# s-esposito/MonoGS

Hardware: AMD Instinct MI355X
Metric: rasteriser fwd+bwd Mpix/s @1080p (higher is better)
Workload: dtype f32; 1 GPU; C5: 2000000 Gaussians, 1920x1080, fwd+bwd, seeded synthetic map (SURVEY.md 8d), one keyframe per GPU; gaussians=2000000, width=1920, height=1080, settle_steps=60, instance_count=device-side (capacity mode, overflow checked), parallelism=keyframe-per-gpu x1

## Files before the change

monogs_amd/csrc/api.hip:

```cpp
#include "common.h"

#include <stdarg.h>
#include <stdio.h>
#include <string.h>

namespace mgs {

static thread_local char g_err[512] = "";

void set_error(const char* fmt, ...) {
    va_list ap;
    va_start(ap, fmt);
    vsnprintf(g_err, sizeof(g_err), fmt, ap);
    va_end(ap);
}

static inline char* take(char*& p, size_t bytes) {
    char* r = p;
    p += align_up(bytes, 256);
    return r;
}

GeometryState GeometryState::carve(void* base, int P) {
    char* p = (char*)align_up((size_t)base, 256);
// ... 17 lines not shown
    g.end = p;
    return g;
}
size_t GeometryState::bytes(int P) {
    const GeometryState g = carve(nullptr, P);
    return (size_t)g.end + 256;
}

size_t ImageState::bytes(int W, int H) {
    const size_t HW = (size_t)W * H, nt = (size_t)tiles_x(W) * tiles_y(H);
    return align_up(HW * 4, 256) * 2 + align_up(nt * sizeof(uint2), 256) + 256;
}
ImageState ImageState::carve(void* base, int W, int H) {
    const size_t HW = (size_t)W * H, nt = (size_t)tiles_x(W) * tiles_y(H);
    char* p = (char*)align_up((size_t)base, 256);
    ImageState s;
    s.final_T = (float*)take(p, HW * 4);
    s.n_contrib = (uint32_t*)take(p, HW * 4);
    s.ranges = (uint2*)take(p, nt * sizeof(uint2));
    return s;
}

size_t BinningState::fwd_mask_rows(uint64_t R, int W, int H) {
    return (size_t)(R / 64) + (size_t)tiles_x(W) * tiles_y(H) + 1;
}
size_t BinningState::bytes(uint64_t R, int W, int H) {
    const size_t r = (size_t)(R ? R : 1);
    return align_up(r * 4, 256) * 4 + align_up(mgs::sort_temp_bytes(R, tile_bits(W, H)), 256) + 256 +
           align_up(fwd_mask_rows(R, W, H) * 4 * sizeof(unsigned long long), 256) + 256;
}
BinningState BinningState::carve(void* base, uint64_t R, int W, int H) {
    const size_t r = (size_t)(R ? R : 1);
    char* p = (char*)align_up((size_t)base, 256);
    BinningState b;
    b.keys_a = (uint32_t*)take(p, r * 4);
    b.keys_b = (uint32_t*)take(p, r * 4);
    b.vals_a = (uint32_t*)take(p, r * 4);
    b.vals_b = (uint32_t*)take(p, r * 4);
    const bool in_b = radix_result_in_b(tile_bits(W, H));
    b.keys_sorted = in_b ? b.keys_b : b.keys_a;
    b.vals_sorted = in_b ? b.vals_b : b.vals_a;
    b.sort_temp_bytes = mgs::sort_temp_bytes(R, tile_bits(W, H));
    b.sort_temp = take(p, b.sort_temp_bytes);
    b.count = (uint32_t*)take(p, 2 * sizeof(uint32_t));
    b.fwd_masks = (unsigned long long*)take(p, fwd_mask_rows(R, W, H) * 4 * sizeof(unsigned long long));
    return b;
}

struct StageTimer {
    hipStream_t s;
    bool on;
    hipEvent_t ev[10];
    int n = 0;
    StageTimer(hipStream_t s_, bool on_) : s(s_), on(on_) {
        if (on) for (auto& e : ev) (void)hipEventCreate(&e);
    }
    ~StageTimer() {
        if (on) for (auto& e : ev) (void)hipEventDestroy(e);
    }
    void mark() {
        if (on && n < 10) (void)hipEventRecord(ev[n++], s);
    }
    float ms(int i) {
        float t = 0.f;
        if (on && i + 1 < n) (void)hipEventElapsedTime(&t, ev[i], ev[i + 1]);
        return t;
    }
    void sync() {
        if (on && n) (void)hipEventSynchronize(ev[n - 1]);
    }
};

static int check_cam(const mgs_camera* cam) {
    if (!cam) { set_error("camera is NULL"); return 1; }
    if (cam->image_width <= 0 || cam->image_height <= 0) { set_error("image size must be positive"); return 1; }
    if (!cam->bg || !cam->viewmatrix || !cam->projmatrix || !cam->projmatrix_raw || !cam->campos) {
        set_error("camera tensors (bg, viewmatrix, projmatrix, projmatrix_raw, campos) must be non-NULL");
        return 1;
    }
    return 0;
}

static hipEvent_t g_dbg_fwd_events[2] = {nullptr, nullptr}, g_dbg_bwd_events[2] = {nullptr, nullptr};

static int check_map_size(int32_t P) {
    if (P > MGS_MAX_GAUSSIANS) {
        set_error("P exceeds MGS_MAX_GAUSSIANS (2^26 - 1): the gradient-line offset of the blend backward is 32-bit");
        return 1;
    }
    return 0;
}

}

using namespace mgs;

extern "C" {

int mgs_abi_version(void) { return MGS_ABI_VERSION; }
int mgs_binning_path(int32_t P, int32_t W, int32_t H) { return binning_path(P, W, H); }
const char* mgs_last_error(void) { return g_err; }

size_t mgs_geometry_bytes(int32_t P) { return GeometryState::bytes(P < 0 ? 0 : P); }
size_t mgs_image_bytes(int32_t W, int32_t H) { return ImageState::bytes(W, H); }
size_t mgs_binning_bytes(uint64_t R, int32_t W, int32_t H) { return BinningState::bytes(R, W, H); }
size_t mgs_backward_bytes(int32_t P) {
    return (size_t)(P < 0 ? 0 : P) * GRAD_FLOATS * sizeof(float) + (size_t)(TAU_SLOTS + 1) * 16 * sizeof(float) + 256;
}
float* mgs_backward_tau(void* backward_scratch, int32_t P) { return backward_tau_out(backward_scratch, P < 0 ? 0 : P); }

int mgs_forward_preprocess(const mgs_camera* cam, int32_t P, const float* means3D, const float* shs,
                           const float* colors_precomp, const float* opacities, const float* scales,
                           const float* rotations, const float* cov3D_precomp, void* geometry, int32_t* radii,
                           void* prepare_backward, uint64_t* num_rendered, const uint32_t* prev_status,
                           uint32_t* prev_status_out, mgs_timing* timing, void* stream) {
    if (check_cam(cam)) return 1;
    if (P < 0) { set_error("P must be >= 0"); return 1; }
    if (check_map_size(P)) return 1;
    if (num_rendered) *num_rendered = 0;
    if (prev_status_out) *prev_status_out = 0;
    if (P == 0) {
        if (prev_status && prev_status_out) {
            MGS_HIP(hipMemcpyAsync(prev_status_out, prev_status, sizeof(uint32_t), hipMemcpyDeviceToHost, (hipStream_t)stream));
            MGS_HIP(hipStreamSynchronize((hipStream_t)stream));
        }
        return 0;
    }
    if (!means3D || !opacities || !geometry || !radii) { set_error("means3D, opacities, geometry, radii must be non-NULL"); return 1; }
    if ((shs == nullptr) == (colors_precomp == nullptr)) {
        set_error("Please provide excatly one of either SHs or precomputed colors!");
        return 1;
    }
    const bool have_sr = scales != nullptr || rotations != nullptr;
    if ((have_sr && (!scales || !rotations || cov3D_precomp)) || (!have_sr && !cov3D_precomp)) {
        set_error("Please provide exactly one of either scale/rotation pair or precomputed 3D covariance!");
        return 1;
    }
    if (shs && (cam->sh_degree < 0 || cam->sh_degree > 3 || cam->sh_coeffs < (cam->sh_degree + 1) * (cam->sh_degree + 1))) {
        set_error("sh_degree must be 0..3 and shs must hold at least (degree+1)^2 coefficients");
        return 1;
    }
    hipStream_t s = (hipStream_t)stream;
    GeometryState g = GeometryState::carve(geometry, P);
    StageTimer tm(s, timing != nullptr);
    tm.mark();
    if (int rc = launch_preprocess_forward(*cam, P, means3D, shs, colors_precomp, opacities, scales, rotations,
                                           cov3D_precomp, g, radii,
                                           prepare_backward ? backward_grad_acc(prepare_backward) : nullptr, s)) return rc;
    tm.mark();
    const bool exclusive = (cam->flags & MGS_FLAG_EXCLUSIVE_DEVICE) != 0;
    const bool per_tile = binning_path(P, cam->image_width, cam->image_height) != 0;
    if (per_tile) {
        tm.mark();
        if (int rc = launch_scan(g, P, s, exclusive, g.rect)) return rc;
    } else {
        if (int rc = launch_depth_sort(g, P, depth_sort_payload(P, cam->image_width, cam->image_height), s, exclusive)) return rc;
        tm.mark();
        if (int rc = launch_scan(g, P, s, exclusive, g.rect_sorted)) return rc;
    }
    tm.mark();
    if (num_rendered) {
        uint32_t total = 0, sort_errors[RADIX_ERROR_WORDS] = {0, 0, 0, 0};
        MGS_HIP(hipMemcpyAsync(&total, g.scan_blocks + scan_nblocks(P), sizeof(uint32_t), hipMemcpyDeviceToHost, s));
        MGS_HIP(hipMemcpyAsync(sort_errors, radix_depth_error_flag(g.sort_temp, (uint64_t)P), sizeof(sort_errors),
                               hipMemcpyDeviceToHost, s));
        if (prev_status && prev_status_out)
            MGS_HIP(hipMemcpyAsync(prev_status_out, prev_status, sizeof(uint32_t), hipMemcpyDeviceToHost, s));
        MGS_HIP(hipStreamSynchronize(s));
        if (sort_errors[0] | sort_errors[1] | sort_errors[2] | sort_errors[3]) { set_error("depth sort: a look-back spin timed out (results invalid)"); return 3; }
        *num_rendered = total;
    }
    if (timing) {
        if (!num_rendered) MGS_HIP(hipStreamSynchronize(s));
        timing->preprocess_ms = tm.ms(0);
        timing->depth_sort_ms = per_tile ? 0.f : tm.ms(1);
        timing->scan_ms = tm.ms(2);
    }
    return 0;
}

static int g_opt_tile_sort_fused = 1;

static int forward_render_impl(const mgs_camera* cam, int32_t P, uint64_t R, bool capacity, void* geometry,
                               void* binning, void* image, float* out_color, float* out_depth, float* out_opacity,
                               int32_t* n_touched, uint32_t* overflow, mgs_timing* timing, void* stream) {
    if (check_cam(cam)) return 1;
    if (P < 0) { set_error("P must be >= 0"); return 1; }
    if (check_map_size(P)) return 1;
    if (!image || !out_color || !out_depth || !out_opacity) { set_error("image scratch and outputs must be non-NULL"); return 1; }
    if (P > 0 && (!geometry || !n_touched)) { set_error("geometry and n_touched must be non-NULL"); return 1; }
    if (R > 0 && !binning) { set_error("binning scratch is NULL"); return 1; }
    if (R >= (1ull << 32)) { set_error("num_rendered exceeds 2^32-1"); return 1; }
    if (P == 0) R = 0;
    hipStream_t s = (hipStream_t)stream;
    const int W = cam->image_width, H = cam->image_height;
    GeometryState g = GeometryState::carve(geometry, P);
    ImageState img = ImageState::carve(image, W, H);
    BinningState b = BinningState::carve(binning, R, W, H);
    const uint32_t* n_dev = nullptr;
    StageTimer tm(s, timing != nullptr);
    const bool cap = capacity && binning;
    if (cap) n_dev = b.count;
    const bool per_tile = binning_path(P, W, H) != 0;
    tm.mark();
    if (int rc = launch_duplicate(*cam, P, g, b, capacity ? R : (R > 0 ? 0xFFFFFFFFull : 0ull), n_touched, img, R,
                                  tile_bits(W, H), cap ? b.count : nullptr, overflow, s, per_tile)) return rc;
    tm.mark();
    if (int rc = launch_sort(g, b, R, tile_bits(W, H), s, n_dev, (cam->flags & MGS_FLAG_EXCLUSIVE_DEVICE) != 0, img.ranges,
                             per_tile)) return rc;
    const uint32_t* sort_err = R > 0 ? radix_error_flag(b.sort_temp, R, tile_bits(W, H)) : nullptr;
    const bool sort_tiles = per_tile && R > 0;
    const TileSortArgs ts = sort_tiles ? tile_sort_args(*cam, g, b, R, n_dev) : TileSortArgs{};
    const bool fused = sort_tiles && g_opt_tile_sort_fused != 0;
    if (sort_tiles && !fused)
        if (int rc = launch_tile_depth_sort(*cam, ts, img, sort_err, s)) return rc;
    tm.mark();
    if (g_dbg_fwd_events[0]) MGS_HIP(hipEventRecord(g_dbg_fwd_events[0], s));
    if (int rc = launch_blend_forward(*cam, g, b, img, out_color, out_depth, out_opacity, n_touched, sort_err, overflow,
                                      fused ? &ts : nullptr, P, s)) return rc;
    if (g_dbg_fwd_events[1]) MGS_HIP(hipEventRecord(g_dbg_fwd_events[1], s));
    tm.mark();
    if (timing) {
        tm.sync();
        timing->duplicate_ms = tm.ms(0);
        timing->sort_ms = tm.ms(1);
        timing->ranges_ms = 0.f;
        timing->blend_fwd_ms = tm.ms(2);
    }
    return 0;
}

int mgs_forward_render(const mgs_camera* cam, int32_t P, uint64_t R, void* geometry, void* binning, void* image,
                       float* out_color, float* out_depth, float* out_opacity, int32_t* n_touched,
                       uint32_t* status, mgs_timing* timing, void* stream) {
    return forward_render_impl(cam, P, R, false, geometry, binning, image, out_color, out_depth, out_opacity, n_touched,
                               status, timing, stream);
}

int mgs_forward_render_capacity(const mgs_camera* cam, int32_t P, uint64_t capacity, void* geometry, void* binning,
                                void* image, float* out_color, float* out_depth, float* out_opacity,
                                int32_t* n_touched, uint32_t* overflow, mgs_timing* timing, void* stream) {
    if (capacity == 0) { set_error("capacity must be > 0"); return 1; }
    return forward_render_impl(cam, P, capacity, true, geometry, binning, image, out_color, out_depth, out_opacity,
                               n_touched, overflow, timing, stream);
}

int mgs_forward_capacity(const mgs_camera* cam, int32_t P, const float* means3D, const float* shs,
                         const float* colors_precomp, const float* opacities, const float* scales, const float* rotations,
                         const float* cov3D_precomp, void* geometry, int32_t* radii, void* prepare_backward,
                         uint64_t capacity, void* binning, void* image, float* out_color, float* out_depth,
                         float* out_opacity, int32_t* n_touched, uint32_t* overflow, mgs_timing* timing, void* stream) {
    if (int rc = mgs_forward_preprocess(cam, P, means3D, shs, colors_precomp, opacities, scales, rotations, cov3D_precomp,
                                        geometry, radii, prepare_backward, nullptr, nullptr, nullptr, timing, stream)) return rc;
    return mgs_forward_render_capacity(cam, P, capacity, geometry, binning, image, out_color, out_depth, out_opacity,
                                       n_touched, overflow, timing, stream);
}

int mgs_backward(const mgs_camera* cam, int32_t P, uint64_t R, const float* means3D, const float* shs,
                 const float* colors_precomp, const float* opacities, const float* scales, const float* rotations,
                 const float* cov3D_precomp, const int32_t* radii, const void* geometry, const void* binning,
                 const void* image, const float* dL_dcolor, const float* dL_ddepth, const float* out_color,
                 const float* out_depth, float* dL_dmeans2D, float* dL_dcolors, float* dL_dopacity, float* dL_dmeans3D, float* dL_dcov3D, float* dL_dsh,
                 float* dL_dscales, float* dL_drotations, float* dL_dtau, void* backward_scratch,
                 int32_t scratch_prepared, mgs_timing* timing, void* stream) {
    if (check_cam(cam)) return 1;
    if (P < 0) { set_error("P must be >= 0"); return 1; }
    if (check_map_size(P)) return 1;
    hipStream_t s = (hipStream_t)stream;
    if (P == 0) {
        if (dL_dtau) MGS_HIP(zero_fill(dL_dtau, 6 * sizeof(float), s));
        return 0;
    }
    if (!means3D || !opacities || !radii || !geometry || !image || !dL_dcolor || !dL_ddepth || !backward_scratch) {
        set_error("means3D, opacities, radii, geometry, image, dL_dcolor, dL_ddepth, backward_scratch must be non-NULL");
        return 1;
    }
    if (R > 0 && !binning) { set_error("binning scratch is NULL"); return 1; }
    const int W = cam->image_width, H = cam->image_height;
    GeometryState g = GeometryState::carve(const_cast<void*>(geometry), P);
    ImageState img = ImageState::carve(const_cast<void*>(image), W, H);
    BinningState b = BinningState::carve(const_cast<void*>(binning), R, W, H);
    float* grad_acc = backward_grad_acc(backward_scratch);
    StageTimer tm(s, timing != nullptr);
    float* tau_part = (dL_dtau && (P + 255) / 256 > TAU_DIRECT_MAX_BLOCKS) ? backward_tau_part(backward_scratch, P) : nullptr;
    if (scratch_prepared) {
        if (dL_dtau && dL_dtau != backward_tau_out(backward_scratch, P)) {
            set_error("scratch_prepared: dL_dtau must be mgs_backward_tau(backward_scratch, P)");
            return 1;
        }
    } else {
        MGS_HIP(zero_fill2(grad_acc, (size_t)P * GRAD_FLOATS * sizeof(float) + (tau_part ? (size_t)TAU_SLOTS * 16 * sizeof(float) : 0),
                           dL_dtau, 6 * sizeof(float), s));
    }
    tm.mark();
    if (R > 0) {
        const bool pose_only = !dL_dcolors && !dL_dopacity && !dL_dsh && !shs;
        if (g_dbg_bwd_events[0]) MGS_HIP(hipEventRecord(g_dbg_bwd_events[0], s));
        if (int rc = launch_blend_backward(*cam, g, b, img, dL_dcolor, dL_ddepth, out_color, out_depth, grad_acc, pose_only, R, s)) return rc;
        if (g_dbg_bwd_events[1]) MGS_HIP(hipEventRecord(g_dbg_bwd_events[1], s));
    }
    tm.mark();
    GeomBackwardArgs a;
    a.means3D = means3D; a.shs = shs; a.colors_precomp = colors_precomp; a.opacities = opacities;
    a.scales = scales; a.rotations = rotations; a.cov3D_precomp = cov3D_precomp; a.radii = radii;
    a.grad_acc = grad_acc;
    a.dL_dmeans2D = dL_dmeans2D; a.dL_dcolors = dL_dcolors; a.dL_dopacity = dL_dopacity;
    a.dL_dmeans3D = dL_dmeans3D; a.dL_dcov3D = dL_dcov3D; a.dL_dsh = dL_dsh; a.dL_dscales = dL_dscales;
// ... 154 lines not shown
```

monogs_amd/csrc/binning.hip:

```cpp
#include "common.h"
#include "tile_sort.h"


namespace mgs {

constexpr int SCAN_THREADS = 256;
__device__ __forceinline__ int scan_nblocks_dev(int P) { return (P + SCAN_ITEMS - 1) / SCAN_ITEMS; }
constexpr int SCAN_PER_THREAD = SCAN_ITEMS / SCAN_THREADS;

__device__ __forceinline__ uint32_t wave_incl_scan(uint32_t v, int) { return wave_incl_scan_dpp(v); }

__device__ __forceinline__ uint32_t block_excl_scan(uint32_t v, uint32_t& total, uint32_t* smem ) {
    const int lane = threadIdx.x & 63, wv = threadIdx.x >> 6;
    const uint32_t incl = wave_incl_scan(v, lane);
    if (lane == 63) smem[wv] = incl;
    __syncthreads();
    uint32_t base = 0;
    for (int w = 0; w < wv; ++w) base += smem[w];
    total = smem[0] + smem[1] + smem[2] + smem[3];
    __syncthreads();
    return base + incl - v;
}

__device__ __forceinline__ uint32_t scan_block_rows(const uint2* __restrict__ rects, int n, int cbase, int lane, int wv,
                                                    uint32_t (&incl)[SCAN_PER_THREAD], uint32_t* smem ) {
    uint32_t v[SCAN_PER_THREAD];
#pragma unroll
    for (int i = 0; i < SCAN_PER_THREAD; ++i) {
        const int idx = cbase + i * WAVE + lane;
        const uint32_t wh = idx < n ? rects[idx].y : 0u;
        v[i] = (wh & 0xFFFFu) * (wh >> 16);
    }
    uint32_t run = 0;
#pragma unroll
    for (int i = 0; i < SCAN_PER_THREAD; ++i) {
        const uint32_t sc = wave_incl_scan_dpp(v[i]);
        incl[i] = run + sc;
        run += (uint32_t)__builtin_amdgcn_readlane((int)sc, 63);
    }
    if (lane == 0) smem[wv] = run;
    __syncthreads();
    uint32_t wbase = 0;
    for (int w = 0; w < wv; ++w) wbase += smem[w];
    const uint32_t total = (smem[0] + smem[1]) + (smem[2] + smem[3]);
#pragma unroll
    for (int i = 0; i < SCAN_PER_THREAD; ++i) incl[i] += wbase;
    return total;
}

__global__ void __launch_bounds__(SCAN_THREADS) scan_local_kernel(const uint2* __restrict__ rects, uint32_t* out,
                                                                  uint32_t* block_sums, int n) {
    __shared__ uint32_t smem[8];
    const int lane = threadIdx.x & 63, wv = threadIdx.x >> 6;
    const int cbase = blockIdx.x * SCAN_ITEMS + wv * (SCAN_PER_THREAD * WAVE);
    uint32_t incl[SCAN_PER_THREAD];
    const uint32_t total = scan_block_rows(rects, n, cbase, lane, wv, incl, smem);
#pragma unroll
    for (int i = 0; i < SCAN_PER_THREAD; ++i) {
        const int idx = cbase + i * WAVE + lane;
        if (idx < n) out[idx] = incl[i];
    }
    if (threadIdx.x == 0) block_sums[blockIdx.x] = total;
}

__global__ void __launch_bounds__(SCAN_THREADS) scan_blocks_kernel(uint32_t* block_sums, int nblocks) {
    __shared__ uint32_t smem[8];
    uint32_t carry = 0;
    for (int start = 0; start < nblocks; start += SCAN_THREADS) {
        const int i = start + threadIdx.x;
        const uint32_t v = i < nblocks ? block_sums[i] : 0u;
        uint32_t total;
        const uint32_t ex = block_excl_scan(v, total, smem);
        if (i < nblocks) block_sums[i] = carry + ex;
        carry += total;
    }
    if (threadIdx.x == 0) block_sums[nblocks] = carry;
}

constexpr uint32_t SCAN_SPIN_LIMIT = 1u << 22;
__global__ void __launch_bounds__(SCAN_THREADS) scan_small_kernel(const uint2* __restrict__ rects, uint32_t* out,
                                                                  uint32_t* block_sums, uint64_t* status, int n, int nb,
                                                                  uint32_t* err, int ticketed) {
    __shared__ uint32_t smem[8];
    __shared__ uint32_t s_prefix, s_bid;
    const int lane = threadIdx.x & 63, wv = threadIdx.x >> 6;
    int bid = (int)blockIdx.x;
    if (ticketed) {
        if (threadIdx.x == 0) s_bid = atomicAdd((uint32_t*)(status + SCAN_SMALL_MAX_BLOCKS), 1u);
        __syncthreads();
        bid = (int)s_bid;
    }
    const int cbase = bid * SCAN_ITEMS + wv * (SCAN_PER_THREAD * WAVE);
    uint32_t incl[SCAN_PER_THREAD];
    const uint32_t total = scan_block_rows(rects, n, cbase, lane, wv, incl, smem);
    if (threadIdx.x == 0)
        __hip_atomic_store(status + bid, (1ull << 63) | (uint64_t)total, __ATOMIC_RELAXED, __HIP_MEMORY_SCOPE_AGENT);
    if (threadIdx.x < WAVE) {
        uint32_t before = 0;
        if ((int)threadIdx.x < bid) {
            uint64_t w = 0;
            uint32_t spins = 0;
            while (true) {
                w = __hip_atomic_load(status + threadIdx.x, __ATOMIC_RELAXED, __HIP_MEMORY_SCOPE_AGENT);
                if (w >> 63) break;
                if (++spins > SCAN_SPIN_LIMIT) { atomicExch(err, 1u); break; }
                __builtin_amdgcn_s_sleep(1);
            }
            before = (uint32_t)w;
        }
#pragma unroll
        for (int o = 32; o > 0; o >>= 1) before += __shfl_xor(before, o, 64);
        if (threadIdx.x == 0) s_prefix = before;
    }
    __syncthreads();
#pragma unroll
    for (int i = 0; i < SCAN_PER_THREAD; ++i) {
        const int idx = cbase + i * WAVE + lane;
        if (idx < n) out[idx] = incl[i] + s_prefix;
    }
    if (threadIdx.x == 0 && bid == nb - 1) block_sums[nb] = s_prefix + total;
}
int g_opt_scan_small = -1;
bool scan_is_small(int P) { return g_opt_scan_small != 0 && scan_nblocks(P) <= SCAN_SMALL_MAX_BLOCKS; }


int launch_scan(const GeometryState& g, int P, hipStream_t s, bool exclusive, const uint2* rects) {
    if (P == 0) return 0;
    const int nb = scan_nblocks(P);
    if (scan_is_small(P)) {
        hipLaunchKernelGGL(scan_small_kernel, dim3(nb), dim3(SCAN_THREADS), 0, s, rects, g.point_offsets, g.scan_blocks,
                           g.scan_status, P, nb, const_cast<uint32_t*>(radix_depth_error_flag(g.sort_temp, (uint64_t)P)),
                           exclusive ? 0 : 1);
        MGS_HIP(hipGetLastError());
        return 0;
    }
    hipLaunchKernelGGL(scan_local_kernel, dim3(nb), dim3(SCAN_THREADS), 0, s, rects, g.point_offsets,
                       g.scan_blocks, P);
    hipLaunchKernelGGL(scan_blocks_kernel, dim3(1), dim3(SCAN_THREADS), 0, s, g.scan_blocks, nb);
    MGS_HIP(hipGetLastError());
    return 0;
}

__device__ __forceinline__ void dup_pair(uint32_t gidx, const uint32_t* __restrict__ depth_key, int lo, uint32_t& val,
                                         uint32_t& kfield) {
    val = gidx; kfield = 0u;
    if (depth_key) {
        const uint32_t k = depth_key[gidx];
        const uint32_t d = k == 0xFFFFFFFFu ? DEPTH_KEY_NARROW : min(k - DEPTH_KEY_SUB, DEPTH_KEY_NARROW);
        kfield = d >> lo;
        if (lo) val |= (d & ((1u << lo) - 1u)) << (32 - lo);
    }
}
__global__ void __launch_bounds__(256) duplicate_kernel(int P, const uint2* __restrict__ rects,
                                                        const uint32_t* __restrict__ perm,
                                                        const uint32_t* __restrict__ depth_key, int tshift, int lo,
                                                        const uint32_t* __restrict__ offsets ,
                                                        const uint32_t* __restrict__ block_sums ,
                                                        uint32_t* keys,
                                                        uint32_t* vals, int gx, int gy, uint32_t r_cap,
                                                        int32_t* __restrict__ n_touched, uint2* __restrict__ ranges,
                                                        int ntiles, uint32_t* __restrict__ zero_ptr, size_t zero_words,
                                                        uint32_t* __restrict__ count, uint32_t* __restrict__ overflow,
                                                        const uint32_t* __restrict__ depth_err, int offsets_global,
                                                        uint32_t* __restrict__ hist , int hist_passes,
                                                        int n_threads , int slot_major,
                                                        unsigned long long* __restrict__ prepare ) {
    const int i = blockIdx.x * 256 + threadIdx.x;
    if (i == 0 && prepare) {
        prepare[1] = prepare[0];
        prepare[0] = 0ull;
    }
    const int lane = threadIdx.x & 63;
    grid_zero(zero_ptr, zero_words, (size_t)n_threads, 256);
    const bool depth_bad = depth_err && radix_failed(depth_err) != 0u;
    if (i == 0 && count) {
        const uint32_t R = (P > 0 && !depth_bad) ? block_sums[scan_nblocks_dev(P)] : 0u;
        count[0] = min(R, r_cap);
        count[1] = R > r_cap ? 1u : 0u;
    }
    if (i == 0 && overflow)
        overflow[0] = (count ? count[1] : 0u) | (depth_bad ? (uint32_t)MGS_STATUS_DEPTH_SORT_TIMEOUT : 0u);
    if (i < ntiles) ranges[i] = make_uint2(0xFFFFFFFFu, 0u);
    if (i < P) n_touched[i] = 0;
    uint32_t idx = 0, nt = 0, off = 0, kf = 0;
    int x0 = 0, y0 = 0, x1 = 0;
    if (i < P) {
        dup_pair(perm ? perm[i] : (uint32_t)i, depth_key, lo, idx, kf);
        const uint2 r = rects[i];
        const int w = (int)(r.y & 0xFFFFu), h = (int)(r.y >> 16);
        nt = (uint32_t)(w * h);
        x0 = (int)(r.x & 0xFFFFu); y0 = (int)(r.x >> 16); x1 = x0 + w;
    }
    if (depth_bad) nt = 0;
    if (nt) off = i == 0 ? 0u : offsets[i - 1] + (offsets_global ? 0u : block_sums[(i - 1) / SCAN_ITEMS]);
    __shared__ uint32_t s_own[4][WAVE];
    __shared__ uint32_t s_idx[4][WAVE], s_off[4][WAVE], s_kf[4][WAVE];
    __shared__ int s_x0[4][WAVE], s_y0[4][WAVE], s_w[4][WAVE];
    __shared__ uint32_t s_hist[2][256];
    if (hist) {
        s_hist[0][threadIdx.x] = 0u; s_hist[1][threadIdx.x] = 0u;
        __syncthreads();
    }
    const int wv = threadIdx.x >> 6;
    if (slot_major) {
        const uint32_t R_all = (P > 0 && !depth_bad) ? block_sums[scan_nblocks_dev(P)] : 0u;
        const uint32_t R_emit = min(R_all, r_cap);
        const uint32_t n_waves = (uint32_t)n_threads / WAVE;
        const uint32_t CH = (((R_emit + n_waves - 1u) / n_waves) + 63u) & ~63u;
        const uint32_t wave_id = (uint32_t)blockIdx.x * 4u + (uint32_t)wv;
        const uint64_t s0w = (uint64_t)wave_id * CH;
        const uint32_t s0 = s0w < (uint64_t)R_emit ? (uint32_t)s0w : R_emit, s1 = (uint64_t)s0 + CH < (uint64_t)R_emit ? s0 + CH : R_emit;
        auto incl = [&](uint32_t k) { return offsets[k] + (offsets_global ? 0u : block_sums[k / SCAN_ITEMS]); };
        uint32_t g = 0;
        if (s0 < s1) {
            uint32_t lo = 0, hi = (uint32_t)P;
            while (hi - lo > 1u) {
                const uint32_t span = hi - lo, step = (span + 63u) / 64u;
                const uint32_t probe = lo + min(((uint32_t)lane + 1u) * step, span) - 1u;
                const unsigned long long above = __builtin_amdgcn_ballot_w64(incl(probe) > s0);
                const int k = __builtin_ctzll(above);
                const uint32_t pk = lo + min(((uint32_t)k + 1u) * step, span) - 1u;
                const uint32_t pk1 = k == 0 ? lo : lo + min((uint32_t)k * step, span);
                lo = pk1; hi = pk + 1u;
            }
            g = lo;
        }
        uint32_t sl = s0;
        while (sl < s1 && g < (uint32_t)P) {
            const uint32_t gi = g + (uint32_t)lane;
            const bool valid = gi < (uint32_t)P;
            uint32_t inc = 0, ntg = 0, idg = 0, kfg = 0;
            int gx0 = 0, gy0 = 0, gw = 1;
            if (valid) {
                inc = incl(gi);
                const uint2 r = rects[gi];
                gw = (int)(r.y & 0xFFFFu);
                ntg = (uint32_t)(gw * (int)(r.y >> 16));
                gx0 = (int)(r.x & 0xFFFFu); gy0 = (int)(r.x >> 16);
                dup_pair(perm ? perm[gi] : gi, depth_key, lo, idg, kfg);
            }
            const uint32_t exc = inc - ntg;
            uint32_t Eg = valid ? inc : 0u;
#pragma unroll
            for (int o2 = 32; o2 > 0; o2 >>= 1) Eg = max(Eg, (uint32_t)__shfl_xor((int)Eg, o2, 64));
            __builtin_amdgcn_wave_barrier();
            s_idx[wv][lane] = idg; s_kf[wv][lane] = kfg; s_off[wv][lane] = exc; s_x0[wv][lane] = gx0; s_y0[wv][lane] = gy0; s_w[wv][lane] = max(gw, 1);
            const uint32_t e = min(s1, Eg);
            const uint32_t cb0 = sl & ~63u;
            const unsigned long long before = __builtin_amdgcn_ballot_w64(ntg != 0u && exc < cb0);
            uint32_t carry = before ? 64u - (uint32_t)__builtin_clzll(before) : 0u;
            for (uint32_t cb = cb0; cb < e; cb += WAVE) {
                __builtin_amdgcn_wave_barrier();
                s_own[wv][lane] = 0u;
                __builtin_amdgcn_wave_barrier();
                if (ntg != 0u && exc >= cb && exc < cb + WAVE) s_own[wv][exc - cb] = (uint32_t)lane + 1u;
                __builtin_amdgcn_wave_barrier();
                uint32_t m = s_own[wv][lane];
#define MGS_DPP_MAX(ctrl, row_mask) m = max(m, (uint32_t)__builtin_amdgcn_update_dpp(0, (int)m, ctrl, row_mask, 0xf, false))
                MGS_DPP_MAX(0x111, 0xf); MGS_DPP_MAX(0x112, 0xf); MGS_DPP_MAX(0x114, 0xf); MGS_DPP_MAX(0x118, 0xf);
                MGS_DPP_MAX(0x142, 0xa); MGS_DPP_MAX(0x143, 0xc);
#undef MGS_DPP_MAX
                const uint32_t owner = max(m, carry);
                carry = (uint32_t)__builtin_amdgcn_readlane((int)owner, 63);
                const uint32_t o = cb + lane;
                if (owner != 0u && o >= sl && o < e) {
                    const uint32_t L = owner - 1u;
                    const uint32_t t = o - s_off[wv][L];
                    const uint32_t w = (uint32_t)s_w[wv][L];
                    const uint32_t yy = t / w, xx = t - yy * w;
                    const uint32_t tid = (uint32_t)((s_y0[wv][L] + (int)yy) * gx + s_x0[wv][L] + (int)xx);
                    const uint32_t key = (tid << tshift) | s_kf[wv][L];
                    keys[o] = key;
                    vals[o] = s_idx[wv][L];
                    if (hist) {
                        atomicAdd(&s_hist[0][(key >> tshift) & 0xFFu], 1u);
                        if (hist_passes > 1) {
                            const uint32_t d1 = (key >> (tshift + 8)) & 0xFFu;
                            const uint32_t lead = (uint32_t)__builtin_amdgcn_readfirstlane((int)d1);
                            const unsigned long long same = __builtin_amdgcn_ballot_w64(d1 == lead);
                            if (d1 != lead) atomicAdd(&s_hist[1][d1], 1u);
                            else if (lane == (int)__builtin_ctzll(same)) atomicAdd(&s_hist[1][lead], (uint32_t)__popcll(same));
                        }
                    }
                }
            }
            sl = max(sl, e);
            if (Eg <= sl) g += WAVE;
        }
        if (hist) {
            __syncthreads();
            const uint32_t c0 = s_hist[0][threadIdx.x], c1 = s_hist[1][threadIdx.x];
            if (c0) atomicAdd(hist + threadIdx.x, c0);
            if (c1) atomicAdd(hist + 256 + threadIdx.x, c1);
        }
        return;
    }
    s_idx[wv][lane] = idx; s_kf[wv][lane] = kf; s_off[wv][lane] = off; s_x0[wv][lane] = x0; s_y0[wv][lane] = y0; s_w[wv][lane] = max(x1 - x0, 1);
    const unsigned long long live = __builtin_amdgcn_ballot_w64(nt != 0);
    if (live == 0ull && !hist) return;
    const int first = live ? __builtin_ctzll(live) : 0, lastl = live ? 63 - __builtin_clzll(live) : 0;
    const uint32_t S = live ? (uint32_t)__builtin_amdgcn_readlane((int)off, first) : 0u;
    const uint32_t E = live ? (uint32_t)__builtin_amdgcn_readlane((int)(off + nt), lastl) : 0u;
    uint32_t carry = 0;
    for (uint32_t cb = S & ~63u; cb < E; cb += WAVE) {
        __builtin_amdgcn_wave_barrier();
        s_own[wv][lane] = 0u;
        __builtin_amdgcn_wave_barrier();
        if (nt != 0 && off >= cb && off < cb + WAVE) s_own[wv][off - cb] = (uint32_t)lane + 1u;
        __builtin_amdgcn_wave_barrier();
        uint32_t m = s_own[wv][lane];
#define MGS_DPP_MAX(ctrl, row_mask) m = max(m, (uint32_t)__builtin_amdgcn_update_dpp(0, (int)m, ctrl, row_mask, 0xf, false))
        MGS_DPP_MAX(0x111, 0xf); MGS_DPP_MAX(0x112, 0xf); MGS_DPP_MAX(0x114, 0xf); MGS_DPP_MAX(0x118, 0xf);
        MGS_DPP_MAX(0x142, 0xa); MGS_DPP_MAX(0x143, 0xc);
#undef MGS_DPP_MAX
        const uint32_t owner = max(m, carry);
        carry = (uint32_t)__builtin_amdgcn_readlane((int)owner, 63);
        const uint32_t o = cb + lane;
        if (owner != 0u && o < E && o < r_cap) {
            const uint32_t L = owner - 1u;
            const uint32_t t = o - s_off[wv][L];
            const uint32_t w = (uint32_t)s_w[wv][L];
            const uint32_t yy = t / w, xx = t - yy * w;
            const uint32_t tid = (uint32_t)((s_y0[wv][L] + (int)yy) * gx + s_x0[wv][L] + (int)xx);
            const uint32_t key = (tid << tshift) | s_kf[wv][L];
            keys[o] = key;
            vals[o] = s_idx[wv][L];
            if (hist) {
                atomicAdd(&s_hist[0][(key >> tshift) & 0xFFu], 1u);
                if (hist_passes > 1) {
                    const uint32_t d1 = (key >> (tshift + 8)) & 0xFFu;
                    const uint32_t lead = (uint32_t)__builtin_amdgcn_readfirstlane((int)d1);
                    const unsigned long long same = __builtin_amdgcn_ballot_w64(d1 == lead);
                    if (d1 != lead) atomicAdd(&s_hist[1][d1], 1u);
                    else if (lane == (int)__builtin_ctzll(same)) atomicAdd(&s_hist[1][lead], (uint32_t)__popcll(same));
                }
            }
        }
    }
    if (hist) {
        __syncthreads();
        const uint32_t c0 = s_hist[0][threadIdx.x], c1 = s_hist[1][threadIdx.x];
        if (c0) atomicAdd(hist + threadIdx.x, c0);
        if (c1) atomicAdd(hist + 256 + threadIdx.x, c1);
    }
}

constexpr uint64_t DUP_SLOT_MAJOR_MIN = 768ull * 1024;
int g_opt_dup_slot_major = -1;

int launch_duplicate(const mgs_camera& cam, int P, const GeometryState& g, const BinningState& b, uint64_t r_cap,
                     int32_t* n_touched, const ImageState& img, uint64_t sort_n, int sort_bits, uint32_t* count,
                     uint32_t* overflow, hipStream_t s, bool per_tile) {
    const uint32_t* depth_err = P > 0 ? radix_depth_error_flag(g.sort_temp, (uint64_t)P) : nullptr;
    const int ntiles = tiles_x(cam.image_width) * tiles_y(cam.image_height);
    int n = P > ntiles ? P : ntiles;
    if (n == 0) return 0;
    const bool slot_major = P > 0 && g_opt_dup_slot_major != 0 &&
                            (g_opt_dup_slot_major > 0 || (sort_n >= DUP_SLOT_MAJOR_MIN && sort_n >= 6ull * (uint64_t)P));
    if (slot_major) {
        const uint64_t want = sort_n / 8;
        if (want > (uint64_t)n) n = (int)(want > 0x3FFFFFFFull ? 0x3FFFFFFFull : want);
    }
    const int n_threads = (n + 255) / 256 * 256;
    uint32_t* zero_ptr = nullptr;
    size_t zero_words = 0;
    if (sort_n > 0) radix_zero_region(b.sort_temp, sort_n, sort_bits, &zero_ptr, &zero_words);
    const bool count_digits = P > 0 && sort_bits <= 16 && radix_wants_hist(sort_n);
    const int tb = tile_bits(cam.image_width, cam.image_height);
    hipLaunchKernelGGL(duplicate_kernel, dim3(n_threads / 256), dim3(256), 0, s, P, per_tile ? g.rect : g.rect_sorted,
                       per_tile ? nullptr : g.perm, per_tile ? g.depth_key : nullptr, per_tile ? 32 - tb : 0,
                       per_tile ? tile_depth_lo_bits(tb) : 0, g.point_offsets,
                       g.scan_blocks, b.keys_a, b.vals_a, tiles_x(cam.image_width), tiles_y(cam.image_height),
                       (uint32_t)(r_cap > 0xFFFFFFFFull ? 0xFFFFFFFFull : r_cap), n_touched, img.ranges, ntiles, zero_ptr,
                       zero_words, count, overflow, depth_err,
                       (P > 0 && scan_is_small(P)) ? 1 : 0,
                       count_digits ? g.tile_hist : nullptr, (sort_bits + 7) / 8, n_threads, slot_major ? 1 : 0,
                       P > 0 ? g.prepare : nullptr);
    MGS_HIP(hipGetLastError());
    return 0;
}

size_t sort_temp_bytes(uint64_t n, int bits) { return radix_temp_bytes(n, bits); }

int launch_depth_sort(const GeometryState& g, int P, bool payload, hipStream_t s, bool exclusive) {
    return radix_sort_depth(g.depth_key, g.depth_alt, g.iota, g.iota_alt, g.rect, payload, g.perm, g.rect_sorted, (uint64_t)P,
                            g.sort_temp, s, true, exclusive);
}

int launch_sort(const GeometryState& g, const BinningState& b, uint64_t R, int bits, hipStream_t s, const uint32_t* n_dev,
                bool exclusive, uint2* ranges, bool per_tile) {
    if (R == 0) return 0;
    const bool counted = bits <= 16 && radix_wants_hist(R) && g.tile_hist != nullptr;
    return radix_sort_pairs(b.keys_a, b.vals_a, b.keys_b, b.vals_b, R, bits, b.sort_temp, s, n_dev, true, nullptr, nullptr,
                            counted ? g.tile_hist : nullptr, false, exclusive, ranges, per_tile ? 32 - bits : 0);
}

TileSortArgs tile_sort_args(const mgs_camera& cam, const GeometryState& g, const BinningState& b, uint64_t R,
                            const uint32_t* n_dev) {
    TileSortArgs ts;
    ts.keys = b.keys_sorted;
    ts.vals = b.vals_sorted;
    ts.keys_alt = b.keys_sorted == b.keys_a ? b.keys_b : b.keys_a;
    ts.vals_alt = b.vals_sorted == b.vals_a ? b.vals_b : b.vals_a;
    ts.depth_key = g.depth_key;
    ts.n_dev = n_dev;
    ts.n_cap = (uint32_t)R;
    ts.tb = tile_bits(cam.image_width, cam.image_height);
    return ts;
}

__global__ void __launch_bounds__(TDS_THREADS) tile_depth_sort_kernel(TileSortArgs ts, const uint2* __restrict__ ranges,
                                                                       int ntiles, const uint32_t* __restrict__ sort_err) {
    __shared__ uint32_t s_k[TDS_CAP], s_v[TDS_CAP];
    __shared__ uint32_t s_cnt[TDS_WAVES][TDS_RADIX];
    __shared__ uint32_t s_wsum[TDS_WAVES], s_red[2 * TDS_WAVES];
    const int tile = blockIdx.x;
    if (tile >= ntiles) return;
    tile_depth_sort(ts, ranges[tile], sort_err && radix_failed(sort_err) != 0u, TdsLds{s_k, s_v, s_cnt, s_wsum, s_red});
}

int launch_tile_depth_sort(const mgs_camera& cam, const TileSortArgs& ts, const ImageState& img, const uint32_t* sort_err,
                           hipStream_t s) {
    const int ntiles = tiles_x(cam.image_width) * tiles_y(cam.image_height);
    hipLaunchKernelGGL(tile_depth_sort_kernel, dim3(ntiles), dim3(TDS_THREADS), 0, s, ts, img.ranges, ntiles, sort_err);
    MGS_HIP(hipGetLastError());
    return 0;
}


}
```

monogs_amd/csrc/common.h:

```cpp
#pragma once

#include <hip/hip_runtime.h>
#include <stdint.h>
#include <stddef.h>

#include "../../include/monogs_raster.h"

namespace mgs {

constexpr int TILE = MGS_TILE;
constexpr int WAVE = 64;
constexpr int SUB = 8;
constexpr int REC_FLOATS = 16;
constexpr int GRAD_FLOATS = 16;

enum : int {
    R_X = 0, R_Y = 1, R_EX = 2, R_EY = 3,
    R_CA = 4, R_CB = 5, R_CC = 6, R_OPAC = 7,
    R_R = 8, R_G = 9, R_B = 10, R_DEPTH = 11,
    R_NA = 12, R_NB = 13, R_NC = 14, R_RADIUS = 15
};
enum : int {
    G_SX = 0, G_SY = 1, G_SXX = 2, G_SXY = 3, G_SYY = 4, G_SH = 5,
    G_DR = 6, G_DG = 7, G_DB = 8, G_DDEPTH = 9
};

inline size_t align_up(size_t v, size_t a) { return (v + a - 1) / a * a; }

#if defined(__HIP_DEVICE_COMPILE__)
typedef const float __attribute__((address_space(4))) * const_float_p;
typedef const unsigned long long __attribute__((address_space(4))) * const_u64_p;
#define MGS_CONST(p) ((mgs::const_float_p)(p))
#define MGS_CONST_U64(p) ((mgs::const_u64_p)(p))
#else
typedef const float* const_float_p;
typedef const unsigned long long* const_u64_p;
#define MGS_CONST(p) (p)
#define MGS_CONST_U64(p) (p)
#endif

__device__ __forceinline__ uint32_t wave_incl_scan_dpp(uint32_t v) {
#define MGS_DPP_ADD(ctrl, row_mask) v += (uint32_t)__builtin_amdgcn_update_dpp(0, (int)v, ctrl, row_mask, 0xf, false)
    MGS_DPP_ADD(0x111, 0xf);
    MGS_DPP_ADD(0x112, 0xf);
    MGS_DPP_ADD(0x114, 0xf);
    MGS_DPP_ADD(0x118, 0xf);
    MGS_DPP_ADD(0x142, 0xa);
    MGS_DPP_ADD(0x143, 0xc);
#undef MGS_DPP_ADD
    return v;
}

__global__ static void zero_fill_kernel(uint32_t* __restrict__ p, size_t n_words, int vec) {
    const size_t i0 = (size_t)blockIdx.x * blockDim.x + threadIdx.x, stride = (size_t)gridDim.x * blockDim.x;
    if (vec) {
        uint4* q = reinterpret_cast<uint4*>(p);
        const size_t nv = n_words / 4;
        for (size_t i = i0; i < nv; i += stride) q[i] = make_uint4(0u, 0u, 0u, 0u);
        for (size_t i = nv * 4 + i0; i < n_words; i += stride) p[i] = 0u;
    } else {
        for (size_t i = i0; i < n_words; i += stride) p[i] = 0u;
    }
}
__device__ __forceinline__ void grid_zero(uint32_t* __restrict__ p, size_t n_words, size_t threads, int block) {
    const size_t i0 = (size_t)blockIdx.x * block + threadIdx.x, stride = threads;
    uint4* q = reinterpret_cast<uint4*>(p);
    const size_t nv = n_words / 4;
    for (size_t i = i0; i < nv; i += stride) q[i] = make_uint4(0u, 0u, 0u, 0u);
    for (size_t i = nv * 4 + i0; i < n_words; i += stride) p[i] = 0u;
}
__global__ static void zero_fill2_kernel(uint32_t* __restrict__ p, size_t n_words, uint32_t* __restrict__ p2, int n2) {
    grid_zero(p, n_words, (size_t)gridDim.x * 256, 256);
    if (blockIdx.x == 0 && (int)threadIdx.x < n2) p2[threadIdx.x] = 0u;
}
static inline hipError_t zero_fill2(void* ptr, size_t bytes, void* ptr2, size_t bytes2, hipStream_t s) {
    const size_t n_words = bytes / 4;
    size_t blocks = (n_words / 4 + 255) / 256;
    blocks = blocks < 1 ? 1 : (blocks > 4096 ? 4096 : blocks);
    hipLaunchKernelGGL(zero_fill2_kernel, dim3((unsigned)blocks), dim3(256), 0, s, (uint32_t*)ptr, n_words,
                       (uint32_t*)ptr2, ptr2 ? (int)(bytes2 / 4) : 0);
    return hipGetLastError();
}
static inline hipError_t zero_fill(void* ptr, size_t bytes, hipStream_t s) {
    if (bytes == 0) return hipSuccess;
    const size_t n_words = bytes / 4;
    const int vec = ((size_t)ptr % 16 == 0) ? 1 : 0;
    const size_t items = vec ? (n_words + 3) / 4 : n_words;
    size_t blocks = (items + 255) / 256;
    if (blocks > 4096) blocks = 4096;
    hipLaunchKernelGGL(zero_fill_kernel, dim3((unsigned)blocks), dim3(256), 0, s, (uint32_t*)ptr, n_words, vec);
    return hipGetLastError();
}

struct GeometryState {
    float* rec;
    uint32_t* depth_key;
    uint32_t* depth_alt;
    uint32_t* iota;
    uint32_t* iota_alt;
    uint32_t* perm;
    uint32_t* point_offsets;
    uint32_t* scan_blocks;
    uint8_t* clamped;
    uint2* rect;
    uint2* rect_sorted;
    uint64_t* scan_status;
    uint32_t* tile_hist;
    void* sort_temp;
    size_t sort_temp_bytes;
    unsigned long long* prepare;
    char* end;
    static size_t bytes(int P);
    static GeometryState carve(void* base, int P);
};
constexpr int SCAN_SMALL_MAX_BLOCKS = 64;

struct ImageState {
    float* final_T;
    uint32_t* n_contrib;
    uint2* ranges;
    static size_t bytes(int W, int H);
    static ImageState carve(void* base, int W, int H);
};

struct BinningState {
    uint32_t* keys_a;
    uint32_t* vals_a;
    uint32_t* keys_b;
    uint32_t* vals_b;
    uint32_t* keys_sorted;
    uint32_t* vals_sorted;
    void* sort_temp;
    size_t sort_temp_bytes;
    uint32_t* count;
    unsigned long long* fwd_masks;
    static size_t fwd_mask_rows(uint64_t R, int W, int H);
    static size_t bytes(uint64_t R, int W, int H);
    static BinningState carve(void* base, uint64_t R, int W, int H);
};

constexpr int SCAN_ITEMS = 2048;
inline int scan_nblocks(int P) { return (P + SCAN_ITEMS - 1) / SCAN_ITEMS; }

inline int tiles_x(int W) { return (W + TILE - 1) / TILE; }
inline int tiles_y(int H) { return (H + TILE - 1) / TILE; }
inline int tile_bits(int W, int H) {
    uint32_t n = (uint32_t)(tiles_x(W) * tiles_y(H));
    int b = 0;
    while ((1u << b) < n && b < 31) ++b;
    return b == 0 ? 1 : b;
}

constexpr uint32_t DEPTH_KEY_SUB = 0x3E4CCCCDu;
constexpr uint32_t DEPTH_KEY_NARROW = (1u << 27) - 1u;
__host__ __device__ inline int tile_depth_lo_bits(int tb) { return tb > 5 ? tb - 5 : 0; }
int binning_path(int P, int W, int H);

void set_error(const char* fmt, ...);
#define MGS_HIP(expr)                                                                     \
    do {                                                                                  \
        hipError_t _e = (expr);                                                           \
        if (_e != hipSuccess) {                                                           \
            mgs::set_error("%s failed: %s (%s:%d)", #expr, hipGetErrorString(_e), __FILE__, __LINE__); \
            return 2;                                                                     \
        }                                                                                 \
    } while (0)

struct StageTimer;

int launch_preprocess_forward(const mgs_camera& cam, int P, const float* means3D, const float* shs,
                              const float* colors_precomp, const float* opacities, const float* scales,
                              const float* rotations, const float* cov3D_precomp,
                              const GeometryState& g, int32_t* radii, float* prepare_grad_acc, hipStream_t s);
constexpr int TAU_SLOTS = 256;
inline float* backward_grad_acc(void* scratch) { return (float*)align_up((size_t)scratch, 256); }
inline float* backward_tau_part(void* scratch, int P) { return backward_grad_acc(scratch) + (size_t)P * GRAD_FLOATS; }
inline float* backward_tau_out(void* scratch, int P) { return backward_tau_part(scratch, P) + (size_t)TAU_SLOTS * 16; }
int launch_scan(const GeometryState& g, int P, hipStream_t s, bool exclusive, const uint2* rects);
int launch_duplicate(const mgs_camera& cam, int P, const GeometryState& g, const BinningState& b, uint64_t r_cap,
                     int32_t* n_touched, const ImageState& img, uint64_t sort_n, int sort_bits, uint32_t* count,
                     uint32_t* overflow, hipStream_t s, bool per_tile);
size_t sort_temp_bytes(uint64_t n, int bits);
size_t radix_temp_bytes(uint64_t n, int bits);
size_t radix_depth_temp_bytes(uint64_t n);
bool radix_result_in_b(int bits);
constexpr int RADIX_ERROR_WORDS = 4;
const uint32_t* radix_error_flag(void* temp, uint64_t n, int bits);
const uint32_t* radix_depth_error_flag(void* temp, uint64_t n);
__device__ __forceinline__ uint32_t radix_failed(const uint32_t* __restrict__ e) { return (e[0] | e[1]) | (e[2] | e[3]); }
void radix_zero_region(void* temp, uint64_t n, int bits, uint32_t** ptr, size_t* words);
void radix_depth_zero_region(void* temp, uint64_t n, uint32_t** ptr, size_t* words, bool header_only = false);
int radix_sort_pairs(uint32_t* ka, uint32_t* va, uint32_t* kb, uint32_t* vb, uint64_t n, int bits, void* temp,
                     hipStream_t s, const uint32_t* n_dev = nullptr, bool temp_zeroed = false,
                     const uint2* aux_in = nullptr, uint2* aux_out = nullptr,
                     const uint32_t* ext_hist = nullptr,
                     bool aux_empty_for_ones = false,
                     bool exclusive = false,
                     uint2* ranges = nullptr,
                     int key_shift = 0);
bool radix_wants_hist(uint64_t n);
bool radix_depth_payload(uint64_t n);
int radix_sort_depth(uint32_t* keys, uint32_t* key_b, uint32_t* val_a, uint32_t* val_b, void* rect, bool payload,
                     uint32_t* perm, uint2* rect_sorted, uint64_t n, void* temp, hipStream_t s, bool temp_zeroed,
                     bool exclusive = false);
inline bool depth_sort_payload(int P, int W, int H) { return radix_depth_payload((uint64_t)P) && tiles_x(W) <= 255 && tiles_y(H) <= 255; }
int launch_depth_sort(const GeometryState& g, int P, bool payload, hipStream_t s, bool exclusive = false);
int launch_sort(const GeometryState& g, const BinningState& b, uint64_t R, int bits, hipStream_t s,
                const uint32_t* n_dev = nullptr, bool exclusive = false, uint2* ranges = nullptr, bool per_tile = false);
struct TileSortArgs {
    uint32_t* keys;
    uint32_t* vals;
    uint32_t* keys_alt;
    uint32_t* vals_alt;
    const uint32_t* depth_key;
    const uint32_t* n_dev;
    uint32_t n_cap;
    int tb;
};
TileSortArgs tile_sort_args(const mgs_camera& cam, const GeometryState& g, const BinningState& b, uint64_t R,
                            const uint32_t* n_dev);
int launch_tile_depth_sort(const mgs_camera& cam, const TileSortArgs& ts, const ImageState& img, const uint32_t* sort_err,
                           hipStream_t s);
int set_radix_spin_limit(uint32_t limit);
extern bool g_opt_blend_bwd_transposed_set;
extern int g_dbg_last_bwd_split;
extern int g_opt_radix_ballot_rank, g_opt_radix_scanned, g_opt_radix_xcd_band, g_opt_knn_grid_min, g_opt_scan_small, g_opt_dup_slot_major, g_opt_blend_bwd_transposed, g_opt_blend_bwd_split, g_opt_blend_bwd_split_min, g_opt_blend_bwd_split_frac;
int launch_blend_forward(const mgs_camera& cam, const GeometryState& g, const BinningState& b,
                         const ImageState& img, float* out_color, float* out_depth, float* out_opacity,
                         int32_t* n_touched, const uint32_t* sort_err, uint32_t* status, const TileSortArgs* tile_sort,
                         int P, hipStream_t s);
int launch_blend_backward(const mgs_camera& cam, const GeometryState& g, const BinningState& b,
                          const ImageState& img, const float* dL_dcolor, const float* dL_ddepth, const float* out_color,
                          const float* out_depth, float* grad_acc, bool pose_only, uint64_t num_rendered, hipStream_t s);
int launch_blend_backward_stats(const mgs_camera& cam, const GeometryState& g, const BinningState& b,
                                const ImageState& img, unsigned long long* stats, hipStream_t s);
int launch_blend_mask_stats(const mgs_camera& cam, const GeometryState& g, const BinningState& b,
                            const ImageState& img, unsigned long long* stats, hipStream_t s);
int launch_valu_ceiling(float* out, int iters, hipStream_t s);
int launch_features_forward(const mgs_camera& cam, int P, int K, const GeometryState& g, const BinningState& b,
                            const ImageState& img, const float* features, const float* bg, float* out, int32_t* labels,
                            float min_opacity, hipStream_t s);
int launch_features_backward(const mgs_camera& cam, int P, int K, const GeometryState& g, const BinningState& b,
                             const ImageState& img, const float* dL_dout, float* dL_dfeatures, hipStream_t s);
struct GeomBackwardArgs {
    const float *means3D, *shs, *colors_precomp, *opacities, *scales, *rotations, *cov3D_precomp;
    const int32_t* radii;
    const float* grad_acc;
    float *dL_dmeans2D, *dL_dcolors, *dL_dopacity, *dL_dmeans3D, *dL_dcov3D, *dL_dsh, *dL_dscales,
        *dL_drotations, *dL_dtau;
    float* tau_part;
};
constexpr int TAU_DIRECT_MAX_BLOCKS = 256;
int launch_geom_backward(const mgs_camera& cam, int P, const GeometryState& g, const GeomBackwardArgs& a,
                         hipStream_t s);
int launch_mark_visible(int P, const float* means3D, const float* viewmatrix, uint8_t* visible, hipStream_t s);
size_t knn_scratch_bytes(int P);
int launch_knn(int P, const float* points, float* out, void* scratch, hipStream_t s);

}
```

monogs_amd/csrc/preprocess.hip:

```cpp
#include "common.h"

#pragma clang fp contract(off)

namespace mgs {

__device__ __forceinline__ float dot3p(float m0, float m1, float m2, float m3, float x, float y, float z) {
    return ((m0 * x + m1 * y) + m2 * z) + m3;
}

__device__ constexpr float SH_C0 = 0.28209479177387814f;
__device__ constexpr float SH_C1 = 0.4886025119029199f;
__device__ constexpr float SH_C2[5] = {1.0925484305920792f, -1.0925484305920792f, 0.31539156525252005f,
                                       -1.0925484305920792f, 0.5462742152960396f};
__device__ constexpr float SH_C3[7] = {-0.5900435899266435f, 2.890611442640554f, -0.4570457994644658f,
                                       0.3731763325901154f, -0.4570457994644658f, 1.445305721320277f,
                                       -0.5900435899266435f};

struct Cam {
    float V[16], PM[16], PR[16];
    float campos[3];
    float tanfovx, tanfovy, focal_x, focal_y, mod;
    int W, H, gx, gy, deg, M;
};

__device__ __forceinline__ void load_cam(Cam& c, const float* V_, const float* PM_, const float* PR_,
                                         const float* campos_) {
    const const_float_p V = MGS_CONST(V_), PM = MGS_CONST(PM_), PR = MGS_CONST(PR_), campos = MGS_CONST(campos_);
#pragma unroll
    for (int i = 0; i < 16; ++i) { c.V[i] = V[i]; c.PM[i] = PM[i]; }
    if (PR_) {
#pragma unroll
        for (int i = 0; i < 16; ++i) c.PR[i] = PR[i];
    } else {
#pragma unroll
        for (int i = 0; i < 16; ++i) c.PR[i] = 0.f;
    }
    c.campos[0] = campos[0]; c.campos[1] = campos[1]; c.campos[2] = campos[2];
}

__device__ __forceinline__ void pin_cam(const Cam& c, bool with_pr) {
    asm volatile("" ::"s"(c.V[0]), "s"(c.V[1]), "s"(c.V[2]), "s"(c.V[3]), "s"(c.V[4]), "s"(c.V[5]), "s"(c.V[6]), "s"(c.V[7]),
                 "s"(c.V[8]), "s"(c.V[9]), "s"(c.V[10]), "s"(c.V[11]), "s"(c.V[12]), "s"(c.V[13]), "s"(c.V[14]), "s"(c.V[15]));
    asm volatile("" ::"s"(c.PM[0]), "s"(c.PM[1]), "s"(c.PM[2]), "s"(c.PM[3]), "s"(c.PM[4]), "s"(c.PM[5]), "s"(c.PM[6]),
                 "s"(c.PM[7]), "s"(c.PM[8]), "s"(c.PM[9]), "s"(c.PM[10]), "s"(c.PM[11]), "s"(c.PM[12]), "s"(c.PM[13]),
                 "s"(c.PM[14]), "s"(c.PM[15]), "s"(c.campos[0]), "s"(c.campos[1]), "s"(c.campos[2]));
    if (with_pr)
        asm volatile("" ::"s"(c.PR[0]), "s"(c.PR[1]), "s"(c.PR[2]), "s"(c.PR[3]), "s"(c.PR[4]), "s"(c.PR[5]), "s"(c.PR[6]),
                     "s"(c.PR[7]), "s"(c.PR[8]), "s"(c.PR[9]), "s"(c.PR[10]), "s"(c.PR[11]), "s"(c.PR[12]), "s"(c.PR[13]),
                     "s"(c.PR[14]), "s"(c.PR[15]));
}

__device__ __forceinline__ void cov3d_from_scale_rot(const float s[3], const float q[4], float mod, float cov[6],
                                                     float Mm[9]) {
    const float r = q[0], x = q[1], y = q[2], z = q[3];
    float Rm[9] = {1.f - 2.f * (y * y + z * z), 2.f * (x * y - r * z), 2.f * (x * z + r * y),
                   2.f * (x * y + r * z), 1.f - 2.f * (x * x + z * z), 2.f * (y * z - r * x),
                   2.f * (x * z - r * y), 2.f * (y * z + r * x), 1.f - 2.f * (x * x + y * y)};
    const float sx = s[0] * mod, sy = s[1] * mod, sz = s[2] * mod;
#pragma unroll
    for (int i = 0; i < 3; ++i) {
        Mm[3 * i + 0] = Rm[3 * i + 0] * sx;
        Mm[3 * i + 1] = Rm[3 * i + 1] * sy;
        Mm[3 * i + 2] = Rm[3 * i + 2] * sz;
    }
    auto e = [&](int i, int j) {
        return (Mm[3 * i] * Mm[3 * j] + Mm[3 * i + 1] * Mm[3 * j + 1]) + Mm[3 * i + 2] * Mm[3 * j + 2];
    };
    cov[0] = e(0, 0); cov[1] = e(0, 1); cov[2] = e(0, 2);
    cov[3] = e(1, 1); cov[4] = e(1, 2); cov[5] = e(2, 2);
}

struct Proj {
    float tx, ty, tz;
    bool clamp_x, clamp_y;
    float J00, J02, J11, J12;
    float T0[3], T1[3];
    float cxx, cxy, cyy;
};

__device__ __forceinline__ void project_cov(const Cam& c, const float pv[3], const float cov[6], Proj& p) {
    const float limx = 1.3f * c.tanfovx, limy = 1.3f * c.tanfovy;
    const float tz = pv[2];
    const float txtz = pv[0] / tz, tytz = pv[1] / tz;
    p.clamp_x = (txtz < -limx) || (txtz > limx);
    p.clamp_y = (tytz < -limy) || (tytz > limy);
    p.tx = fminf(limx, fmaxf(-limx, txtz)) * tz;
    p.ty = fminf(limy, fmaxf(-limy, tytz)) * tz;
    p.tz = tz;
    const float tz2 = tz * tz;
    p.J00 = c.focal_x / tz;
    p.J02 = -(c.focal_x * p.tx) / tz2;
    p.J11 = c.focal_y / tz;
    p.J12 = -(c.focal_y * p.ty) / tz2;
#pragma unroll
    for (int j = 0; j < 3; ++j) {
        p.T0[j] = p.J00 * c.V[4 * j + 0] + p.J02 * c.V[4 * j + 2];
        p.T1[j] = p.J11 * c.V[4 * j + 1] + p.J12 * c.V[4 * j + 2];
    }
    const float S[3][3] = {{cov[0], cov[1], cov[2]}, {cov[1], cov[3], cov[4]}, {cov[2], cov[4], cov[5]}};
    float U0[3], U1[3];
#pragma unroll
    for (int j = 0; j < 3; ++j) {
        U0[j] = (p.T0[0] * S[0][j] + p.T0[1] * S[1][j]) + p.T0[2] * S[2][j];
        U1[j] = (p.T1[0] * S[0][j] + p.T1[1] * S[1][j]) + p.T1[2] * S[2][j];
    }
    p.cxx = ((U0[0] * p.T0[0] + U0[1] * p.T0[1]) + U0[2] * p.T0[2]) + 0.3f;
    p.cxy = (U0[0] * p.T1[0] + U0[1] * p.T1[1]) + U0[2] * p.T1[2];
    p.cyy = ((U1[0] * p.T1[0] + U1[1] * p.T1[1]) + U1[2] * p.T1[2]) + 0.3f;
}

__device__ __forceinline__ void tile_rect(float px, float py, float radius, int gx, int gy, int& x0, int& y0,
                                          int& x1, int& y1) {
    x0 = min(gx, max(0, (int)((px - radius) / (float)TILE)));
    y0 = min(gy, max(0, (int)((py - radius) / (float)TILE)));
    x1 = min(gx, max(0, (int)(((px + radius) + (float)(TILE - 1)) / (float)TILE)));
    y1 = min(gy, max(0, (int)(((py + radius) + (float)(TILE - 1)) / (float)TILE)));
}

__device__ __forceinline__ void eval_sh(int deg, const float* sh, const float d[3], float out[3]) {
    const float x = d[0], y = d[1], z = d[2];
#pragma unroll
    for (int ch = 0; ch < 3; ++ch) {
        float res = SH_C0 * sh[ch];
        if (deg > 0) {
            res = res - SH_C1 * y * sh[3 + ch] + SH_C1 * z * sh[6 + ch] - SH_C1 * x * sh[9 + ch];
            if (deg > 1) {
                const float xx = x * x, yy = y * y, zz = z * z, xy = x * y, yz = y * z, xz = x * z;
                res = res + SH_C2[0] * xy * sh[12 + ch] + SH_C2[1] * yz * sh[15 + ch] +
                      SH_C2[2] * (2.f * zz - xx - yy) * sh[18 + ch] + SH_C2[3] * xz * sh[21 + ch] +
                      SH_C2[4] * (xx - yy) * sh[24 + ch];
                if (deg > 2) {
                    res = res + SH_C3[0] * y * (3.f * xx - yy) * sh[27 + ch] + SH_C3[1] * xy * z * sh[30 + ch] +
                          SH_C3[2] * y * (4.f * zz - xx - yy) * sh[33 + ch] +
                          SH_C3[3] * z * (2.f * zz - 3.f * xx - 3.f * yy) * sh[36 + ch] +
                          SH_C3[4] * x * (4.f * zz - xx - yy) * sh[39 + ch] + SH_C3[5] * z * (xx - yy) * sh[42 + ch] +
                          SH_C3[6] * x * (xx - 3.f * yy) * sh[45 + ch];
                }
            }
        }
        out[ch] = res + 0.5f;
    }
}

struct PreArgs {
    const float *means3D, *shs, *colors, *opacities, *scales, *rotations, *cov3D;
    const float *V, *PM, *campos;
    float* rec;
    uint32_t* depth_key;
    int rect_packed;
    uint8_t* clamped;
    uint2* rect;
    int32_t* radii;
    float tanfovx, tanfovy, focal_x, focal_y, mod;
    int P, W, H, gx, gy, deg, M;
    int iso;
    int rot_aligned16;
    uint32_t* zero_ptr;
    size_t zero_words;
    float* grad_acc;
    unsigned long long* prepare;
};

__device__ __forceinline__ void load4(const float* __restrict__ p, bool aligned16, float o[4]) {
    if (aligned16) {
        const float4 v = *reinterpret_cast<const float4*>(p);
        o[0] = v.x; o[1] = v.y; o[2] = v.z; o[3] = v.w;
    } else {
        o[0] = p[0]; o[1] = p[1]; o[2] = p[2]; o[3] = p[3];
    }
}

struct PreOut {
    float4 r0, r1, r2, r3;
    int radius;
    uint2 rect;
    uint32_t key;
};

template <bool COV, bool PRECOMP>
__device__ __forceinline__ bool preprocess_one(const PreArgs& a, const Cam& c, int idx, float x, float y, float z,
                                               const float cov_in[6], const float s[3], const float q[4],
                                               const float col_in[3], float opac, PreOut& o) {
    float pv[3];
#pragma unroll
    for (int k = 0; k < 3; ++k) pv[k] = dot3p(c.V[k], c.V[4 + k], c.V[8 + k], c.V[12 + k], x, y, z);
    if (!(pv[2] > 0.2f)) return false;
    float ph[4];
#pragma unroll
    for (int k = 0; k < 4; ++k) ph[k] = dot3p(c.PM[k], c.PM[4 + k], c.PM[8 + k], c.PM[12 + k], x, y, z);
    const float p_w = 1.0f / (ph[3] + 0.0000001f);
    const float projx = ph[0] * p_w, projy = ph[1] * p_w;

    float cov[6];
    if (COV) {
#pragma unroll
        for (int k = 0; k < 6; ++k) cov[k] = cov_in[k];
    } else {
        float Mm[9];
        cov3d_from_scale_rot(s, q, a.mod, cov, Mm);
    }
    Proj p;
    project_cov(c, pv, cov, p);
    const float det = p.cxx * p.cyy - p.cxy * p.cxy;
    if (det == 0.0f) return false;
    const float det_inv = 1.f / det;
    const float ca = p.cyy * det_inv, cb = -p.cxy * det_inv, cc = p.cxx * det_inv;
    const float mid = 0.5f * (p.cxx + p.cyy);
    const float disc = sqrtf(fmaxf(0.1f, mid * mid - det));
    const float lam = fmaxf(mid + disc, mid - disc);
    const float radius = ceilf(3.f * sqrtf(lam));
    const float px = ((projx + 1.0f) * (float)a.W - 1.0f) * 0.5f;
    const float py = ((projy + 1.0f) * (float)a.H - 1.0f) * 0.5f;
    if (!(isfinite(px) && isfinite(py) && isfinite(radius))) return false;
    int x0, y0, x1, y1;
    tile_rect(px, py, radius, a.gx, a.gy, x0, y0, x1, y1);
    const int ntile = (x1 - x0) * (y1 - y0);
    if (ntile == 0) return false;

    float rgb[3];
    if (PRECOMP) {
        rgb[0] = col_in[0]; rgb[1] = col_in[1]; rgb[2] = col_in[2];
    } else {
        float d[3] = {x - c.campos[0], y - c.campos[1], z - c.campos[2]};
        const float len = sqrtf((d[0] * d[0] + d[1] * d[1]) + d[2] * d[2]);
        d[0] = d[0] / len; d[1] = d[1] / len; d[2] = d[2] / len;
        eval_sh(a.deg, a.shs + (size_t)idx * a.M * 3, d, rgb);
#pragma unroll
        for (int ch = 0; ch < 3; ++ch) {
            a.clamped[4 * idx + ch] = rgb[ch] < 0.f;
            rgb[ch] = fmaxf(rgb[ch], 0.f);
        }
    }

    float ex = -1.f, ey = -1.f;
    float na = 0.f, nb = 0.f, nc = 0.f;
    const float tau = logf(255.0f * opac);
    if (tau > 0.f) {
        ex = sqrtf(2.f * tau * p.cxx) * 1.001f + 0.05f;
        ey = sqrtf(2.f * tau * p.cyy) * 1.001f + 0.05f;
        const float it = 1.f / (2.f * tau);
        na = ca * it; nb = cb * it; nc = cc * it;
    } else if (!(tau <= 0.f)) {
        ex = ey = 3.0e38f;
    }

    o.r0 = make_float4(px, py, ex, ey);
    constexpr float LOG2E = 1.4426950408889634f;
    o.r1 = make_float4(-0.5f * LOG2E * ca, -LOG2E * cb, -0.5f * LOG2E * cc, opac);
    o.r2 = make_float4(rgb[0], rgb[1], rgb[2], pv[2]);
    o.r3 = make_float4(na, nb, nc, radius);
    o.radius = (int)radius;
    o.rect = make_uint2((uint32_t)x0 | ((uint32_t)y0 << 16), (uint32_t)(x1 - x0) | ((uint32_t)(y1 - y0) << 16));
    o.key = __float_as_uint(pv[2]);
    return true;
}

template <bool COV, bool PRECOMP>
__global__ void __launch_bounds__(256) preprocess_forward_kernel(PreArgs a) {
    const int idx = blockIdx.x * 256 + threadIdx.x;
    grid_zero(a.zero_ptr, a.zero_words, (size_t)((a.P + 255) / 256) * 256, 256);
    if (a.grad_acc && blockIdx.x == 0) {
        float4* t4 = reinterpret_cast<float4*>(a.grad_acc + (size_t)a.P * GRAD_FLOATS);
        for (int i = threadIdx.x; i < (TAU_SLOTS + 1) * 4; i += 256) t4[i] = make_float4(0.f, 0.f, 0.f, 0.f);
    }
    if (idx == 0) a.prepare[0] = (unsigned long long)(uintptr_t)a.grad_acc;
    if (idx >= a.P) return;
    Cam c;
    load_cam(c, a.V, a.PM, nullptr, a.campos);
    c.tanfovx = a.tanfovx; c.tanfovy = a.tanfovy; c.focal_x = a.focal_x; c.focal_y = a.focal_y;
    const float x = a.means3D[3 * idx], y = a.means3D[3 * idx + 1], z = a.means3D[3 * idx + 2];
    const float opac = a.opacities[idx];
    float cov_in[6] = {0.f, 0.f, 0.f, 0.f, 0.f, 0.f}, s[3] = {0.f, 0.f, 0.f}, q[4] = {1.f, 0.f, 0.f, 0.f};
    float col_in[3] = {0.f, 0.f, 0.f};
    if (COV) {
#pragma unroll
        for (int k = 0; k < 6; ++k) cov_in[k] = a.cov3D[6 * idx + k];
    } else {
        const float* sp = a.scales + (a.iso ? (size_t)idx : 3 * (size_t)idx);
        const int o1 = a.iso ? 0 : 1, o2 = a.iso ? 0 : 2;
        s[0] = sp[0]; s[1] = sp[o1]; s[2] = sp[o2];
        load4(a.rotations + 4 * (size_t)idx, a.rot_aligned16 != 0, q);
    }
    if (PRECOMP) { col_in[0] = a.colors[3 * idx]; col_in[1] = a.colors[3 * idx + 1]; col_in[2] = a.colors[3 * idx + 2]; }
    asm volatile("" ::"v"(x), "v"(y), "v"(z), "v"(opac), "v"(s[0]), "v"(s[1]), "v"(s[2]), "v"(q[0]), "v"(q[1]), "v"(q[2]),
                 "v"(q[3]), "v"(col_in[0]), "v"(col_in[1]), "v"(col_in[2]));
    if (COV) asm volatile("" ::"v"(cov_in[0]), "v"(cov_in[1]), "v"(cov_in[2]), "v"(cov_in[3]), "v"(cov_in[4]), "v"(cov_in[5]));
    pin_cam(c, false);

    PreOut o;
    const bool vis = preprocess_one<COV, PRECOMP>(a, c, idx, x, y, z, cov_in, s, q, col_in, opac, o);
    a.radii[idx] = vis ? o.radius : 0;
    if (a.rect_packed) {
        const uint32_t r4 = (o.rect.x & 0xFFu) | ((o.rect.x >> 16) << 8) | ((o.rect.y & 0xFFu) << 16) | ((o.rect.y >> 16) << 24);
        reinterpret_cast<uint32_t*>(a.rect)[idx] = vis ? r4 : 0u;
    } else {
        a.rect[idx] = vis ? o.rect : make_uint2(0u, 0u);
    }
    a.depth_key[idx] = vis ? o.key : 0xFFFFFFFFu;
    {
        __shared__ float4 s_rec[4][WAVE * 5];
        const int lane = threadIdx.x & 63, wv = threadIdx.x >> 6, wave_first = idx - lane;
        if (wave_first + WAVE <= a.P) {
            const unsigned long long vm = __builtin_amdgcn_ballot_w64(vis);
            float4* mine = s_rec[wv] + lane * 5;
            mine[0] = o.r0; mine[1] = o.r1; mine[2] = o.r2; mine[3] = o.r3;
            float4* base = reinterpret_cast<float4*>(a.rec + (size_t)wave_first * REC_FLOATS);
#pragma unroll
            for (int k = 0; k < 4; ++k) {
                const int src = (lane >> 2) + 16 * k;
                const float4 v = s_rec[wv][src * 5 + (lane & 3)];
                if ((vm >> src) & 1ull) base[k * WAVE + lane] = v;
            }
        } else if (vis) {
            float4* rec = reinterpret_cast<float4*>(a.rec + (size_t)idx * REC_FLOATS);
            rec[0] = o.r0; rec[1] = o.r1; rec[2] = o.r2; rec[3] = o.r3;
        }
    }
}

int launch_preprocess_forward(const mgs_camera& cam, int P, const float* means3D, const float* shs,
                              const float* colors_precomp, const float* opacities, const float* scales,
                              const float* rotations, const float* cov3D_precomp, const GeometryState& g,
                              int32_t* radii, float* prepare_grad_acc, hipStream_t s) {
    PreArgs a;
    a.means3D = means3D; a.shs = shs; a.colors = colors_precomp; a.opacities = opacities;
    a.scales = scales; a.rotations = rotations; a.cov3D = cov3D_precomp;
    a.V = cam.viewmatrix; a.PM = cam.projmatrix; a.campos = cam.campos;
    a.rec = g.rec; a.depth_key = g.depth_key;
    a.grad_acc = prepare_grad_acc;
    a.prepare = g.prepare;
    a.rot_aligned16 = rotations && ((size_t)rotations % 16 == 0);
    a.clamped = g.clamped; a.rect = g.rect; a.radii = radii;
    a.tanfovx = cam.tanfovx; a.tanfovy = cam.tanfovy;
    a.focal_x = (float)cam.image_width / (2.0f * cam.tanfovx);
    a.focal_y = (float)cam.image_height / (2.0f * cam.tanfovy);
    a.mod = cam.scale_modifier;
    a.iso = cam.scale_dim == 1;
    a.P = P; a.W = cam.image_width; a.H = cam.image_height;
    a.gx = tiles_x(a.W); a.gy = tiles_y(a.H); a.deg = cam.sh_degree; a.M = cam.sh_coeffs;
    if (P == 0) return 0;
    const bool per_tile = binning_path(P, cam.image_width, cam.image_height) != 0;
    a.rect_packed = (!per_tile && depth_sort_payload(P, cam.image_width, cam.image_height)) ? 1 : 0;
    radix_depth_zero_region(g.sort_temp, (uint64_t)P, &a.zero_ptr, &a.zero_words, per_tile);
    a.zero_words += (size_t)((char*)a.zero_ptr - (char*)g.scan_status) / 4;
    a.zero_ptr = (uint32_t*)g.scan_status;
    const dim3 grid((P + 255) / 256), block(256);
    if (cov3D_precomp && colors_precomp) hipLaunchKernelGGL((preprocess_forward_kernel<true, true>), grid, block, 0, s, a);
    else if (cov3D_precomp) hipLaunchKernelGGL((preprocess_forward_kernel<true, false>), grid, block, 0, s, a);
    else if (colors_precomp) hipLaunchKernelGGL((preprocess_forward_kernel<false, true>), grid, block, 0, s, a);
    else hipLaunchKernelGGL((preprocess_forward_kernel<false, false>), grid, block, 0, s, a);
    MGS_HIP(hipGetLastError());
    return 0;
}

struct BwdArgs {
    GeomBackwardArgs g;
    const float *V, *PM, *PR, *campos;
    const float* rec;
    const uint8_t* clamped;
    float tanfovx, tanfovy, focal_x, focal_y, mod;
    int P, W, H, deg, M;
    int iso;
    int rot_aligned16, drot_aligned16;
};

__device__ __forceinline__ float wave_sum(float v) {
#pragma unroll
    for (int o = 32; o > 0; o >>= 1) v += __shfl_xor(v, o, 64);
    return v;
}

template <bool SH, bool COV>
__global__ void __launch_bounds__(256) geom_backward_kernel(BwdArgs a) {
    const int idx = blockIdx.x * 256 + threadIdx.x;
    float tau[6] = {0.f, 0.f, 0.f, 0.f, 0.f, 0.f};
    const bool in = idx < a.P;
    const size_t ci = in ? (size_t)idx : 0;
    Cam c;
    load_cam(c, a.V, a.PM, a.PR, a.campos);
    c.tanfovx = a.tanfovx; c.tanfovy = a.tanfovy; c.focal_x = a.focal_x; c.focal_y = a.focal_y;
    const int rad = a.g.radii[ci];
    const float x = a.g.means3D[3 * ci], y = a.g.means3D[3 * ci + 1], z = a.g.means3D[3 * ci + 2];
    const float opq = a.g.opacities[ci];
    __shared__ float4 s_ga[4][WAVE * 5];
    const int lane_ = threadIdx.x & 63, wv_ = threadIdx.x >> 6, wave_first = idx - lane_;
    const bool full_wave = wave_first + WAVE <= a.P;
    const float4* gsrc = full_wave ? reinterpret_cast<const float4*>(a.g.grad_acc + (size_t)wave_first * GRAD_FLOATS) + lane_
                                   : reinterpret_cast<const float4*>(a.g.grad_acc + ci * GRAD_FLOATS);
    const int gstep = full_wave ? WAVE : 1;
    const float4 t0 = gsrc[0], t1 = gsrc[gstep], t2 = gsrc[2 * gstep], t3 = gsrc[3 * gstep];
    float cov[6] = {0.f, 0.f, 0.f, 0.f, 0.f, 0.f}, Mm[9];
    float s[3] = {0.f, 0.f, 0.f}, q[4] = {1.f, 0.f, 0.f, 0.f};
    if (COV) {
#pragma unroll
        for (int k = 0; k < 6; ++k) cov[k] = a.g.cov3D_precomp[6 * ci + k];
        asm volatile("" ::"v"(cov[0]), "v"(cov[1]), "v"(cov[2]), "v"(cov[3]), "v"(cov[4]), "v"(cov[5]));
    } else {
        const float* sp = a.g.scales + (a.iso ? ci : 3 * ci);
        const int o1 = a.iso ? 0 : 1, o2 = a.iso ? 0 : 2;
        s[0] = sp[0]; s[1] = sp[o1]; s[2] = sp[o2];
        load4(a.g.rotations + 4 * ci, a.rot_aligned16 != 0, q);
        asm volatile("" ::"v"(s[0]), "v"(s[1]), "v"(s[2]), "v"(q[0]), "v"(q[1]), "v"(q[2]), "v"(q[3]));
    }
    asm volatile("" ::"v"(rad), "v"(x), "v"(y), "v"(z), "v"(opq));
    float4 ga0 = t0, ga1 = t1, ga2 = t2;
    if (full_wave) {
        float4* row = s_ga[wv_] + (lane_ >> 2) * 5 + (lane_ & 3);
        row[0] = t0; row[16 * 5] = t1; row[32 * 5] = t2; row[48 * 5] = t3;
        ga0 = s_ga[wv_][lane_ * 5 + 0]; ga1 = s_ga[wv_][lane_ * 5 + 1]; ga2 = s_ga[wv_][lane_ * 5 + 2];
    }
    pin_cam(c, true);
    const float ga[GRAD_FLOATS] = {ga0.x, ga0.y, ga0.z, ga0.w, ga1.x, ga1.y, ga1.z, ga1.w, ga2.x, ga2.y, 0.f, 0.f, 0.f, 0.f, 0.f, 0.f};
    const bool live = in && rad > 0;
    float o_m2[2] = {0.f, 0.f}, o_m3[3] = {0.f, 0.f, 0.f}, o_col[3] = {0.f, 0.f, 0.f}, o_sc[3] = {0.f, 0.f, 0.f};
    float o_rot[4] = {0.f, 0.f, 0.f, 0.f}, o_cov[6] = {0.f, 0.f, 0.f, 0.f, 0.f, 0.f}, o_opac = 0.f, o_siso = 0.f;
    if (in && !live && a.g.dL_dsh) for (int k = 0; k < a.M * 3; ++k) a.g.dL_dsh[(size_t)idx * a.M * 3 + k] = 0.f;
    if (live) {
        float pv[3];
#pragma unroll
        for (int k = 0; k < 3; ++k) pv[k] = dot3p(c.V[k], c.V[4 + k], c.V[8 + k], c.V[12 + k], x, y, z);
        if (!COV) cov3d_from_scale_rot(s, q, a.mod, cov, Mm);
        Proj p;
        project_cov(c, pv, cov, p);

        const float det_q = p.cxx * p.cyy - p.cxy * p.cxy;
        const float det_inv_q = 1.f / det_q;
        const float qa = p.cyy * det_inv_q, qb = -p.cxy * det_inv_q, qc = p.cxx * det_inv_q;
        const float gA = -0.5f * opq * ga[G_SXX], gBh = 0.5f * (-opq * ga[G_SXY]), gC = -0.5f * opq * ga[G_SYY];
        const float n00 = gA * qa + gBh * qb, n01 = gA * qb + gBh * qc;
        const float n10 = gBh * qa + gC * qb, n11 = gBh * qb + gC * qc;
        const float m00 = -(qa * n00 + qb * n10);
        const float m01 = -(qa * n01 + qb * n11);
        const float m11 = -(qb * n01 + qc * n11);

        float A0[3], A1[3];
#pragma unroll
        for (int j = 0; j < 3; ++j) {
            A0[j] = m00 * p.T0[j] + m01 * p.T1[j];
            A1[j] = m01 * p.T0[j] + m11 * p.T1[j];
        }
        float Gs[3][3];
#pragma unroll
        for (int i = 0; i < 3; ++i)
#pragma unroll
            for (int j = 0; j < 3; ++j) Gs[i][j] = p.T0[i] * A0[j] + p.T1[i] * A1[j];
        const float S[3][3] = {{cov[0], cov[1], cov[2]}, {cov[1], cov[3], cov[4]}, {cov[2], cov[4], cov[5]}};
        float dT0[3], dT1[3];
#pragma unroll
        for (int j = 0; j < 3; ++j) {
            dT0[j] = 2.f * ((A0[0] * S[0][j] + A0[1] * S[1][j]) + A0[2] * S[2][j]);
            dT1[j] = 2.f * ((A1[0] * S[0][j] + A1[1] * S[1][j]) + A1[2] * S[2][j]);
        }
        const float dJ00 = (dT0[0] * c.V[0] + dT0[1] * c.V[4]) + dT0[2] * c.V[8];
        const float dJ02 = (dT0[0] * c.V[2] + dT0[1] * c.V[6]) + dT0[2] * c.V[10];
        const float dJ11 = (dT1[0] * c.V[1] + dT1[1] * c.V[5]) + dT1[2] * c.V[9];
        const float dJ12 = (dT1[0] * c.V[2] + dT1[1] * c.V[6]) + dT1[2] * c.V[10];
        float dRv[3][3];
#pragma unroll
        for (int j = 0; j < 3; ++j) {
            dRv[0][j] = p.J00 * dT0[j];
            dRv[1][j] = p.J11 * dT1[j];
            dRv[2][j] = p.J02 * dT0[j] + p.J12 * dT1[j];
        }
        const float tz = p.tz, itz = 1.f / tz, itz2 = itz * itz, itz3 = itz2 * itz;
        float gpc[3];
        gpc[0] = p.clamp_x ? 0.f : -c.focal_x * itz2 * dJ02;
        gpc[1] = p.clamp_y ? 0.f : -c.focal_y * itz2 * dJ12;
        gpc[2] = -c.focal_x * itz2 * dJ00 - c.focal_y * itz2 * dJ11 + 2.f * c.focal_x * p.tx * itz3 * dJ02 +
                 2.f * c.focal_y * p.ty * itz3 * dJ12;

        const float gpx = -opq * (qa * ga[G_SX] + qb * ga[G_SY]);
        const float gpy = -opq * (qc * ga[G_SY] + qb * ga[G_SX]);
        const float gnx = gpx * 0.5f * (float)a.W, gny = gpy * 0.5f * (float)a.H;
        o_m2[0] = gnx; o_m2[1] = gny;
        float ph[4];
#pragma unroll
        for (int k = 0; k < 4; ++k) ph[k] = dot3p(c.PM[k], c.PM[4 + k], c.PM[8 + k], c.PM[12 + k], x, y, z);
        const float p_w = 1.0f / (ph[3] + 0.0000001f);
        const float dph[4] = {gnx * p_w, gny * p_w, 0.f, -(gnx * ph[0] + gny * ph[1]) * p_w * p_w};
#pragma unroll
        for (int j = 0; j < 3; ++j)
            gpc[j] += ((dph[0] * c.PR[4 * j] + dph[1] * c.PR[4 * j + 1]) + dph[2] * c.PR[4 * j + 2]) +
                      dph[3] * c.PR[4 * j + 3];
        gpc[2] += ga[G_DDEPTH];

        float gmean_w[3] = {0.f, 0.f, 0.f};
        if (!SH) {
            if (a.g.dL_dcolors) { o_col[0] = ga[G_DR]; o_col[1] = ga[G_DG]; o_col[2] = ga[G_DB]; }
        } else {
            float gc[3] = {ga[G_DR], ga[G_DG], ga[G_DB]};
#pragma unroll
            for (int ch = 0; ch < 3; ++ch) if (a.clamped[4 * idx + ch]) gc[ch] = 0.f;
            float dv[3] = {x - c.campos[0], y - c.campos[1], z - c.campos[2]};
            const float len2 = (dv[0] * dv[0] + dv[1] * dv[1]) + dv[2] * dv[2];
            const float len = sqrtf(len2), ilen = 1.f / len;
            const float dx = dv[0] * ilen, dy = dv[1] * ilen, dz = dv[2] * ilen;
            const float* sh = a.g.shs + (size_t)idx * a.M * 3;
            float* dsh = a.g.dL_dsh ? a.g.dL_dsh + (size_t)idx * a.M * 3 : nullptr;
// ... 212 lines not shown
```

monogs_amd/csrc/radix_sort.hip:

```cpp
#include "common.h"

namespace mgs {

#ifdef RS_TRACE
__device__ uint64_t* g_rs_trace = nullptr;
#define RS_STAMP(k) do { if (g_rs_trace && threadIdx.x == 0) g_rs_trace[(size_t)blockIdx.x * 8 + (k)] = wall_clock64(); } while (0)
#define RS_DRAIN() asm volatile("s_waitcnt vmcnt(0) lgkmcnt(0)" ::: "memory")
__device__ uint64_t* g_rs_htrace = nullptr;
#define RS_HSTAMP(k) do { if (g_rs_htrace && threadIdx.x == 0) g_rs_htrace[(size_t)blockIdx.x * 4 + (k)] = wall_clock64(); } while (0)
#else
#define RS_HSTAMP(k)
#define RS_STAMP(k)
#define RS_DRAIN()
#endif

constexpr int RS_THREADS = 256;
constexpr int RS_WAVES = RS_THREADS / WAVE;
constexpr int RS_ITEMS = 16;
constexpr int RS_ITEMS_WIDE = 12;
constexpr int RS_ITEMS_MID = 8;
constexpr int RS_ITEMS_SMALL = 4;
constexpr uint64_t RS_ONE_SWEEP_MAX = 512ull * 1024;
static inline int rs_items(uint64_t n) {
    return n <= 192ull * 1024 ? RS_ITEMS_SMALL : (n <= RS_ONE_SWEEP_MAX ? RS_ITEMS_MID : RS_ITEMS);
}
constexpr int RS_MAX_RADIX = 512;
constexpr int RS_MAX_PASSES = 4;
constexpr uint64_t RS_FLAG_LOCAL = 1ull << 62;
constexpr uint64_t RS_FLAG_GLOBAL = 2ull << 62;
constexpr uint64_t RS_COUNT_MASK = (1ull << 62) - 1;
constexpr uint32_t RS_SPIN_LIMIT = 1u << 22;
__device__ uint32_t g_rs_spin_limit = RS_SPIN_LIMIT;
constexpr uint32_t RS_GROUP = 16;

constexpr uint32_t RS_DEPTH_SUB = DEPTH_KEY_SUB;
constexpr uint32_t RS_DEPTH_NARROW = DEPTH_KEY_NARROW;
__device__ __forceinline__ uint32_t rs_xf(uint32_t k, uint32_t sub) { return k == 0xFFFFFFFFu ? k : k - sub; }

int g_opt_radix_scanned = -1;
int g_opt_radix_ballot_rank = 0;
int g_opt_radix_xcd_band = 1;
constexpr uint64_t RS_SCANNED_MIN = 64ull * 1024;
static inline bool rs_scanned(uint64_t n) {
    if (g_opt_radix_scanned >= 0) return g_opt_radix_scanned == 1 && n > RS_SCANNED_MIN;
    return n > RS_ONE_SWEEP_MAX;
}

int binning_path(int P, int W, int H) {
    if (P <= 0) return 0;
    const bool large = g_opt_radix_scanned >= 0 ? g_opt_radix_scanned == 1 : (uint64_t)P > RS_ONE_SWEEP_MAX;
    const int tb = tile_bits(W, H);
    if (!large || tb > 16) return 0;
    return (uint64_t)P <= (1ull << (32 - tile_depth_lo_bits(tb))) ? 1 : 0;
}
static inline int rs_tile_items(uint64_t n, bool scanned) {
    if (!scanned) return rs_items(n);
    return n > 1024ull * RS_THREADS * RS_ITEMS ? RS_ITEMS_WIDE : RS_ITEMS;
}
static inline uint32_t rs_tiles(uint64_t n, bool scanned) {
    const uint64_t tile = (uint64_t)RS_THREADS * rs_tile_items(n, scanned);
    return (uint32_t)((n + tile - 1) / tile);
}
static inline uint32_t rs_tiles(uint64_t n) { return rs_tiles(n, rs_scanned(n)); }

struct RsPlan {
    int npasses;
    int shift[RS_MAX_PASSES];
    int db[RS_MAX_PASSES];
    int radix;
    uint32_t sub;
    bool depth;
};
static inline RsPlan rs_plan_plain(int bits) {
    RsPlan pl;
    pl.npasses = (bits + 7) / 8;
    for (int p = 0; p < RS_MAX_PASSES; ++p) { pl.shift[p] = 8 * p; pl.db[p] = 8; }
    pl.radix = 256; pl.sub = 0u; pl.depth = false;
    return pl;
}
static inline RsPlan rs_plan_depth() {
    RsPlan pl;
    pl.npasses = 4;
    for (int p = 0; p < 3; ++p) { pl.shift[p] = 9 * p; pl.db[p] = 9; }
    pl.shift[3] = 27; pl.db[3] = 8;
    pl.radix = 512; pl.sub = RS_DEPTH_SUB; pl.depth = true;
    return pl;
}

static inline RsPlan rs_plan_for_depth(uint64_t n) { return rs_scanned(n) ? rs_plan_depth() : rs_plan_plain(32); }

constexpr int RS_FAN_LOG = 2;
constexpr int RS_TOP_BATCH = 8;
constexpr int RS_MAX_LEVELS = 6;
struct RsTree {
    int levels;
    uint32_t rows[RS_MAX_LEVELS];
    uint32_t off[RS_MAX_LEVELS];
    uint32_t sum_rows;
};
static inline RsTree rs_tree(uint32_t tiles) {
    RsTree tr;
    tr.levels = 1; tr.rows[0] = tiles; tr.off[0] = 0; tr.sum_rows = 0;
    while (tr.rows[tr.levels - 1] > (uint32_t)RS_TOP_BATCH && tr.levels < RS_MAX_LEVELS) {
        tr.rows[tr.levels] = (tr.rows[tr.levels - 1] + (1u << RS_FAN_LOG) - 1u) >> RS_FAN_LOG;
        tr.off[tr.levels] = tr.sum_rows;
        tr.sum_rows += tr.rows[tr.levels];
        ++tr.levels;
    }
    return tr;
}

static inline size_t rs_status_rows(uint32_t tiles) { return (size_t)tiles + (tiles + RS_GROUP - 1) / RS_GROUP; }
struct RsTemp {
    uint32_t* hist;
    uint32_t* tickets;
    uint32_t* error;
    uint32_t* wide;
    uint64_t* status;
    uint32_t* sums;
    uint32_t* counts;
    size_t zero_bytes;
    size_t bytes;
};
static RsTemp rs_carve(void* temp, uint64_t n, const RsPlan& pl, bool scanned) {
    char* p = (char*)align_up((size_t)temp, 256);
    RsTemp t;
    t.hist = (uint32_t*)p;
    t.tickets = t.hist + RS_MAX_PASSES * pl.radix;
    t.error = t.tickets + RS_MAX_PASSES;
    t.wide = t.error + RS_MAX_PASSES;
    char* q = (char*)align_up((size_t)(t.wide + 1), 256);
    t.status = (uint64_t*)q;
    t.sums = (uint32_t*)q;
    const uint32_t tiles = rs_tiles(n, scanned);
    if (scanned) {
        const size_t sums_bytes = (size_t)pl.npasses * rs_tree(tiles).sum_rows * pl.radix * sizeof(uint32_t);
        t.counts = (uint32_t*)(q + sums_bytes);
        t.zero_bytes = (size_t)(q - p) + sums_bytes;
        t.bytes = t.zero_bytes + (size_t)tiles * pl.radix * sizeof(uint32_t);
    } else {
        t.counts = nullptr;
        t.zero_bytes = (size_t)(q - p) + (size_t)pl.npasses * rs_status_rows(tiles) * pl.radix * sizeof(uint64_t);
        t.bytes = t.zero_bytes;
    }
    return t;
}
static size_t rs_temp_bytes(uint64_t n, const RsPlan& pl) {
    if (n == 0) return 256;
    const size_t a = rs_carve(nullptr, n, pl, false).bytes;
    const size_t b = n > RS_SCANNED_MIN ? rs_carve(nullptr, n, pl, true).bytes : 0;
    return (a > b ? a : b) + 512;
}
size_t radix_temp_bytes(uint64_t n, int bits) { return rs_temp_bytes(n, rs_plan_plain(bits)); }
size_t radix_depth_temp_bytes(uint64_t n) {
    const size_t a = rs_temp_bytes(n, rs_plan_depth()), b = rs_temp_bytes(n, rs_plan_plain(32));
    return a > b ? a : b;
}


struct RsHistArgs {
    int npasses, radix;
    int shift[RS_MAX_PASSES], mask[RS_MAX_PASSES];
    uint32_t sub;
    uint32_t* wide;
};
__global__ void __launch_bounds__(RS_THREADS) rs_hist_kernel(const uint32_t* __restrict__ keys, uint32_t n,
                                                             const uint32_t* __restrict__ n_dev, RsHistArgs h,
                                                             uint32_t* __restrict__ hist) {
    __shared__ uint32_t lh[RS_WAVES][RS_MAX_PASSES * RS_MAX_RADIX];
    if (n_dev) n = min(n, n_dev[0]);
    const int words = h.npasses * h.radix;
    for (int w = 0; w < RS_WAVES; ++w)
        for (int i = threadIdx.x; i < words; i += RS_THREADS) lh[w][i] = 0;
    __syncthreads();
    const int wv = threadIdx.x >> 6;
    bool far = false;
    for (uint32_t i = blockIdx.x * RS_THREADS + threadIdx.x; i < n; i += gridDim.x * RS_THREADS) {
        const uint32_t k = keys[i], x = rs_xf(k, h.sub);
        far |= k != 0xFFFFFFFFu && x >= RS_DEPTH_NARROW;
        for (int p = 0; p < h.npasses; ++p) atomicAdd(&lh[wv][p * h.radix + ((x >> h.shift[p]) & h.mask[p])], 1u);
    }
    if (h.wide && far) atomicOr(h.wide, 1u);
    __syncthreads();
    for (int i = threadIdx.x; i < words; i += RS_THREADS) {
        uint32_t c = 0;
#pragma unroll
        for (int w = 0; w < RS_WAVES; ++w) c += lh[w][i];
        if (c) atomicAdd(hist + i, c);
    }
}

struct RsTreeArgs {
    int levels;
    uint32_t off[RS_MAX_LEVELS];
    uint32_t top_rows;
};
struct RsTileHistArgs {
    const uint32_t* keys;
    uint32_t n;
    const uint32_t* n_dev;
    int shift;
    uint32_t sub;
    uint32_t tiles;
    RsTreeArgs tr;
    uint32_t* counts;
    uint32_t* sums;
    uint32_t* wide;
    int detect;
    int only_if_wide;
};
template <int ITEMS, int TPW, int DB>
__global__ void __launch_bounds__(RS_THREADS * TPW) rs_tile_hist_kernel(RsTileHistArgs a) {
    static_assert(TPW == 1 || TPW == (1 << RS_FAN_LOG), "a workgroup counts one tile or one level-1 node");
    constexpr int RADIX = 1 << DB, DPT = RADIX / RS_THREADS, COPIES = 16 / DPT;
    constexpr uint32_t TILE_PAIRS = RS_THREADS * ITEMS;
    __shared__ uint32_t wh[TPW][COPIES][RADIX];
    const int t = threadIdx.x & (RS_THREADS - 1), q = threadIdx.x >> 8, wv = t >> 6, lane = t & 63;
    if (a.only_if_wide && a.wide[0] == 0u) return;
    RS_HSTAMP(0);
    const uint32_t n_live = a.n_dev ? min(a.n, a.n_dev[0]) : a.n;
    if (a.tr.levels > 1 && (uint64_t)blockIdx.x * TPW * TILE_PAIRS >= n_live) return;
    const uint32_t tile = blockIdx.x * TPW + q, tile_start = tile * TILE_PAIRS;
    const uint32_t tile_n = tile_start < n_live ? min(TILE_PAIRS, n_live - tile_start) : 0u;
    uint32_t k[ITEMS];
#pragma unroll
    for (int i = 0; i < ITEMS; ++i) {
        const uint32_t e = (uint32_t)i * RS_THREADS + t;
        k[i] = e < tile_n ? a.keys[tile_start + e] : 0xFFFFFFFFu;
    }
#pragma unroll
    for (int i = 0; i < COPIES; ++i)
#pragma unroll
        for (int j = 0; j < DPT; ++j) wh[q][i][t * DPT + j] = 0;
    __syncthreads();
    RS_DRAIN();
    RS_HSTAMP(1);
    uint32_t* mine = wh[q][wv * (COPIES / RS_WAVES) + (lane & (COPIES / RS_WAVES - 1))];
    bool far = false;
#pragma unroll
    for (int i = 0; i < ITEMS; ++i) {
        const uint32_t x = rs_xf(k[i], a.sub);
        far |= k[i] != 0xFFFFFFFFu && x >= RS_DEPTH_NARROW;
        if ((uint32_t)i * RS_THREADS + t < tile_n) atomicAdd(&mine[(x >> a.shift) & (RADIX - 1)], 1u);
    }
    if (a.detect && far) atomicOr(a.wide, 1u);
    __syncthreads();
    RS_HSTAMP(2);
    uint32_t c[DPT];
#pragma unroll
    for (int j = 0; j < DPT; ++j) {
        c[j] = 0;
#pragma unroll
        for (int i = 0; i < COPIES; ++i) c[j] += wh[q][i][t * DPT + j];
        if (tile < a.tiles) a.counts[(size_t)tile * RADIX + t * DPT + j] = c[j];
    }
    if (TPW == 1) {
#pragma unroll
        for (int j = 0; j < DPT; ++j)
            if (c[j])
                for (int l = 1; l < a.tr.levels; ++l)
                    atomicAdd(a.sums + ((size_t)a.tr.off[l] + (tile >> (RS_FAN_LOG * l))) * RADIX + t * DPT + j, c[j]);
    } else if (a.tr.levels > 1) {
        __syncthreads();
#pragma unroll
        for (int j = 0; j < DPT; ++j) wh[q][0][t * DPT + j] = c[j];
        __syncthreads();
        if (q == 0) {
#pragma unroll
            for (int j = 0; j < DPT; ++j) {
                uint32_t s1 = 0;
#pragma unroll
                for (int m = 0; m < TPW; ++m) s1 += wh[m][0][t * DPT + j];
                a.sums[((size_t)a.tr.off[1] + blockIdx.x) * RADIX + t * DPT + j] = s1;
                if (s1)
                    for (int l = 2; l < a.tr.levels; ++l)
                        atomicAdd(a.sums + ((size_t)a.tr.off[l] + (blockIdx.x >> (RS_FAN_LOG * (l - 1)))) * RADIX + t * DPT + j, s1);
            }
        }
    }
    RS_DRAIN();
    RS_HSTAMP(3);
}
template <int ITEMS, int DB>
static void rs_launch_tile_hist(const RsTileHistArgs& a, hipStream_t s) {
    if (a.tiles >= 1024u)
        hipLaunchKernelGGL((rs_tile_hist_kernel<ITEMS, 4, DB>), dim3((a.tiles + 3) / 4), dim3(RS_THREADS * 4), 0, s, a);
    else
        hipLaunchKernelGGL((rs_tile_hist_kernel<ITEMS, 1, DB>), dim3(a.tiles), dim3(RS_THREADS), 0, s, a);
}

struct RsPassArgs {
    const uint32_t* kin;
    const uint32_t* vin;
    const uint32_t* pin;
    uint32_t* kout;
    uint32_t* vout;
    uint32_t* pout;
    uint32_t* vfinal;
    uint32_t* kfinal;
    const uint2* aux_in;
    uint2* aux_out;
    int aux_skip_ones;
    uint32_t n;
    const uint32_t* n_dev;
    int shift;
    uint32_t sub;
    const uint32_t* hist;
    uint64_t* status;
    uint32_t tiles;
    uint32_t* ticket;
    uint32_t* error;
    int pass;
    int xcd_band;
    int last;
    int range_shift;
    int cond;
    const uint32_t* wide;
    uint2* ranges;
    const uint32_t* counts;
    const uint32_t* sums;
    RsTreeArgs tree;
};

template <int ITEMS>
__device__ __forceinline__ void rs_exchange(uint32_t* __restrict__ sbuf, const uint32_t (&slot)[ITEMS], uint32_t (&x)[ITEMS], int t) {
#pragma unroll
    for (int i = 0; i < ITEMS; ++i)
        if (slot[i] != 0xFFFFFFFFu) sbuf[slot[i]] = x[i];
    __syncthreads();
#pragma unroll
    for (int i = 0; i < ITEMS; ++i) x[i] = sbuf[min((uint32_t)i * RS_THREADS + (uint32_t)t, (uint32_t)(RS_THREADS * ITEMS - 1))];
}

template <int DPT>
__device__ __forceinline__ void rs_digit_bases(const uint32_t (&hcount)[DPT], uint32_t (&gdigit_base)[DPT], uint32_t* wsum, int lane, int wv) {
    uint32_t hsum = 0;
#pragma unroll
    for (int j = 0; j < DPT; ++j) hsum += hcount[j];
    const uint32_t hincl = wave_incl_scan_dpp(hsum);
    __syncthreads();
    if (lane == 63) wsum[wv] = hincl;
    __syncthreads();
    uint32_t hadd = 0;
    for (int w = 0; w < wv; ++w) hadd += wsum[w];
    uint32_t run = hadd + hincl - hsum;
#pragma unroll
    for (int j = 0; j < DPT; ++j) { gdigit_base[j] = run; run += hcount[j]; }
}

__device__ __forceinline__ bool rs_gather(const uint64_t* row, size_t stride, uint32_t cnt, uint32_t& pre, uint32_t& spins,
                                          uint32_t* err) {
    constexpr uint32_t G = RS_GROUP;
    for (uint32_t r0 = 0; r0 < cnt; r0 += G) {
        uint64_t w[G];
        bool ready;
        do {
#pragma unroll
            for (uint32_t q = 0; q < G; ++q) {
                const uint32_t r = r0 + q;
                w[q] = r < cnt ? __hip_atomic_load(row + (size_t)r * stride, __ATOMIC_RELAXED, __HIP_MEMORY_SCOPE_AGENT)
                                              : RS_FLAG_GLOBAL;
            }
            ready = true;
#pragma unroll
            for (uint32_t q = 0; q < G; ++q) ready &= (w[q] >> 62) != 0ull;
            if (!ready) {
                if (++spins > g_rs_spin_limit) { atomicExch(err, 1u); return false; }
                __builtin_amdgcn_s_sleep(1);
            }
        } while (!ready);
#pragma unroll
        for (uint32_t q = 0; q < G; ++q) pre += (uint32_t)(w[q] & RS_COUNT_MASK);
    }
    return true;
}

template <int ITEMS, int DB, bool SCANNED, bool PAYLOAD, bool BALLOT, bool VIDX>
__global__ void __launch_bounds__(RS_THREADS, (SCANNED && ITEMS == RS_ITEMS_WIDE && DB == 8 && !PAYLOAD) ? 7 : 1) rs_pass_kernel(RsPassArgs a) {
    constexpr int TILE_PAIRS = RS_THREADS * ITEMS;
    constexpr int RADIX = 1 << DB, DPT = RADIX / RS_THREADS;
    constexpr int SBUF = (SCANNED && 2 * RS_WAVES * RADIX > TILE_PAIRS) ? 2 * RS_WAVES * RADIX : TILE_PAIRS;
    __shared__ uint32_t wave_hist[RS_WAVES][RADIX];
    __shared__ uint32_t digit_base[RADIX];
    __shared__ uint32_t gbase[RADIX];
    __shared__ uint32_t sbuf[SBUF];
    __shared__ uint32_t wsum[RS_WAVES];
    __shared__ uint32_t s_tile;

    const int t = threadIdx.x, lane = t & 63, wv = t >> 6;
    const bool wide = a.wide ? a.wide[0] != 0u : false;
    if (a.cond == 2 && !wide) return;
    RS_STAMP(0);
    const bool final_pass = a.cond == 0 ? a.last != 0 : (a.cond == 1 ? !wide : true);
    if (!SCANNED) {
        uint32_t failed = 0;
        for (int q = 0; q < a.pass; ++q) failed |= a.error[q];
        if (failed) return;
    }
    const uint32_t n_live = a.n_dev ? min(a.n, a.n_dev[0]) : a.n;
    if (t == 0) {
        uint32_t id = blockIdx.x;
        if (a.xcd_band) {
            const uint32_t live = (n_live + (uint32_t)TILE_PAIRS - 1) / (uint32_t)TILE_PAIRS;
            const uint32_t q = live >> 3, r = live & 7u, x = id & 7u, j = id >> 3;
            id = j < q + (x < r ? 1u : 0u) ? x * q + min(x, r) + j : 0xFFFFFFFFu;
        }
        s_tile = (!SCANNED && a.ticket) ? atomicAdd(a.ticket, 1u) : id;
    }
#pragma unroll
    for (int w = 0; w < RS_WAVES; ++w)
#pragma unroll
        for (int j = 0; j < DPT; ++j) wave_hist[w][t * DPT + j] = 0;
    __syncthreads();
    const uint32_t tile = s_tile;
    if (tile == 0xFFFFFFFFu) return;
    const uint32_t tile_start = tile * (uint32_t)TILE_PAIRS;
    if (tile_start >= n_live) return;
    const uint32_t tile_n = min((uint32_t)TILE_PAIRS, n_live - tile_start);

    uint32_t hcount[DPT], before[DPT];
#pragma unroll
    for (int j = 0; j < DPT; ++j) hcount[j] = before[j] = 0;
    constexpr int R4 = RADIX / 4;
    uint4 lv[RS_MAX_LEVELS - 1][DPT], tv[RS_TOP_BATCH / RS_WAVES][DPT];
    uint32_t lw[RS_MAX_LEVELS - 1], tw[RS_TOP_BATCH / RS_WAVES], tb[RS_TOP_BATCH / RS_WAVES];
    const int levels = a.tree.levels;
    const uint32_t top_node = tile >> (RS_FAN_LOG * (levels - 1));
    const uint4* __restrict__ c4 = reinterpret_cast<const uint4*>(a.counts);
    const uint4* __restrict__ top4 = levels == 1 ? c4 : reinterpret_cast<const uint4*>(a.sums) + (size_t)a.tree.off[levels - 1] * R4;
    if (SCANNED) {
#pragma unroll
        for (int l = 0; l < RS_MAX_LEVELS - 1; ++l) {
            const bool have = l < levels - 1;
            const uint32_t node = tile >> (RS_FAN_LOG * l), first = node & ~3u, nb = node & 3u;
            const uint4* base = (l == 0 || !have) ? c4 : reinterpret_cast<const uint4*>(a.sums) + (size_t)a.tree.off[l] * R4;
            lw[l] = (have && (uint32_t)wv < nb) ? 1u : 0u;
#pragma unroll
            for (int j = 0; j < DPT; ++j) lv[l][j] = base[(size_t)(lw[l] ? first + (uint32_t)wv : 0u) * R4 + j * WAVE + lane];
        }
#pragma unroll
        for (int q = 0; q < RS_TOP_BATCH / RS_WAVES; ++q) {
            const uint32_t r = (uint32_t)wv + 4u * q;
            tw[q] = r < a.tree.top_rows ? 1u : 0u;
            tb[q] = r < top_node ? 1u : 0u;
#pragma unroll
            for (int j = 0; j < DPT; ++j) tv[q][j] = top4[(size_t)(tw[q] ? r : 0u) * R4 + j * WAVE + lane];
        }
    } else {
#pragma unroll
        for (int j = 0; j < DPT; ++j) hcount[j] = a.hist[t * DPT + j];
    }

    uint32_t key[ITEMS], val[ITEMS], rank[ITEMS], pay[PAYLOAD ? ITEMS : 1];
#pragma unroll
    for (int i = 0; i < ITEMS; ++i) {
        const uint32_t e = (uint32_t)wv * (ITEMS * WAVE) + (uint32_t)i * WAVE + lane;
        const bool valid = e < tile_n;
        key[i] = valid ? a.kin[tile_start + e] : 0xFFFFFFFFu;
        if constexpr (VIDX) val[i] = tile_start + e;
        else val[i] = valid ? a.vin[tile_start + e] : 0u;
        if constexpr (PAYLOAD) pay[i] = valid ? a.pin[tile_start + e] : 0u;
    }
    if (SCANNED) {
        uint4* part = reinterpret_cast<uint4*>(sbuf);
#pragma unroll
        for (int j = 0; j < DPT; ++j) {
            uint4 ab = make_uint4(0u, 0u, 0u, 0u), at = make_uint4(0u, 0u, 0u, 0u);
#pragma unroll
            for (int l = 0; l < RS_MAX_LEVELS - 1; ++l) {
                ab.x += lw[l] ? lv[l][j].x : 0u; ab.y += lw[l] ? lv[l][j].y : 0u; ab.z += lw[l] ? lv[l][j].z : 0u; ab.w += lw[l] ? lv[l][j].w : 0u;
            }
#pragma unroll
            for (int q = 0; q < RS_TOP_BATCH / RS_WAVES; ++q) {
                at.x += tw[q] ? tv[q][j].x : 0u; at.y += tw[q] ? tv[q][j].y : 0u; at.z += tw[q] ? tv[q][j].z : 0u; at.w += tw[q] ? tv[q][j].w : 0u;
                ab.x += tb[q] ? tv[q][j].x : 0u; ab.y += tb[q] ? tv[q][j].y : 0u; ab.z += tb[q] ? tv[q][j].z : 0u; ab.w += tb[q] ? tv[q][j].w : 0u;
            }
            for (uint32_t r0 = RS_TOP_BATCH; r0 < a.tree.top_rows; r0 += RS_TOP_BATCH)
#pragma unroll
                for (int q = 0; q < RS_TOP_BATCH / RS_WAVES; ++q) {
                    const uint32_t r = r0 + (uint32_t)wv + 4u * q;
                    if (r < a.tree.top_rows) {
                        const uint4 v = top4[(size_t)r * R4 + j * WAVE + lane];
                        at.x += v.x; at.y += v.y; at.z += v.z; at.w += v.w;
                        if (r < top_node) { ab.x += v.x; ab.y += v.y; ab.z += v.z; ab.w += v.w; }
                    }
                }
            part[(wv * 2 + 0) * R4 + j * WAVE + lane] = ab;
            part[(wv * 2 + 1) * R4 + j * WAVE + lane] = at;
        }
    }
    RS_DRAIN();
    RS_STAMP(1);
    if (!BALLOT) {
#pragma unroll
        for (int i = 0; i < ITEMS; ++i) {
            const uint32_t e = (uint32_t)wv * (ITEMS * WAVE) + (uint32_t)i * WAVE + lane;
            const uint32_t d = (rs_xf(key[i], a.sub) >> a.shift) & (RADIX - 1);
            rank[i] = 0;
            if (e < tile_n) rank[i] = __hip_atomic_fetch_add(&wave_hist[wv][d], 1u, __ATOMIC_RELAXED, __HIP_MEMORY_SCOPE_WORKGROUP);
        }
    } else {
        const unsigned long long lt_mask = (1ull << lane) - 1ull;
#pragma unroll
        for (int i = 0; i < ITEMS; ++i) {
            const uint32_t e = (uint32_t)wv * (ITEMS * WAVE) + (uint32_t)i * WAVE + lane;
            const bool valid = e < tile_n;
            const uint32_t d = (rs_xf(key[i], a.sub) >> a.shift) & (RADIX - 1);
            unsigned long long peers = __builtin_amdgcn_ballot_w64(valid);
#pragma unroll
            for (int b = 0; b < DB; ++b) {
                const bool bit = (d >> b) & 1u;
                const unsigned long long bm = __builtin_amdgcn_ballot_w64(valid && bit);
                peers &= bit ? bm : ~bm;
            }
            rank[i] = 0;
            if (valid) {
                const uint32_t prev = wave_hist[wv][d];
                rank[i] = prev + (uint32_t)__popcll(peers & lt_mask);
                if ((peers & lt_mask) == 0ull) wave_hist[wv][d] = prev + (uint32_t)__popcll(peers);
            }
        }
    }
    __syncthreads();
    if (SCANNED) {
#pragma unroll
        for (int j = 0; j < DPT; ++j)
#pragma unroll
            for (int w = 0; w < RS_WAVES; ++w) {
                before[j] += sbuf[(w * 2 + 0) * RADIX + t * DPT + j];
                hcount[j] += sbuf[(w * 2 + 1) * RADIX + t * DPT + j];
            }
    }
    RS_STAMP(2);

    uint32_t total[DPT], tsum = 0;
#pragma unroll
    for (int j = 0; j < DPT; ++j) {
        uint32_t run = 0;
#pragma unroll
        for (int w = 0; w < RS_WAVES; ++w) {
            const uint32_t c = wave_hist[w][t * DPT + j];
            wave_hist[w][t * DPT + j] = run;
            run += c;
        }
        total[j] = run;
        tsum += run;
    }
    const uint32_t incl = wave_incl_scan_dpp(tsum);
    if (lane == 63) wsum[wv] = incl;
    __syncthreads();
    uint32_t wadd = 0;
    for (int w = 0; w < wv; ++w) wadd += wsum[w];
    uint32_t dbase[DPT];
    {
        uint32_t run = wadd + incl - tsum;
#pragma unroll
        for (int j = 0; j < DPT; ++j) { dbase[j] = run; digit_base[t * DPT + j] = run; run += total[j]; }
    }
    uint32_t gdigit_base[DPT];
    if constexpr (SCANNED) {
        rs_digit_bases<DPT>(hcount, gdigit_base, wsum, lane, wv);
#pragma unroll
        for (int j = 0; j < DPT; ++j) gbase[t * DPT + j] = gdigit_base[j] + before[j] - dbase[j];
        __syncthreads();
    } else {
        static_assert(DPT == 1, "the one-sweep path ranks 256 digits");
        constexpr uint32_t G = RS_GROUP;
        const uint32_t live_tiles = (n_live + (uint32_t)TILE_PAIRS - 1) / (uint32_t)TILE_PAIRS;
        const uint32_t grp = tile / G, jin = tile % G;
        const uint32_t members = min(G, live_tiles - grp * G);
        uint64_t* gstat = a.status + (size_t)a.tiles * RADIX;
        rs_digit_bases<DPT>(hcount, gdigit_base, wsum, lane, wv);
        __hip_atomic_store(a.status + (size_t)tile * RADIX + t, RS_FLAG_LOCAL | (uint64_t)total[0], __ATOMIC_RELAXED,
                           __HIP_MEMORY_SCOPE_AGENT);
        uint32_t spins = 0, pre = 0, gpre = 0;
        bool ok = rs_gather(a.status + (size_t)grp * G * RADIX + t, RADIX, jin, pre, spins, a.error + a.pass);
        if (jin == members - 1)
            __hip_atomic_store(gstat + (size_t)grp * RADIX + t, RS_FLAG_GLOBAL | (uint64_t)(pre + total[0]), __ATOMIC_RELAXED,
                               __HIP_MEMORY_SCOPE_AGENT);
        if (ok) ok = rs_gather(gstat + t, RADIX, grp, gpre, spins, a.error + a.pass);
        gbase[t] = gdigit_base[0] + gpre + pre - dbase[0];
        __syncthreads();
    }

    RS_STAMP(3);
#pragma unroll
    for (int i = 0; i < ITEMS; ++i) {
        const uint32_t e = (uint32_t)wv * (ITEMS * WAVE) + (uint32_t)i * WAVE + lane;
        const uint32_t d = (rs_xf(key[i], a.sub) >> a.shift) & (RADIX - 1);
        rank[i] = e < tile_n ? digit_base[d] + wave_hist[wv][d] + rank[i] : 0xFFFFFFFFu;
    }
    rs_exchange<ITEMS>(sbuf, rank, key, t);
    __syncthreads();
    rs_exchange<ITEMS>(sbuf, rank, val, t);
    if constexpr (PAYLOAD) {
        __syncthreads();
        rs_exchange<ITEMS>(sbuf, rank, pay, t);
    }
    RS_STAMP(4);
    uint32_t g[ITEMS];
    bool live[ITEMS];
#pragma unroll
    for (int i = 0; i < ITEMS; ++i) {
        const uint32_t p = (uint32_t)i * RS_THREADS + t;
        live[i] = p < tile_n;
        g[i] = gbase[(rs_xf(key[i], a.sub) >> a.shift) & (RADIX - 1)] + p;
    }
    if (!final_pass) {
#pragma unroll
        for (int i = 0; i < ITEMS; ++i)
            if (live[i]) {
                a.kout[g[i]] = key[i];
                a.vout[g[i]] = val[i];
                if constexpr (PAYLOAD) a.pout[g[i]] = pay[i];
            }
        RS_STAMP(5); RS_DRAIN(); RS_STAMP(6); RS_STAMP(7);
        return;
    }
#pragma unroll
    for (int i = 0; i < ITEMS; ++i)
        if (live[i]) {
            if (a.kfinal) a.kfinal[g[i]] = key[i];
            a.vfinal[g[i]] = val[i];
        }
    if (a.ranges) {
        __shared__ uint32_t s_edge[RS_WAVES * ITEMS];
        if (lane == 63) {
#pragma unroll
            for (int i = 0; i < ITEMS; ++i) s_edge[wv * ITEMS + i] = key[i];
        }
        __syncthreads();
#pragma unroll
        for (int i = 0; i < ITEMS; ++i) {
            const uint32_t p = (uint32_t)i * RS_THREADS + t;
            uint32_t l = (uint32_t)__shfl_up((int)key[i], 1, 64);
            if (lane == 0) l = wv > 0 ? s_edge[(wv - 1) * ITEMS + i] : (i > 0 ? s_edge[(RS_WAVES - 1) * ITEMS + i - 1] : 0xFFFFFFFFu);
            const uint32_t kr = key[i] >> a.range_shift, lr = l >> a.range_shift;
            if (p < tile_n && (p == 0 || lr != kr)) {
                atomicMin(&a.ranges[kr].x, g[i]);
                if (p > 0)
                    atomicMax(&a.ranges[lr].y, gbase[(rs_xf(l, a.sub) >> a.shift) & (RADIX - 1)] + p);
            }
            if (p + 1 == tile_n) atomicMax(&a.ranges[kr].y, g[i] + 1u);
        }
    }
    RS_STAMP(5);
    RS_DRAIN();
    RS_STAMP(6);
    if (a.aux_out) {
        uint2* __restrict__ aout = a.aux_out;
        if constexpr (PAYLOAD) {
#pragma unroll
            for (int i = 0; i < ITEMS; ++i)
                if (live[i]) {
                    const uint32_t r = pay[i];
                    aout[g[i]] = key[i] == 0xFFFFFFFFu ? make_uint2(0u, 0u)
                                                       : make_uint2((r & 0xFFu) | ((r & 0xFF00u) << 8), ((r >> 16) & 0xFFu) | ((r >> 24) << 16));
                }
        } else {
            const uint2* __restrict__ ain = a.aux_in;
            uint2 r[ITEMS];
#pragma unroll
            for (int i = 0; i < ITEMS; ++i)
                r[i] = (live[i] && !(a.aux_skip_ones && key[i] == 0xFFFFFFFFu)) ? ain[val[i]] : make_uint2(0u, 0u);
#pragma unroll
            for (int i = 0; i < ITEMS; ++i)
                if (live[i]) aout[g[i]] = r[i];
        }
    }
    RS_DRAIN();
    RS_STAMP(7);
}


bool radix_result_in_b(int bits) { return (rs_plan_plain(bits).npasses & 1) != 0; }

const uint32_t* radix_error_flag(void* temp, uint64_t n, int bits) {
    return rs_carve(temp, n ? n : 1, rs_plan_plain(bits), rs_scanned(n ? n : 1)).error;
}
const uint32_t* radix_depth_error_flag(void* temp, uint64_t n) {
    return rs_carve(temp, n ? n : 1, rs_plan_for_depth(n ? n : 1), rs_scanned(n ? n : 1)).error;
}

void radix_zero_region(void* temp, uint64_t n, int bits, uint32_t** ptr, size_t* words) {
    const RsTemp t = rs_carve(temp, n ? n : 1, rs_plan_plain(bits), rs_scanned(n ? n : 1));
    *ptr = t.hist;
    *words = t.zero_bytes / 4;
}
void radix_depth_zero_region(void* temp, uint64_t n, uint32_t** ptr, size_t* words, bool header_only) {
    const RsTemp t = rs_carve(temp, n ? n : 1, rs_plan_for_depth(n ? n : 1), rs_scanned(n ? n : 1));
    *ptr = t.hist;
    *words = header_only ? (size_t)((char*)t.status - (char*)t.hist) / 4 : t.zero_bytes / 4;
}

bool radix_wants_hist(uint64_t n) { return n > 0 && !rs_scanned(n); }
bool radix_depth_payload(uint64_t n) { return n > 0 && rs_scanned(n); }

template <int ITEMS, int DB, bool SCANNED, bool PAYLOAD>
static void rs_launch_pass(const RsPassArgs& a, uint32_t tiles, bool ballot, hipStream_t s) {
    if (ballot && DB == 8 && !PAYLOAD && a.vin != nullptr)
        hipLaunchKernelGGL((rs_pass_kernel<ITEMS, 8, SCANNED, false, true, false>), dim3(tiles), dim3(RS_THREADS), 0, s, a);
    else if (a.vin == nullptr && (DB == 9 || !SCANNED))
        hipLaunchKernelGGL((rs_pass_kernel<ITEMS, DB, SCANNED, PAYLOAD, false, (DB == 9 || !SCANNED)>), dim3(tiles), dim3(RS_THREADS), 0, s, a);
    else
        hipLaunchKernelGGL((rs_pass_kernel<ITEMS, DB, SCANNED, PAYLOAD, false, false>), dim3(tiles), dim3(RS_THREADS), 0, s, a);
}
template <int DB, bool PAYLOAD>
static void rs_launch_pass_items(const RsPassArgs& a, int items, bool scanned, uint32_t tiles, bool ballot, hipStream_t s) {
    if (scanned) {
        if (items == RS_ITEMS_WIDE) rs_launch_pass<RS_ITEMS_WIDE, DB, true, PAYLOAD>(a, tiles, ballot, s);
        else rs_launch_pass<RS_ITEMS, DB, true, PAYLOAD>(a, tiles, ballot, s);
    } else if constexpr (!PAYLOAD && DB == 8) {
        if (items == RS_ITEMS_SMALL) rs_launch_pass<RS_ITEMS_SMALL, 8, false, false>(a, tiles, ballot, s);
        else if (items == RS_ITEMS_MID) rs_launch_pass<RS_ITEMS_MID, 8, false, false>(a, tiles, ballot, s);
        else rs_launch_pass<RS_ITEMS, 8, false, false>(a, tiles, ballot, s);
    }
}

struct RsBuffers {
    uint2* ranges;
    uint32_t *ka, *va, *pa;
    bool va_is_index;
    uint32_t *kb, *vb, *pb;
    uint32_t *kfinal, *vfinal;
    const uint2* aux_in;
    uint2* aux_out;
    bool aux_skip_ones;
};
static int rs_run(const RsPlan& pl, const RsBuffers& b, uint64_t n, void* temp, hipStream_t s, const uint32_t* n_dev,
                  bool temp_zeroed, const uint32_t* ext_hist, bool exclusive, int key_shift = 0) {
    if (n == 0) return 0;
    if (n >= (1ull << 32)) { set_error("radix sort: more than 2^32-1 pairs"); return 1; }
    const bool scanned = rs_scanned(n);
    const RsTemp t = rs_carve(temp, n, pl, scanned);
    if (!temp_zeroed) MGS_HIP(zero_fill(t.hist, t.zero_bytes, s));
    const uint32_t tiles = rs_tiles(n, scanned);
    const int items = rs_tile_items(n, scanned);
    const bool payload = b.pa != nullptr;
    if (payload && !scanned) { set_error("radix sort: payloads need the counted-tiles path"); return 1; }
    const RsTree tree = rs_tree(tiles);
    RsTreeArgs ta;
    ta.levels = tree.levels;
    for (int l = 0; l < RS_MAX_LEVELS; ++l) ta.off[l] = l < tree.levels ? tree.off[l] : 0u;
    ta.top_rows = tree.rows[tree.levels - 1];
    if (!scanned && !ext_hist) {
        RsHistArgs h;
        h.npasses = pl.npasses; h.radix = pl.radix; h.sub = pl.sub; h.wide = pl.depth ? t.wide : nullptr;
        for (int p = 0; p < RS_MAX_PASSES; ++p) { h.shift[p] = pl.shift[p]; h.mask[p] = (1 << pl.db[p]) - 1; }
        hipLaunchKernelGGL(rs_hist_kernel, dim3(min(tiles, 1024u)), dim3(RS_THREADS), 0, s, b.ka, (uint32_t)n, n_dev, h, t.hist);
    }
    const uint32_t* ghist = (!scanned && ext_hist) ? ext_hist : t.hist;
    const int hstride = (!scanned && ext_hist) ? 256 : pl.radix;
    const uint32_t *kin = b.ka, *vin = b.va_is_index ? nullptr : b.va, *pin = b.pa;
    uint32_t *kout = b.kb, *vout = b.vb, *pout = b.pb;
    uint32_t *kalt = b.ka, *valt = b.va, *palt = b.pa;
    for (int p = 0; p < pl.npasses; ++p) {
        RsPassArgs a;
        a.kin = kin; a.vin = vin; a.pin = pin; a.kout = kout; a.vout = vout; a.pout = pout;
        a.n = (uint32_t)n; a.n_dev = n_dev; a.shift = pl.shift[p]; a.sub = pl.sub;
        a.hist = ghist + p * hstride;
        a.status = t.status + (size_t)p * rs_status_rows(tiles) * pl.radix;
        a.tiles = tiles;
        a.ticket = (exclusive && tiles <= 256u) ? nullptr : t.tickets + p;
        a.error = t.error;
        a.pass = p;
        a.xcd_band = (scanned && g_opt_radix_xcd_band != 0) ? 1 : 0;
        a.counts = t.counts; a.sums = t.sums + (size_t)p * tree.sum_rows * pl.radix;
        a.tree = ta;
        a.wide = pl.depth ? t.wide : nullptr;
        a.cond = pl.depth ? (p == 2 ? 1 : (p == 3 ? 2 : 0)) : 0;
        a.last = (!pl.depth && p == pl.npasses - 1) ? 1 : 0;
        a.vfinal = b.vfinal ? b.vfinal : vout;
        a.kfinal = b.vfinal ? b.kfinal : kout;
        a.ranges = (!pl.depth && p == pl.npasses - 1) ? b.ranges : nullptr;
        a.range_shift = key_shift;
        if (a.ranges && key_shift == 0) a.kfinal = nullptr;
        a.aux_in = b.aux_in; a.aux_out = b.aux_out; a.aux_skip_ones = b.aux_skip_ones ? 1 : 0;
        if (scanned) {
            RsTileHistArgs h;
            h.keys = kin; h.n = (uint32_t)n; h.n_dev = n_dev; h.shift = a.shift; h.sub = pl.sub; h.tiles = tiles; h.tr = ta;
            h.counts = t.counts; h.sums = const_cast<uint32_t*>(a.sums);
            h.wide = t.wide; h.detect = (pl.depth && p == 0) ? 1 : 0; h.only_if_wide = a.cond == 2 ? 1 : 0;
            if (items == RS_ITEMS_WIDE) {
                if (pl.db[p] == 9) rs_launch_tile_hist<RS_ITEMS_WIDE, 9>(h, s); else rs_launch_tile_hist<RS_ITEMS_WIDE, 8>(h, s);
            } else {
                if (pl.db[p] == 9) rs_launch_tile_hist<RS_ITEMS, 9>(h, s); else rs_launch_tile_hist<RS_ITEMS, 8>(h, s);
            }
        }
        const bool ballot = g_opt_radix_ballot_rank != 0;
        if (pl.db[p] == 9) {
            if (payload) rs_launch_pass_items<9, true>(a, items, scanned, tiles, ballot, s);
            else rs_launch_pass_items<9, false>(a, items, scanned, tiles, ballot, s);
        } else {
            if (payload) rs_launch_pass_items<8, true>(a, items, scanned, tiles, ballot, s);
            else rs_launch_pass_items<8, false>(a, items, scanned, tiles, ballot, s);
        }
        kin = kout; vin = vout; pin = pout;
        uint32_t* tk = kalt; kalt = kout; kout = tk;
        uint32_t* tv = valt; valt = vout; vout = tv;
        uint32_t* tp = palt; palt = pout; pout = tp;
    }
    MGS_HIP(hipGetLastError());
    return 0;
}

int radix_sort_pairs(uint32_t* ka, uint32_t* va, uint32_t* kb, uint32_t* vb, uint64_t n, int bits, void* temp,
                     hipStream_t s, const uint32_t* n_dev, bool temp_zeroed, const uint2* aux_in, uint2* aux_out,
                     const uint32_t* ext_hist, bool aux_empty_for_ones, bool exclusive, uint2* ranges, int key_shift) {
    RsPlan pl = rs_plan_plain(bits);
    for (int p = 0; p < RS_MAX_PASSES; ++p) pl.shift[p] += key_shift;
    if (pl.npasses > RS_MAX_PASSES) { set_error("radix sort: more than 32 key bits"); return 1; }
    RsBuffers b;
    b.ranges = ranges;
    b.ka = ka; b.va = va; b.va_is_index = false; b.pa = nullptr; b.kb = kb; b.vb = vb; b.pb = nullptr; b.kfinal = nullptr; b.vfinal = nullptr;
    b.aux_in = aux_in; b.aux_out = aux_out; b.aux_skip_ones = aux_empty_for_ones;
    return rs_run(pl, b, n, temp, s, n_dev, temp_zeroed, ext_hist, exclusive, key_shift);
}

int radix_sort_depth(uint32_t* keys, uint32_t* key_b, uint32_t* val_a, uint32_t* val_b, void* rect, bool payload,
                     uint32_t* perm, uint2* rect_sorted, uint64_t n, void* temp, hipStream_t s, bool temp_zeroed, bool exclusive) {
    const RsPlan pl = rs_plan_for_depth(n);
    RsBuffers b;
    b.ranges = nullptr;
    b.ka = keys; b.va = val_a; b.va_is_index = true; b.kb = key_b; b.vb = val_b;
    b.pa = payload ? (uint32_t*)rect : nullptr; b.pb = payload ? (uint32_t*)rect + n : nullptr;
    b.kfinal = nullptr; b.vfinal = perm;
    b.aux_in = payload ? nullptr : (const uint2*)rect; b.aux_out = rect_sorted; b.aux_skip_ones = true;
    return rs_run(pl, b, n, temp, s, nullptr, temp_zeroed, nullptr, exclusive);
}

int set_radix_spin_limit(uint32_t limit) {
    const uint32_t v = limit == 0xFFFFFFFFu ? RS_SPIN_LIMIT : limit;
    MGS_HIP(hipMemcpyToSymbol(HIP_SYMBOL(g_rs_spin_limit), &v, sizeof(v)));
    return 0;
}

}
```

monogs_amd/csrc/tile_sort.h:

```cpp
#pragma once
#include "common.h"

namespace mgs {

constexpr int TDS_THREADS = 256, TDS_WAVES = TDS_THREADS / WAVE, TDS_ITEMS = 4, TDS_CAP = TDS_THREADS * TDS_ITEMS;
constexpr int TDS_DB = 9, TDS_RADIX = 1 << TDS_DB, TDS_DPT = TDS_RADIX / TDS_THREADS;

struct TdsLds {
    uint32_t* k;
    uint32_t* v;
    uint32_t (*cnt)[TDS_RADIX];
    uint32_t* wsum;
    uint32_t* red;
};

__device__ __forceinline__ void tds_minmax(uint32_t lo, uint32_t hi, uint32_t* s_red , uint32_t& mn,
                                           uint32_t& mx) {
    const int lane = threadIdx.x & 63, wv = threadIdx.x >> 6;
#pragma unroll
    for (int o = 32; o > 0; o >>= 1) {
        lo = min(lo, (uint32_t)__shfl_xor((int)lo, o, 64));
        hi = max(hi, (uint32_t)__shfl_xor((int)hi, o, 64));
    }
    if (lane == 0) { s_red[wv] = lo; s_red[TDS_WAVES + wv] = hi; }
    __syncthreads();
    mn = s_red[0]; mx = s_red[TDS_WAVES];
#pragma unroll
    for (int w = 1; w < TDS_WAVES; ++w) { mn = min(mn, s_red[w]); mx = max(mx, s_red[TDS_WAVES + w]); }
    __syncthreads();
}

__device__ __forceinline__ void tds_lds_sort(uint32_t* s_k, uint32_t* s_v, uint32_t (*s_cnt)[TDS_RADIX], uint32_t* s_wsum,
                                             int base, int m, int bits) {
    const int t = threadIdx.x, lane = t & 63, wv = t >> 6;
    for (int sh = 0; sh < bits; sh += TDS_DB) {
#pragma unroll
        for (int w = 0; w < TDS_WAVES; ++w)
#pragma unroll
            for (int j = 0; j < TDS_DPT; ++j) s_cnt[w][t * TDS_DPT + j] = 0u;
        __syncthreads();
        uint32_t k[TDS_ITEMS], v[TDS_ITEMS], r[TDS_ITEMS];
#pragma unroll
        for (int i = 0; i < TDS_ITEMS; ++i) {
            const int e = wv * (TDS_ITEMS * WAVE) + i * WAVE + lane;
            k[i] = 0u; v[i] = 0u; r[i] = 0u;
            if (e < m) {
                k[i] = s_k[base + e]; v[i] = s_v[base + e];
                r[i] = __hip_atomic_fetch_add(&s_cnt[wv][(k[i] >> sh) & (TDS_RADIX - 1)], 1u, __ATOMIC_RELAXED,
                                              __HIP_MEMORY_SCOPE_WORKGROUP);
            }
        }
        __syncthreads();
        uint32_t c[TDS_DPT][TDS_WAVES], tot[TDS_DPT], tsum = 0;
#pragma unroll
        for (int j = 0; j < TDS_DPT; ++j) {
            tot[j] = 0u;
#pragma unroll
            for (int w = 0; w < TDS_WAVES; ++w) { c[j][w] = s_cnt[w][t * TDS_DPT + j]; tot[j] += c[j][w]; }
            tsum += tot[j];
        }
        const uint32_t incl = wave_incl_scan_dpp(tsum);
        if (lane == 63) s_wsum[wv] = incl;
        __syncthreads();
        uint32_t run = incl - tsum;
        for (int w = 0; w < wv; ++w) run += s_wsum[w];
#pragma unroll
        for (int j = 0; j < TDS_DPT; ++j)
#pragma unroll
            for (int w = 0; w < TDS_WAVES; ++w) { s_cnt[w][t * TDS_DPT + j] = run; run += c[j][w]; }
        __syncthreads();
#pragma unroll
        for (int i = 0; i < TDS_ITEMS; ++i) {
            const int e = wv * (TDS_ITEMS * WAVE) + i * WAVE + lane;
            if (e < m) {
                const uint32_t dst = s_cnt[wv][(k[i] >> sh) & (TDS_RADIX - 1)] + r[i];
                s_k[base + dst] = k[i]; s_v[base + dst] = v[i];
            }
        }
        __syncthreads();
    }
    __syncthreads();
}

__device__ inline void tds_global_sort(uint32_t* __restrict__ kx, uint32_t* __restrict__ vx, uint32_t* __restrict__ ky,
                                       uint32_t* __restrict__ vy, uint32_t n, const uint32_t* __restrict__ depth_key, int lo,
                                       uint32_t (*s_cnt)[TDS_RADIX], uint32_t* s_run, uint32_t* s_wsum) {
    const int t = threadIdx.x, lane = t & 63, wv = t >> 6;
    const uint32_t imask = lo ? (1u << (32 - lo)) - 1u : 0xFFFFFFFFu;
    for (uint32_t e = t; e < n; e += TDS_THREADS) {
        const uint32_t g = vx[e] & imask;
        kx[e] = depth_key[g] - DEPTH_KEY_SUB;
        vx[e] = g;
    }
    for (int sh = 0; sh < 32; sh += 8) {
        __threadfence();
        if (t < 256) s_run[t] = 0u;
#pragma unroll
        for (int w = 0; w < TDS_WAVES; ++w) s_cnt[w][t] = 0u;
        __syncthreads();
        for (uint32_t e = t; e < n; e += TDS_THREADS) atomicAdd(&s_run[(kx[e] >> sh) & 255u], 1u);
        __syncthreads();
        {
            const uint32_t c = s_run[t], incl = wave_incl_scan_dpp(c);
            if (lane == 63) s_wsum[wv] = incl;
            __syncthreads();
            uint32_t b0 = incl - c;
            for (int w = 0; w < wv; ++w) b0 += s_wsum[w];
            s_run[t] = b0;
        }
        __syncthreads();
        for (uint32_t c0 = 0; c0 < n; c0 += TDS_THREADS) {
            const uint32_t e = c0 + (uint32_t)t;
            uint32_t k = 0u, v = 0u, r = 0u, d = 0u;
            if (e < n) {
                k = kx[e]; v = vx[e]; d = (k >> sh) & 255u;
                r = __hip_atomic_fetch_add(&s_cnt[wv][d], 1u, __ATOMIC_RELAXED, __HIP_MEMORY_SCOPE_WORKGROUP);
            }
            __syncthreads();
            uint32_t pre[TDS_WAVES];
            {
                uint32_t run = s_run[t];
#pragma unroll
                for (int w = 0; w < TDS_WAVES; ++w) { const uint32_t c = s_cnt[w][t]; pre[w] = run; run += c; }
                s_run[t] = run;
            }
            __syncthreads();
#pragma unroll
            for (int w = 0; w < TDS_WAVES; ++w) s_cnt[w][t] = pre[w];
            __syncthreads();
            if (e < n) { const uint32_t dst = s_cnt[wv][d] + r; ky[dst] = k; vy[dst] = v; }
            __syncthreads();
#pragma unroll
            for (int w = 0; w < TDS_WAVES; ++w) s_cnt[w][t] = 0u;
            __syncthreads();
        }
        __threadfence();
        __syncthreads();
        uint32_t* tk = kx; kx = ky; ky = tk;
        uint32_t* tv = vx; vx = vy; vy = tv;
    }
}

__device__ __forceinline__ uint32_t tile_depth_sort(const TileSortArgs& ts, uint2 rg, bool skip, const TdsLds& lds) {
    const int t = threadIdx.x, lane = t & 63, wv = t >> 6;
    const uint32_t n_live = ts.n_dev ? min(ts.n_cap, ts.n_dev[0]) : ts.n_cap;
    const uint32_t start = rg.x, end = min(rg.y, n_live);
    if (skip || start >= end) return 0u;
    const uint32_t n = end - start;
    const int lo = tile_depth_lo_bits(ts.tb);
    const uint32_t kmask = ts.tb < 32 ? (0xFFFFFFFFu >> ts.tb) : 0u, imask = lo ? (1u << (32 - lo)) - 1u : 0xFFFFFFFFu;
    if (n > (uint32_t)TDS_CAP) {
        uint32_t* const k = ts.keys + start;
        uint32_t* const v = ts.vals + start;
        tds_global_sort(k, v, ts.keys_alt + start, ts.vals_alt + start, n, ts.depth_key, lo, lds.cnt, lds.k, lds.wsum);
        return 0u;
    }
    uint32_t d[TDS_ITEMS], g[TDS_ITEMS];
    uint32_t dmin = 0xFFFFFFFFu, dmax = 0u;
#pragma unroll
    for (int i = 0; i < TDS_ITEMS; ++i) {
        const uint32_t e = (uint32_t)(wv * (TDS_ITEMS * WAVE) + i * WAVE + lane);
        d[i] = 0u; g[i] = 0u;
        if (e < n) {
            const uint32_t k = ts.keys[start + e], v = ts.vals[start + e];
            d[i] = ((k & kmask) << lo) | (lo ? v >> (32 - lo) : 0u);
            g[i] = v & imask;
            dmin = min(dmin, d[i]); dmax = max(dmax, d[i]);
        }
    }
    uint32_t mn, mx;
    tds_minmax(dmin, dmax, lds.red, mn, mx);
#pragma unroll
    for (int i = 0; i < TDS_ITEMS; ++i) {
        const int e = wv * (TDS_ITEMS * WAVE) + i * WAVE + lane;
        if (e < (int)n) { lds.k[e] = d[i] - mn; lds.v[e] = g[i]; }
    }
    const uint32_t span = mx - mn;
    tds_lds_sort(lds.k, lds.v, lds.cnt, lds.wsum, 0, (int)n, span ? 32 - __builtin_clz(span) : 0);
    if (mx == DEPTH_KEY_NARROW) {
        uint32_t c = 0;
#pragma unroll
        for (int i = 0; i < TDS_ITEMS; ++i) {
            const uint32_t e = (uint32_t)(wv * (TDS_ITEMS * WAVE) + i * WAVE + lane);
            c += (e < n && d[i] == DEPTH_KEY_NARROW) ? 1u : 0u;
        }
#pragma unroll
        for (int o = 32; o > 0; o >>= 1) c += (uint32_t)__shfl_xor((int)c, o, 64);
        if (lane == 0) lds.red[wv] = c;
        __syncthreads();
        uint32_t m = 0;
#pragma unroll
        for (int w = 0; w < TDS_WAVES; ++w) m += lds.red[w];
        __syncthreads();
        const uint32_t f = n - m;
        uint32_t xmin = 0xFFFFFFFFu, xmax = 0u;
        for (uint32_t e = f + t; e < n; e += TDS_THREADS) {
            const uint32_t x = ts.depth_key[lds.v[e]] - DEPTH_KEY_SUB;
            lds.k[e] = x;
            xmin = min(xmin, x); xmax = max(xmax, x);
        }
        uint32_t rmn, rmx;
        tds_minmax(xmin, xmax, lds.red, rmn, rmx);
        for (uint32_t e = f + t; e < n; e += TDS_THREADS) lds.k[e] -= rmn;
        __syncthreads();
        const uint32_t rspan = rmx - rmn;
        tds_lds_sort(lds.k, lds.v, lds.cnt, lds.wsum, (int)f, (int)m, rspan ? 32 - __builtin_clz(rspan) : 0);
    }
#pragma unroll
    for (int i = 0; i < TDS_ITEMS; ++i) {
        const int e = wv * (TDS_ITEMS * WAVE) + i * WAVE + lane;
        if (e < (int)n) ts.vals[start + e] = lds.v[e];
    }
    return n;
}

}
```

Baseline: 2968 Mpix/s.

## Fuse per-tile scan into preprocess and drop packed depth bits from tile keys

On the per-tile binning path, preprocess now writes 256-item block-local offsets, and a single-block kernel scans the block totals. This replaces the separate scan_local/scan_blocks launches and the extra pass over rects. Duplicate no longer packs low depth bits into keys and vals. The per-tile sort instead gathers depth_key directly, which removes the narrow-depth fallback re-sort, and radix sort gains a token mode. This trades an extra random gather of depth_key in the tile sort for fewer kernels and less key packing, and it reuses the perm buffer as scratch for the scan totals.

```diff
diff --git a/monogs_amd/csrc/api.hip b/monogs_amd/csrc/api.hip
--- a/monogs_amd/csrc/api.hip
+++ b/monogs_amd/csrc/api.hip
@@ -193,7 +193,9 @@
     const bool per_tile = binning_path(P, cam->image_width, cam->image_height) != 0;
     if (per_tile) {
         tm.mark();
-        if (int rc = launch_scan(g, P, s, exclusive, g.rect)) return rc;
+        if (scan_in_preprocess(P, cam->image_width, cam->image_height)) {
+            if (int rc = launch_scan_totals(g, P, s)) return rc;
+        } else if (int rc = launch_scan(g, P, s, exclusive, g.rect)) return rc;
     } else {
         if (int rc = launch_depth_sort(g, P, depth_sort_payload(P, cam->image_width, cam->image_height), s, exclusive)) return rc;
         tm.mark();
diff --git a/monogs_amd/csrc/binning.hip b/monogs_amd/csrc/binning.hip
--- a/monogs_amd/csrc/binning.hip
+++ b/monogs_amd/csrc/binning.hip
@@ -5,7 +5,6 @@
 namespace mgs {
 
 constexpr int SCAN_THREADS = 256;
-__device__ __forceinline__ int scan_nblocks_dev(int P) { return (P + SCAN_ITEMS - 1) / SCAN_ITEMS; }
 constexpr int SCAN_PER_THREAD = SCAN_ITEMS / SCAN_THREADS;
 
 __device__ __forceinline__ uint32_t wave_incl_scan(uint32_t v, int) { return wave_incl_scan_dpp(v); }
@@ -123,6 +122,60 @@
 int g_opt_scan_small = -1;
 bool scan_is_small(int P) { return g_opt_scan_small != 0 && scan_nblocks(P) <= SCAN_SMALL_MAX_BLOCKS; }
 
+constexpr int ST_THREADS = 1024, ST_PER_THREAD = 8, ST_WAVES = ST_THREADS / WAVE;
+__global__ void __launch_bounds__(ST_THREADS) scan_totals_kernel(uint32_t* totals, int nb, uint32_t* __restrict__ total_out) {
+    __shared__ uint32_t s_w[ST_WAVES];
+    const int lane = threadIdx.x & 63, wv = threadIdx.x >> 6;
+    uint32_t carry = 0;
+    for (int start = 0; start < nb; start += ST_THREADS * ST_PER_THREAD) {
+        const int i0 = start + (int)threadIdx.x * ST_PER_THREAD;
+        const bool full = i0 + ST_PER_THREAD <= nb;
+        uint32_t v[ST_PER_THREAD];
+        if (full) {
+            const uint4 a = *reinterpret_cast<const uint4*>(totals + i0), b = *reinterpret_cast<const uint4*>(totals + i0 + 4);
+            v[0] = a.x; v[1] = a.y; v[2] = a.z; v[3] = a.w; v[4] = b.x; v[5] = b.y; v[6] = b.z; v[7] = b.w;
+        } else {
+#pragma unroll
+            for (int k = 0; k < ST_PER_THREAD; ++k) v[k] = i0 + k < nb ? totals[i0 + k] : 0u;
+        }
+        uint32_t sum = 0;
+#pragma unroll
+        for (int k = 0; k < ST_PER_THREAD; ++k) sum += v[k];
+        const uint32_t incl = wave_incl_scan_dpp(sum);
+        if (lane == 63) s_w[wv] = incl;
+        __syncthreads();
+        uint32_t wbase = 0, trip = 0;
+#pragma unroll
+        for (int w = 0; w < ST_WAVES; ++w) {
+            const uint32_t t = s_w[w];
+            wbase += w < wv ? t : 0u;
+            trip += t;
+        }
+        __syncthreads();
+        uint32_t run = carry + wbase + (incl - sum);
+        uint32_t e[ST_PER_THREAD];
+#pragma unroll
+        for (int k = 0; k < ST_PER_THREAD; ++k) { e[k] = run; run += v[k]; }
+        if (full) {
+            *reinterpret_cast<uint4*>(totals + i0) = make_uint4(e[0], e[1], e[2], e[3]);
+            *reinterpret_cast<uint4*>(totals + i0 + 4) = make_uint4(e[4], e[5], e[6], e[7]);
+        } else {
+#pragma unroll
+            for (int k = 0; k < ST_PER_THREAD; ++k) if (i0 + k < nb) totals[i0 + k] = e[k];
+        }
+        carry += trip;
+    }
+    if (threadIdx.x == 0) *total_out = carry;
+}
+bool scan_in_preprocess(int P, int W, int H) { return P > 0 && binning_path(P, W, H) == 1 && !scan_is_small(P); }
+int launch_scan_totals(const GeometryState& g, int P, hipStream_t s) {
+    if (P == 0) return 0;
+    hipLaunchKernelGGL(scan_totals_kernel, dim3(1), dim3(ST_THREADS), 0, s, scan_totals_256(g),
+                       (P + PRE_SCAN_ITEMS - 1) / PRE_SCAN_ITEMS, g.scan_blocks + scan_nblocks(P));
+    MGS_HIP(hipGetLastError());
+    return 0;
+}
+
 
 int launch_scan(const GeometryState& g, int P, hipStream_t s, bool exclusive, const uint2* rects) {
     if (P == 0) return 0;
@@ -141,21 +194,13 @@
     return 0;
 }
 
-__device__ __forceinline__ void dup_pair(uint32_t gidx, const uint32_t* __restrict__ depth_key, int lo, uint32_t& val,
-                                         uint32_t& kfield) {
-    val = gidx; kfield = 0u;
-    if (depth_key) {
-        const uint32_t k = depth_key[gidx];
-        const uint32_t d = k == 0xFFFFFFFFu ? DEPTH_KEY_NARROW : min(k - DEPTH_KEY_SUB, DEPTH_KEY_NARROW);
-        kfield = d >> lo;
-        if (lo) val |= (d & ((1u << lo) - 1u)) << (32 - lo);
-    }
-}
 __global__ void __launch_bounds__(256) duplicate_kernel(int P, const uint2* __restrict__ rects,
                                                         const uint32_t* __restrict__ perm,
-                                                        const uint32_t* __restrict__ depth_key, int tshift, int lo,
+                                                        int tshift,
                                                         const uint32_t* __restrict__ offsets ,
                                                         const uint32_t* __restrict__ block_sums ,
+                                                        int granule ,
+                                                        const uint32_t* __restrict__ total ,
                                                         uint32_t* keys,
                                                         uint32_t* vals, int gx, int gy, uint32_t r_cap,
                                                         int32_t* __restrict__ n_touched, uint2* __restrict__ ranges,
@@ -171,10 +216,11 @@
         prepare[0] = 0ull;
     }
     const int lane = threadIdx.x & 63;
+    const int gsh = 31 - __builtin_clz((uint32_t)granule);
     grid_zero(zero_ptr, zero_words, (size_t)n_threads, 256);
     const bool depth_bad = depth_err && radix_failed(depth_err) != 0u;
     if (i == 0 && count) {
-        const uint32_t R = (P > 0 && !depth_bad) ? block_sums[scan_nblocks_dev(P)] : 0u;
+        const uint32_t R = (P > 0 && !depth_bad) ? total[0] : 0u;
         count[0] = min(R, r_cap);
         count[1] = R > r_cap ? 1u : 0u;
     }
@@ -182,19 +228,19 @@
         overflow[0] = (count ? count[1] : 0u) | (depth_bad ? (uint32_t)MGS_STATUS_DEPTH_SORT_TIMEOUT : 0u);
     if (i < ntiles) ranges[i] = make_uint2(0xFFFFFFFFu, 0u);
     if (i < P) n_touched[i] = 0;
-    uint32_t idx = 0, nt = 0, off = 0, kf = 0;
+    uint32_t idx = 0, nt = 0, off = 0;
     int x0 = 0, y0 = 0, x1 = 0;
     if (i < P) {
-        dup_pair(perm ? perm[i] : (uint32_t)i, depth_key, lo, idx, kf);
+        idx = perm ? perm[i] : (uint32_t)i;
         const uint2 r = rects[i];
         const int w = (int)(r.y & 0xFFFFu), h = (int)(r.y >> 16);
         nt = (uint32_t)(w * h);
         x0 = (int)(r.x & 0xFFFFu); y0 = (int)(r.x >> 16); x1 = x0 + w;
     }
     if (depth_bad) nt = 0;
-    if (nt) off = i == 0 ? 0u : offsets[i - 1] + (offsets_global ? 0u : block_sums[(i - 1) / SCAN_ITEMS]);
+    if (nt) off = i == 0 ? 0u : offsets[i - 1] + (offsets_global ? 0u : block_sums[(i - 1) >> gsh]);
     __shared__ uint32_t s_own[4][WAVE];
-    __shared__ uint32_t s_idx[4][WAVE], s_off[4][WAVE], s_kf[4][WAVE];
+    __shared__ uint32_t s_idx[4][WAVE], s_off[4][WAVE];
     __shared__ int s_x0[4][WAVE], s_y0[4][WAVE], s_w[4][WAVE];
     __shared__ uint32_t s_hist[2][256];
     if (hist) {
@@ -203,14 +249,14 @@
     }
     const int wv = threadIdx.x >> 6;
     if (slot_major) {
-        const uint32_t R_all = (P > 0 && !depth_bad) ? block_sums[scan_nblocks_dev(P)] : 0u;
+        const uint32_t R_all = (P > 0 && !depth_bad) ? total[0] : 0u;
         const uint32_t R_emit = min(R_all, r_cap);
         const uint32_t n_waves = (uint32_t)n_threads / WAVE;
         const uint32_t CH = (((R_emit + n_waves - 1u) / n_waves) + 63u) & ~63u;
         const uint32_t wave_id = (uint32_t)blockIdx.x * 4u + (uint32_t)wv;
         const uint64_t s0w = (uint64_t)wave_id * CH;
         const uint32_t s0 = s0w < (uint64_t)R_emit ? (uint32_t)s0w : R_emit, s1 = (uint64_t)s0 + CH < (uint64_t)R_emit ? s0 + CH : R_emit;
-        auto incl = [&](uint32_t k) { return offsets[k] + (offsets_global ? 0u : block_sums[k / SCAN_ITEMS]); };
+        auto incl = [&](uint32_t k) { return offsets[k] + (offsets_global ? 0u : block_sums[k >> gsh]); };
         uint32_t g = 0;
         if (s0 < s1) {
             uint32_t lo = 0, hi = (uint32_t)P;
@@ -229,7 +275,7 @@
         while (sl < s1 && g < (uint32_t)P) {
             const uint32_t gi = g + (uint32_t)lane;
             const bool valid = gi < (uint32_t)P;
-            uint32_t inc = 0, ntg = 0, idg = 0, kfg = 0;
+            uint32_t inc = 0, ntg = 0, idg = 0;
             int gx0 = 0, gy0 = 0, gw = 1;
             if (valid) {
                 inc = incl(gi);
@@ -237,14 +283,14 @@
                 gw = (int)(r.y & 0xFFFFu);
                 ntg = (uint32_t)(gw * (int)(r.y >> 16));
                 gx0 = (int)(r.x & 0xFFFFu); gy0 = (int)(r.x >> 16);
-                dup_pair(perm ? perm[gi] : gi, depth_key, lo, idg, kfg);
+                idg = perm ? perm[gi] : gi;
             }
             const uint32_t exc = inc - ntg;
             uint32_t Eg = valid ? inc : 0u;
 #pragma unroll
             for (int o2 = 32; o2 > 0; o2 >>= 1) Eg = max(Eg, (uint32_t)__shfl_xor((int)Eg, o2, 64));
             __builtin_amdgcn_wave_barrier();
-            s_idx[wv][lane] = idg; s_kf[wv][lane] = kfg; s_off[wv][lane] = exc; s_x0[wv][lane] = gx0; s_y0[wv][lane] = gy0; s_w[wv][lane] = max(gw, 1);
+            s_idx[wv][lane] = idg; s_off[wv][lane] = exc; s_x0[wv][lane] = gx0; s_y0[wv][lane] = gy0; s_w[wv][lane] = max(gw, 1);
             const uint32_t e = min(s1, Eg);
             const uint32_t cb0 = sl & ~63u;
             const unsigned long long before = __builtin_amdgcn_ballot_w64(ntg != 0u && exc < cb0);
@@ -269,7 +315,7 @@
                     const uint32_t w = (uint32_t)s_w[wv][L];
                     const uint32_t yy = t / w, xx = t - yy * w;
                     const uint32_t tid = (uint32_t)((s_y0[wv][L] + (int)yy) * gx + s_x0[wv][L] + (int)xx);
-                    const uint32_t key = (tid << tshift) | s_kf[wv][L];
+                    const uint32_t key = tid << tshift;
                     keys[o] = key;
                     vals[o] = s_idx[wv][L];
                     if (hist) {
@@ -295,7 +341,7 @@
         }
         return;
     }
-    s_idx[wv][lane] = idx; s_kf[wv][lane] = kf; s_off[wv][lane] = off; s_x0[wv][lane] = x0; s_y0[wv][lane] = y0; s_w[wv][lane] = max(x1 - x0, 1);
+    s_idx[wv][lane] = idx; s_off[wv][lane] = off; s_x0[wv][lane] = x0; s_y0[wv][lane] = y0; s_w[wv][lane] = max(x1 - x0, 1);
     const unsigned long long live = __builtin_amdgcn_ballot_w64(nt != 0);
     if (live == 0ull && !hist) return;
     const int first = live ? __builtin_ctzll(live) : 0, lastl = live ? 63 - __builtin_clzll(live) : 0;
@@ -322,7 +368,7 @@
             const uint32_t w = (uint32_t)s_w[wv][L];
             const uint32_t yy = t / w, xx = t - yy * w;
             const uint32_t tid = (uint32_t)((s_y0[wv][L] + (int)yy) * gx + s_x0[wv][L] + (int)xx);
-            const uint32_t key = (tid << tshift) | s_kf[wv][L];
+            const uint32_t key = tid << tshift;
             keys[o] = key;
             vals[o] = s_idx[wv][L];
             if (hist) {
@@ -367,10 +413,11 @@
     if (sort_n > 0) radix_zero_region(b.sort_temp, sort_n, sort_bits, &zero_ptr, &zero_words);
     const bool count_digits = P > 0 && sort_bits <= 16 && radix_wants_hist(sort_n);
     const int tb = tile_bits(cam.image_width, cam.image_height);
+    const bool pre_scanned = per_tile && scan_in_preprocess(P, cam.image_width, cam.image_height);
     hipLaunchKernelGGL(duplicate_kernel, dim3(n_threads / 256), dim3(256), 0, s, P, per_tile ? g.rect : g.rect_sorted,
-                       per_tile ? nullptr : g.perm, per_tile ? g.depth_key : nullptr, per_tile ? 32 - tb : 0,
-                       per_tile ? tile_depth_lo_bits(tb) : 0, g.point_offsets,
-                       g.scan_blocks, b.keys_a, b.vals_a, tiles_x(cam.image_width), tiles_y(cam.image_height),
+                       per_tile ? nullptr : g.perm, per_tile ? 32 - tb : 0, g.point_offsets,
+                       pre_scanned ? scan_totals_256(g) : g.scan_blocks, pre_scanned ? PRE_SCAN_ITEMS : SCAN_ITEMS,
+                       g.scan_blocks + scan_nblocks(P), b.keys_a, b.vals_a, tiles_x(cam.image_width), tiles_y(cam.image_height),
                        (uint32_t)(r_cap > 0xFFFFFFFFull ? 0xFFFFFFFFull : r_cap), n_touched, img.ranges, ntiles, zero_ptr,
                        zero_words, count, overflow, depth_err,
                        (P > 0 && scan_is_small(P)) ? 1 : 0,
@@ -392,7 +439,7 @@
     if (R == 0) return 0;
     const bool counted = bits <= 16 && radix_wants_hist(R) && g.tile_hist != nullptr;
     return radix_sort_pairs(b.keys_a, b.vals_a, b.keys_b, b.vals_b, R, bits, b.sort_temp, s, n_dev, true, nullptr, nullptr,
-                            counted ? g.tile_hist : nullptr, false, exclusive, ranges, per_tile ? 32 - bits : 0);
+                            counted ? g.tile_hist : nullptr, false, exclusive, ranges, per_tile ? 32 - bits : 0, per_tile);
 }
 
 TileSortArgs tile_sort_args(const mgs_camera& cam, const GeometryState& g, const BinningState& b, uint64_t R,
@@ -405,7 +452,6 @@
     ts.depth_key = g.depth_key;
     ts.n_dev = n_dev;
     ts.n_cap = (uint32_t)R;
-    ts.tb = tile_bits(cam.image_width, cam.image_height);
     return ts;
 }
 
diff --git a/monogs_amd/csrc/common.h b/monogs_amd/csrc/common.h
--- a/monogs_amd/csrc/common.h
+++ b/monogs_amd/csrc/common.h
@@ -153,7 +153,6 @@
 
 constexpr uint32_t DEPTH_KEY_SUB = 0x3E4CCCCDu;
 constexpr uint32_t DEPTH_KEY_NARROW = (1u << 27) - 1u;
-__host__ __device__ inline int tile_depth_lo_bits(int tb) { return tb > 5 ? tb - 5 : 0; }
 int binning_path(int P, int W, int H);
 
 void set_error(const char* fmt, ...);
@@ -177,6 +176,10 @@
 inline float* backward_tau_part(void* scratch, int P) { return backward_grad_acc(scratch) + (size_t)P * GRAD_FLOATS; }
 inline float* backward_tau_out(void* scratch, int P) { return backward_tau_part(scratch, P) + (size_t)TAU_SLOTS * 16; }
 int launch_scan(const GeometryState& g, int P, hipStream_t s, bool exclusive, const uint2* rects);
+constexpr int PRE_SCAN_ITEMS = 256;
+bool scan_in_preprocess(int P, int W, int H);
+inline uint32_t* scan_totals_256(const GeometryState& g) { return g.perm; }
+int launch_scan_totals(const GeometryState& g, int P, hipStream_t s);
 int launch_duplicate(const mgs_camera& cam, int P, const GeometryState& g, const BinningState& b, uint64_t r_cap,
                      int32_t* n_touched, const ImageState& img, uint64_t sort_n, int sort_bits, uint32_t* count,
                      uint32_t* overflow, hipStream_t s, bool per_tile);
@@ -197,7 +200,8 @@
                      bool aux_empty_for_ones = false,
                      bool exclusive = false,
                      uint2* ranges = nullptr,
-                     int key_shift = 0);
+                     int key_shift = 0,
+                     bool tokens = false);
 bool radix_wants_hist(uint64_t n);
 bool radix_depth_payload(uint64_t n);
 int radix_sort_depth(uint32_t* keys, uint32_t* key_b, uint32_t* val_a, uint32_t* val_b, void* rect, bool payload,
@@ -208,14 +212,13 @@
 int launch_sort(const GeometryState& g, const BinningState& b, uint64_t R, int bits, hipStream_t s,
                 const uint32_t* n_dev = nullptr, bool exclusive = false, uint2* ranges = nullptr, bool per_tile = false);
 struct TileSortArgs {
+    uint32_t* vals;
     uint32_t* keys;
-    uint32_t* vals;
     uint32_t* keys_alt;
     uint32_t* vals_alt;
     const uint32_t* depth_key;
     const uint32_t* n_dev;
     uint32_t n_cap;
-    int tb;
 };
 TileSortArgs tile_sort_args(const mgs_camera& cam, const GeometryState& g, const BinningState& b, uint64_t R,
                             const uint32_t* n_dev);
diff --git a/monogs_amd/csrc/preprocess.hip b/monogs_amd/csrc/preprocess.hip
--- a/monogs_amd/csrc/preprocess.hip
+++ b/monogs_amd/csrc/preprocess.hip
@@ -159,6 +159,8 @@
     size_t zero_words;
     float* grad_acc;
     unsigned long long* prepare;
+    uint32_t* scan_out;
+    uint32_t* scan_totals;
 };
 
 __device__ __forceinline__ void load4(const float* __restrict__ p, bool aligned16, float o[4]) {
@@ -256,15 +258,7 @@
 }
 
 template <bool COV, bool PRECOMP>
-__global__ void __launch_bounds__(256) preprocess_forward_kernel(PreArgs a) {
-    const int idx = blockIdx.x * 256 + threadIdx.x;
-    grid_zero(a.zero_ptr, a.zero_words, (size_t)((a.P + 255) / 256) * 256, 256);
-    if (a.grad_acc && blockIdx.x == 0) {
-        float4* t4 = reinterpret_cast<float4*>(a.grad_acc + (size_t)a.P * GRAD_FLOATS);
-        for (int i = threadIdx.x; i < (TAU_SLOTS + 1) * 4; i += 256) t4[i] = make_float4(0.f, 0.f, 0.f, 0.f);
-    }
-    if (idx == 0) a.prepare[0] = (unsigned long long)(uintptr_t)a.grad_acc;
-    if (idx >= a.P) return;
+__device__ __forceinline__ uint32_t preprocess_gaussian(const PreArgs& a, const int idx, float4 (*s_rec)[WAVE * 5]) {
     Cam c;
     load_cam(c, a.V, a.PM, nullptr, a.campos);
     c.tanfovx = a.tanfovx; c.tanfovy = a.tanfovy; c.focal_x = a.focal_x; c.focal_y = a.focal_y;
@@ -298,7 +292,6 @@
     }
     a.depth_key[idx] = vis ? o.key : 0xFFFFFFFFu;
     {
-        __shared__ float4 s_rec[4][WAVE * 5];
         const int lane = threadIdx.x & 63, wv = threadIdx.x >> 6, wave_first = idx - lane;
         if (wave_first + WAVE <= a.P) {
             const unsigned long long vm = __builtin_amdgcn_ballot_w64(vis);
@@ -315,6 +308,32 @@
             float4* rec = reinterpret_cast<float4*>(a.rec + (size_t)idx * REC_FLOATS);
             rec[0] = o.r0; rec[1] = o.r1; rec[2] = o.r2; rec[3] = o.r3;
         }
+    }
+    return vis ? (o.rect.y & 0xFFFFu) * (o.rect.y >> 16) : 0u;
+}
+
+template <bool COV, bool PRECOMP>
+__global__ void __launch_bounds__(256) preprocess_forward_kernel(PreArgs a) {
+    const int idx = blockIdx.x * 256 + threadIdx.x;
+    grid_zero(a.zero_ptr, a.zero_words, (size_t)((a.P + 255) / 256) * 256, 256);
+    if (a.grad_acc && blockIdx.x == 0) {
+        float4* t4 = reinterpret_cast<float4*>(a.grad_acc + (size_t)a.P * GRAD_FLOATS);
+        for (int i = threadIdx.x; i < (TAU_SLOTS + 1) * 4; i += 256) t4[i] = make_float4(0.f, 0.f, 0.f, 0.f);
+    }
+    if (idx == 0) a.prepare[0] = (unsigned long long)(uintptr_t)a.grad_acc;
+    __shared__ float4 s_rec[4][WAVE * 5];
+    uint32_t nt = 0;
+    if (idx < a.P) nt = preprocess_gaussian<COV, PRECOMP>(a, idx, s_rec);
+    if (a.scan_out) {
+        const int lane = threadIdx.x & 63, wv = threadIdx.x >> 6;
+        const uint32_t incl = wave_incl_scan_dpp(nt);
+        if (lane == 63) reinterpret_cast<uint32_t*>(&s_rec[wv][4])[0] = incl;
+        __syncthreads();
+        const uint32_t t0 = reinterpret_cast<const uint32_t*>(&s_rec[0][4])[0], t1 = reinterpret_cast<const uint32_t*>(&s_rec[1][4])[0];
+        const uint32_t t2 = reinterpret_cast<const uint32_t*>(&s_rec[2][4])[0], t3 = reinterpret_cast<const uint32_t*>(&s_rec[3][4])[0];
+        const uint32_t base = (wv > 0 ? t0 : 0u) + (wv > 1 ? t1 : 0u) + (wv > 2 ? t2 : 0u);
+        if (idx < a.P) a.scan_out[idx] = base + incl;
+        if (threadIdx.x == 0) a.scan_totals[blockIdx.x] = (t0 + t1) + (t2 + t3);
     }
 }
 
@@ -344,6 +363,9 @@
     radix_depth_zero_region(g.sort_temp, (uint64_t)P, &a.zero_ptr, &a.zero_words, per_tile);
     a.zero_words += (size_t)((char*)a.zero_ptr - (char*)g.scan_status) / 4;
     a.zero_ptr = (uint32_t*)g.scan_status;
+    const bool scan_here = scan_in_preprocess(P, cam.image_width, cam.image_height);
+    a.scan_out = scan_here ? g.point_offsets : nullptr;
+    a.scan_totals = scan_here ? scan_totals_256(g) : nullptr;
     const dim3 grid((P + 255) / 256), block(256);
     if (cov3D_precomp && colors_precomp) hipLaunchKernelGGL((preprocess_forward_kernel<true, true>), grid, block, 0, s, a);
     else if (cov3D_precomp) hipLaunchKernelGGL((preprocess_forward_kernel<true, false>), grid, block, 0, s, a);
diff --git a/monogs_amd/csrc/radix_sort.hip b/monogs_amd/csrc/radix_sort.hip
--- a/monogs_amd/csrc/radix_sort.hip
+++ b/monogs_amd/csrc/radix_sort.hip
@@ -51,7 +51,7 @@
     const bool large = g_opt_radix_scanned >= 0 ? g_opt_radix_scanned == 1 : (uint64_t)P > RS_ONE_SWEEP_MAX;
     const int tb = tile_bits(W, H);
     if (!large || tb > 16) return 0;
-    return (uint64_t)P <= (1ull << (32 - tile_depth_lo_bits(tb))) ? 1 : 0;
+    return (uint64_t)P <= (1ull << (tb > 5 ? 37 - tb : 32)) ? 1 : 0;
 }
 static inline int rs_tile_items(uint64_t n, bool scanned) {
     if (!scanned) return rs_items(n);
@@ -321,6 +321,7 @@
     const uint32_t* sums;
     RsTreeArgs tree;
 };
+__device__ __forceinline__ uint32_t* rs_token_starts(uint32_t* error) { return error - RS_MAX_PASSES - 2 * 256; }
 
 template <int ITEMS>
 __device__ __forceinline__ void rs_exchange(uint32_t* __restrict__ sbuf, const uint32_t (&slot)[ITEMS], uint32_t (&x)[ITEMS], int t) {
@@ -377,299 +378,15 @@
 
 template <int ITEMS, int DB, bool SCANNED, bool PAYLOAD, bool BALLOT, bool VIDX>
 __global__ void __launch_bounds__(RS_THREADS, (SCANNED && ITEMS == RS_ITEMS_WIDE && DB == 8 && !PAYLOAD) ? 7 : 1) rs_pass_kernel(RsPassArgs a) {
-    constexpr int TILE_PAIRS = RS_THREADS * ITEMS;
-    constexpr int RADIX = 1 << DB, DPT = RADIX / RS_THREADS;
-    constexpr int SBUF = (SCANNED && 2 * RS_WAVES * RADIX > TILE_PAIRS) ? 2 * RS_WAVES * RADIX : TILE_PAIRS;
-    __shared__ uint32_t wave_hist[RS_WAVES][RADIX];
-    __shared__ uint32_t digit_base[RADIX];
-    __shared__ uint32_t gbase[RADIX];
-    __shared__ uint32_t sbuf[SBUF];
-    __shared__ uint32_t wsum[RS_WAVES];
-    __shared__ uint32_t s_tile;
-
-    const int t = threadIdx.x, lane = t & 63, wv = t >> 6;
-    const bool wide = a.wide ? a.wide[0] != 0u : false;
-    if (a.cond == 2 && !wide) return;
-    RS_STAMP(0);
-    const bool final_pass = a.cond == 0 ? a.last != 0 : (a.cond == 1 ? !wide : true);
-    if (!SCANNED) {
-        uint32_t failed = 0;
-        for (int q = 0; q < a.pass; ++q) failed |= a.error[q];
-        if (failed) return;
-    }
-    const uint32_t n_live = a.n_dev ? min(a.n, a.n_dev[0]) : a.n;
-    if (t == 0) {
-        uint32_t id = blockIdx.x;
-        if (a.xcd_band) {
-            const uint32_t live = (n_live + (uint32_t)TILE_PAIRS - 1) / (uint32_t)TILE_PAIRS;
-            const uint32_t q = live >> 3, r = live & 7u, x = id & 7u, j = id >> 3;
-            id = j < q + (x < r ? 1u : 0u) ? x * q + min(x, r) + j : 0xFFFFFFFFu;
-        }
-        s_tile = (!SCANNED && a.ticket) ? atomicAdd(a.ticket, 1u) : id;
-    }
-#pragma unroll
-    for (int w = 0; w < RS_WAVES; ++w)
-#pragma unroll
-        for (int j = 0; j < DPT; ++j) wave_hist[w][t * DPT + j] = 0;
-    __syncthreads();
-    const uint32_t tile = s_tile;
-    if (tile == 0xFFFFFFFFu) return;
-    const uint32_t tile_start = tile * (uint32_t)TILE_PAIRS;
-    if (tile_start >= n_live) return;
-    const uint32_t tile_n = min((uint32_t)TILE_PAIRS, n_live - tile_start);
-
-    uint32_t hcount[DPT], before[DPT];
-#pragma unroll
-    for (int j = 0; j < DPT; ++j) hcount[j] = before[j] = 0;
-    constexpr int R4 = RADIX / 4;
-    uint4 lv[RS_MAX_LEVELS - 1][DPT], tv[RS_TOP_BATCH / RS_WAVES][DPT];
-    uint32_t lw[RS_MAX_LEVELS - 1], tw[RS_TOP_BATCH / RS_WAVES], tb[RS_TOP_BATCH / RS_WAVES];
-    const int levels = a.tree.levels;
-    const uint32_t top_node = tile >> (RS_FAN_LOG * (levels - 1));
-    const uint4* __restrict__ c4 = reinterpret_cast<const uint4*>(a.counts);
-    const uint4* __restrict__ top4 = levels == 1 ? c4 : reinterpret_cast<const uint4*>(a.sums) + (size_t)a.tree.off[levels - 1] * R4;
-    if (SCANNED) {
-#pragma unroll
-        for (int l = 0; l < RS_MAX_LEVELS - 1; ++l) {
-            const bool have = l < levels - 1;
-            const uint32_t node = tile >> (RS_FAN_LOG * l), first = node & ~3u, nb = node & 3u;
-            const uint4* base = (l == 0 || !have) ? c4 : reinterpret_cast<const uint4*>(a.sums) + (size_t)a.tree.off[l] * R4;
-            lw[l] = (have && (uint32_t)wv < nb) ? 1u : 0u;
-#pragma unroll
-            for (int j = 0; j < DPT; ++j) lv[l][j] = base[(size_t)(lw[l] ? first + (uint32_t)wv : 0u) * R4 + j * WAVE + lane];
-        }
-#pragma unroll
-        for (int q = 0; q < RS_TOP_BATCH / RS_WAVES; ++q) {
-            const uint32_t r = (uint32_t)wv + 4u * q;
-            tw[q] = r < a.tree.top_rows ? 1u : 0u;
-            tb[q] = r < top_node ? 1u : 0u;
-#pragma unroll
-            for (int j = 0; j < DPT; ++j) tv[q][j] = top4[(size_t)(tw[q] ? r : 0u) * R4 + j * WAVE + lane];
-        }
-    } else {
-#pragma unroll
-        for (int j = 0; j < DPT; ++j) hcount[j] = a.hist[t * DPT + j];
-    }
-
-    uint32_t key[ITEMS], val[ITEMS], rank[ITEMS], pay[PAYLOAD ? ITEMS : 1];
-#pragma unroll
-    for (int i = 0; i < ITEMS; ++i) {
-        const uint32_t e = (uint32_t)wv * (ITEMS * WAVE) + (uint32_t)i * WAVE + lane;
-        const bool valid = e < tile_n;
-        key[i] = valid ? a.kin[tile_start + e] : 0xFFFFFFFFu;
-        if constexpr (VIDX) val[i] = tile_start + e;
-        else val[i] = valid ? a.vin[tile_start + e] : 0u;
-        if constexpr (PAYLOAD) pay[i] = valid ? a.pin[tile_start + e] : 0u;
-    }
-    if (SCANNED) {
-        uint4* part = reinterpret_cast<uint4*>(sbuf);
-#pragma unroll
-        for (int j = 0; j < DPT; ++j) {
-            uint4 ab = make_uint4(0u, 0u, 0u, 0u), at = make_uint4(0u, 0u, 0u, 0u);
-#pragma unroll
-            for (int l = 0; l < RS_MAX_LEVELS - 1; ++l) {
-                ab.x += lw[l] ? lv[l][j].x : 0u; ab.y += lw[l] ? lv[l][j].y : 0u; ab.z += lw[l] ? lv[l][j].z : 0u; ab.w += lw[l] ? lv[l][j].w : 0u;
-            }
-#pragma unroll
-            for (int q = 0; q < RS_TOP_BATCH / RS_WAVES; ++q) {
-                at.x += tw[q] ? tv[q][j].x : 0u; at.y += tw[q] ? tv[q][j].y : 0u; at.z += tw[q] ? tv[q][j].z : 0u; at.w += tw[q] ? tv[q][j].w : 0u;
-                ab.x += tb[q] ? tv[q][j].x : 0u; ab.y += tb[q] ? tv[q][j].y : 0u; ab.z += tb[q] ? tv[q][j].z : 0u; ab.w += tb[q] ? tv[q][j].w : 0u;
-            }
-            for (uint32_t r0 = RS_TOP_BATCH; r0 < a.tree.top_rows; r0 += RS_TOP_BATCH)
-#pragma unroll
-                for (int q = 0; q < RS_TOP_BATCH / RS_WAVES; ++q) {
-                    const uint32_t r = r0 + (uint32_t)wv + 4u * q;
-                    if (r < a.tree.top_rows) {
-                        const uint4 v = top4[(size_t)r * R4 + j * WAVE + lane];
-                        at.x += v.x; at.y += v.y; at.z += v.z; at.w += v.w;
-                        if (r < top_node) { ab.x += v.x; ab.y += v.y; ab.z += v.z; ab.w += v.w; }
-                    }
-                }
-            part[(wv * 2 + 0) * R4 + j * WAVE + lane] = ab;
-            part[(wv * 2 + 1) * R4 + j * WAVE + lane] = at;
-        }
-    }
-    RS_DRAIN();
-    RS_STAMP(1);
-    if (!BALLOT) {
-#pragma unroll
-        for (int i = 0; i < ITEMS; ++i) {
-            const uint32_t e = (uint32_t)wv * (ITEMS * WAVE) + (uint32_t)i * WAVE + lane;
-            const uint32_t d = (rs_xf(key[i], a.sub) >> a.shift) & (RADIX - 1);
-            rank[i] = 0;
-            if (e < tile_n) rank[i] = __hip_atomic_fetch_add(&wave_hist[wv][d], 1u, __ATOMIC_RELAXED, __HIP_MEMORY_SCOPE_WORKGROUP);
-        }
-    } else {
-        const unsigned long long lt_mask = (1ull << lane) - 1ull;
-#pragma unroll
-        for (int i = 0; i < ITEMS; ++i) {
-            const uint32_t e = (uint32_t)wv * (ITEMS * WAVE) + (uint32_t)i * WAVE + lane;
-            const bool valid = e < tile_n;
-            const uint32_t d = (rs_xf(key[i], a.sub) >> a.shift) & (RADIX - 1);
-            unsigned long long peers = __builtin_amdgcn_ballot_w64(valid);
-#pragma unroll
-            for (int b = 0; b < DB; ++b) {
-                const bool bit = (d >> b) & 1u;
-                const unsigned long long bm = __builtin_amdgcn_ballot_w64(valid && bit);
-                peers &= bit ? bm : ~bm;
-            }
-            rank[i] = 0;
-            if (valid) {
-                const uint32_t prev = wave_hist[wv][d];
-                rank[i] = prev + (uint32_t)__popcll(peers & lt_mask);
-                if ((peers & lt_mask) == 0ull) wave_hist[wv][d] = prev + (uint32_t)__popcll(peers);
-            }
-        }
-    }
-    __syncthreads();
-    if (SCANNED) {
-#pragma unroll
-        for (int j = 0; j < DPT; ++j)
-#pragma unroll
-            for (int w = 0; w < RS_WAVES; ++w) {
-                before[j] += sbuf[(w * 2 + 0) * RADIX + t * DPT + j];
-                hcount[j] += sbuf[(w * 2 + 1) * RADIX + t * DPT + j];
-            }
-    }
-    RS_STAMP(2);
-
-    uint32_t total[DPT], tsum = 0;
-#pragma unroll
-    for (int j = 0; j < DPT; ++j) {
-        uint32_t run = 0;
-#pragma unroll
-        for (int w = 0; w < RS_WAVES; ++w) {
-            const uint32_t c = wave_hist[w][t * DPT + j];
-            wave_hist[w][t * DPT + j] = run;
-            run += c;
-        }
-        total[j] = run;
-        tsum += run;
-    }
-    const uint32_t incl = wave_incl_scan_dpp(tsum);
-    if (lane == 63) wsum[wv] = incl;
-    __syncthreads();
-    uint32_t wadd = 0;
-    for (int w = 0; w < wv; ++w) wadd += wsum[w];
-    uint32_t dbase[DPT];
-    {
-        uint32_t run = wadd + incl - tsum;
-#pragma unroll
-        for (int j = 0; j < DPT; ++j) { dbase[j] = run; digit_base[t * DPT + j] = run; run += total[j]; }
-    }
-    uint32_t gdigit_base[DPT];
-    if constexpr (SCANNED) {
-        rs_digit_bases<DPT>(hcount, gdigit_base, wsum, lane, wv);
-#pragma unroll
-        for (int j = 0; j < DPT; ++j) gbase[t * DPT + j] = gdigit_base[j] + before[j] - dbase[j];
-        __syncthreads();
-    } else {
-        static_assert(DPT == 1, "the one-sweep path ranks 256 digits");
-        constexpr uint32_t G = RS_GROUP;
-        const uint32_t live_tiles = (n_live + (uint32_t)TILE_PAIRS - 1) / (uint32_t)TILE_PAIRS;
-        const uint32_t grp = tile / G, jin = tile % G;
-        const uint32_t members = min(G, live_tiles - grp * G);
-        uint64_t* gstat = a.status + (size_t)a.tiles * RADIX;
-        rs_digit_bases<DPT>(hcount, gdigit_base, wsum, lane, wv);
-        __hip_atomic_store(a.status + (size_t)tile * RADIX + t, RS_FLAG_LOCAL | (uint64_t)total[0], __ATOMIC_RELAXED,
-                           __HIP_MEMORY_SCOPE_AGENT);
-        uint32_t spins = 0, pre = 0, gpre = 0;
-        bool ok = rs_gather(a.status + (size_t)grp * G * RADIX + t, RADIX, jin, pre, spins, a.error + a.pass);
-        if (jin == members - 1)
-            __hip_atomic_store(gstat + (size_t)grp * RADIX + t, RS_FLAG_GLOBAL | (uint64_t)(pre + total[0]), __ATOMIC_RELAXED,
-                               __HIP_MEMORY_SCOPE_AGENT);
-        if (ok) ok = rs_gather(gstat + t, RADIX, grp, gpre, spins, a.error + a.pass);
-        gbase[t] = gdigit_base[0] + gpre + pre - dbase[0];
-        __syncthreads();
-    }
-
-    RS_STAMP(3);
-#pragma unroll
-    for (int i = 0; i < ITEMS; ++i) {
-        const uint32_t e = (uint32_t)wv * (ITEMS * WAVE) + (uint32_t)i * WAVE + lane;
-        const uint32_t d = (rs_xf(key[i], a.sub) >> a.shift) & (RADIX - 1);
-        rank[i] = e < tile_n ? digit_base[d] + wave_hist[wv][d] + rank[i] : 0xFFFFFFFFu;
-    }
-    rs_exchange<ITEMS>(sbuf, rank, key, t);
-    __syncthreads();
-    rs_exchange<ITEMS>(sbuf, rank, val, t);
-    if constexpr (PAYLOAD) {
-        __syncthreads();
-        rs_exchange<ITEMS>(sbuf, rank, pay, t);
-    }
-    RS_STAMP(4);
-    uint32_t g[ITEMS];
-    bool live[ITEMS];
-#pragma unroll
-    for (int i = 0; i < ITEMS; ++i) {
-        const uint32_t p = (uint32_t)i * RS_THREADS + t;
-        live[i] = p < tile_n;
-        g[i] = gbase[(rs_xf(key[i], a.sub) >> a.shift) & (RADIX - 1)] + p;
-    }
-    if (!final_pass) {
-#pragma unroll
-        for (int i = 0; i < ITEMS; ++i)
-            if (live[i]) {
-                a.kout[g[i]] = key[i];
-                a.vout[g[i]] = val[i];
-                if constexpr (PAYLOAD) a.pout[g[i]] = pay[i];
-            }
-        RS_STAMP(5); RS_DRAIN(); RS_STAMP(6); RS_STAMP(7);
-        return;
-    }
-#pragma unroll
-    for (int i = 0; i < ITEMS; ++i)
-        if (live[i]) {
-            if (a.kfinal) a.kfinal[g[i]] = key[i];
-            a.vfinal[g[i]] = val[i];
-        }
-    if (a.ranges) {
-        __shared__ uint32_t s_edge[RS_WAVES * ITEMS];
-        if (lane == 63) {
-#pragma unroll
-            for (int i = 0; i < ITEMS; ++i) s_edge[wv * ITEMS + i] = key[i];
-        }
-        __syncthreads();
-#pragma unroll
-        for (int i = 0; i < ITEMS; ++i) {
-            const uint32_t p = (uint32_t)i * RS_THREADS + t;
-            uint32_t l = (uint32_t)__shfl_up((int)key[i], 1, 64);
-            if (lane == 0) l = wv > 0 ? s_edge[(wv - 1) * ITEMS + i] : (i > 0 ? s_edge[(RS_WAVES - 1) * ITEMS + i - 1] : 0xFFFFFFFFu);
-            const uint32_t kr = key[i] >> a.range_shift, lr = l >> a.range_shift;
-            if (p < tile_n && (p == 0 || lr != kr)) {
-                atomicMin(&a.ranges[kr].x, g[i]);
-                if (p > 0)
-                    atomicMax(&a.ranges[lr].y, gbase[(rs_xf(l, a.sub) >> a.shift) & (RADIX - 1)] + p);
-            }
-            if (p + 1 == tile_n) atomicMax(&a.ranges[kr].y, g[i] + 1u);
-        }
-    }
-    RS_STAMP(5);
-    RS_DRAIN();
-    RS_STAMP(6);
-    if (a.aux_out) {
-        uint2* __restrict__ aout = a.aux_out;
-        if constexpr (PAYLOAD) {
-#pragma unroll
-            for (int i = 0; i < ITEMS; ++i)
-                if (live[i]) {
-                    const uint32_t r = pay[i];
-                    aout[g[i]] = key[i] == 0xFFFFFFFFu ? make_uint2(0u, 0u)
-                                                       : make_uint2((r & 0xFFu) | ((r & 0xFF00u) << 8), ((r >> 16) & 0xFFu) | ((r >> 24) << 16));
-                }
-        } else {
-            const uint2* __restrict__ ain = a.aux_in;
-            uint2 r[ITEMS];
-#pragma unroll
-            for (int i = 0; i < ITEMS; ++i)
-                r[i] = (live[i] && !(a.aux_skip_ones && key[i] == 0xFFFFFFFFu)) ? ain[val[i]] : make_uint2(0u, 0u);
-#pragma unroll
-            for (int i = 0; i < ITEMS; ++i)
-                if (live[i]) aout[g[i]] = r[i];
-        }
-    }
-    RS_DRAIN();
-    RS_STAMP(7);
+    constexpr int TOK = 0;
+#include "rs_pass_body.inc"
+}
+template <int ITEMS, bool SCANNED, int TOK>
+__global__ void __launch_bounds__(RS_THREADS, (SCANNED && ITEMS == RS_ITEMS_WIDE) ? 7 : 1) rs_token_pass_kernel(RsPassArgs a) {
+    static_assert(TOK == 1 || TOK == 2, "first or second pass");
+    constexpr int DB = 8;
+    constexpr bool PAYLOAD = false, BALLOT = false, VIDX = false;
+#include "rs_pass_body.inc"
 }
 
 
@@ -717,6 +434,22 @@
     }
 }
 
+template <int ITEMS, bool SCANNED>
+static void rs_launch_token_pass(const RsPassArgs& a, uint32_t tiles, int tok, hipStream_t s) {
+    if (tok == 1) hipLaunchKernelGGL((rs_token_pass_kernel<ITEMS, SCANNED, 1>), dim3(tiles), dim3(RS_THREADS), 0, s, a);
+    else hipLaunchKernelGGL((rs_token_pass_kernel<ITEMS, SCANNED, 2>), dim3(tiles), dim3(RS_THREADS), 0, s, a);
+}
+static void rs_launch_token_pass_items(const RsPassArgs& a, int items, bool scanned, uint32_t tiles, int tok, hipStream_t s) {
+    if (scanned) {
+        if (items == RS_ITEMS_WIDE) rs_launch_token_pass<RS_ITEMS_WIDE, true>(a, tiles, tok, s);
+        else rs_launch_token_pass<RS_ITEMS, true>(a, tiles, tok, s);
+    } else {
+        if (items == RS_ITEMS_SMALL) rs_launch_token_pass<RS_ITEMS_SMALL, false>(a, tiles, tok, s);
+        else if (items == RS_ITEMS_MID) rs_launch_token_pass<RS_ITEMS_MID, false>(a, tiles, tok, s);
+        else rs_launch_token_pass<RS_ITEMS, false>(a, tiles, tok, s);
+    }
+}
+
 struct RsBuffers {
     uint2* ranges;
     uint32_t *ka, *va, *pa;
@@ -728,7 +461,7 @@
     bool aux_skip_ones;
 };
 static int rs_run(const RsPlan& pl, const RsBuffers& b, uint64_t n, void* temp, hipStream_t s, const uint32_t* n_dev,
-                  bool temp_zeroed, const uint32_t* ext_hist, bool exclusive, int key_shift = 0) {
+                  bool temp_zeroed, const uint32_t* ext_hist, bool exclusive, int key_shift = 0, bool tokens = false) {
     if (n == 0) return 0;
     if (n >= (1ull << 32)) { set_error("radix sort: more than 2^32-1 pairs"); return 1; }
     const bool scanned = rs_scanned(n);
@@ -751,6 +484,7 @@
     }
     const uint32_t* ghist = (!scanned && ext_hist) ? ext_hist : t.hist;
     const int hstride = (!scanned && ext_hist) ? 256 : pl.radix;
+    const bool token_passes = tokens && pl.npasses == 2 && !pl.depth && !payload;
     const uint32_t *kin = b.ka, *vin = b.va_is_index ? nullptr : b.va, *pin = b.pa;
     uint32_t *kout = b.kb, *vout = b.vb, *pout = b.pb;
     uint32_t *kalt = b.ka, *valt = b.va, *palt = b.pa;
@@ -774,7 +508,7 @@
         a.kfinal = b.vfinal ? b.kfinal : kout;
         a.ranges = (!pl.depth && p == pl.npasses - 1) ? b.ranges : nullptr;
         a.range_shift = key_shift;
-        if (a.ranges && key_shift == 0) a.kfinal = nullptr;
+        if (a.ranges && (key_shift == 0 || tokens)) a.kfinal = nullptr;
         a.aux_in = b.aux_in; a.aux_out = b.aux_out; a.aux_skip_ones = b.aux_skip_ones ? 1 : 0;
         if (scanned) {
             RsTileHistArgs h;
@@ -788,6 +522,12 @@
             }
         }
         const bool ballot = g_opt_radix_ballot_rank != 0;
+        if (token_passes) {
+            rs_launch_token_pass_items(a, items, scanned, tiles, p + 1, s);
+            kin = vout; vin = nullptr;
+            uint32_t* tv = valt; valt = vout; vout = tv;
+            continue;
+        }
         if (pl.db[p] == 9) {
             if (payload) rs_launch_pass_items<9, true>(a, items, scanned, tiles, ballot, s);
             else rs_launch_pass_items<9, false>(a, items, scanned, tiles, ballot, s);
@@ -806,7 +546,7 @@
 
 int radix_sort_pairs(uint32_t* ka, uint32_t* va, uint32_t* kb, uint32_t* vb, uint64_t n, int bits, void* temp,
                      hipStream_t s, const uint32_t* n_dev, bool temp_zeroed, const uint2* aux_in, uint2* aux_out,
-                     const uint32_t* ext_hist, bool aux_empty_for_ones, bool exclusive, uint2* ranges, int key_shift) {
+                     const uint32_t* ext_hist, bool aux_empty_for_ones, bool exclusive, uint2* ranges, int key_shift, bool tokens) {
     RsPlan pl = rs_plan_plain(bits);
     for (int p = 0; p < RS_MAX_PASSES; ++p) pl.shift[p] += key_shift;
     if (pl.npasses > RS_MAX_PASSES) { set_error("radix sort: more than 32 key bits"); return 1; }
@@ -814,7 +554,7 @@
     b.ranges = ranges;
     b.ka = ka; b.va = va; b.va_is_index = false; b.pa = nullptr; b.kb = kb; b.vb = vb; b.pb = nullptr; b.kfinal = nullptr; b.vfinal = nullptr;
     b.aux_in = aux_in; b.aux_out = aux_out; b.aux_skip_ones = aux_empty_for_ones;
-    return rs_run(pl, b, n, temp, s, n_dev, temp_zeroed, ext_hist, exclusive, key_shift);
+    return rs_run(pl, b, n, temp, s, n_dev, temp_zeroed, ext_hist, exclusive, key_shift, tokens);
 }
 
 int radix_sort_depth(uint32_t* keys, uint32_t* key_b, uint32_t* val_a, uint32_t* val_b, void* rect, bool payload,
diff --git a/monogs_amd/csrc/rs_pass_body.inc b/monogs_amd/csrc/rs_pass_body.inc
--- /dev/null
+++ b/monogs_amd/csrc/rs_pass_body.inc
@@ -0,0 +1,337 @@
+    constexpr int TILE_PAIRS = RS_THREADS * ITEMS;
+    constexpr int RADIX = 1 << DB, DPT = RADIX / RS_THREADS;
+    constexpr int SBUF = (SCANNED && 2 * RS_WAVES * RADIX > TILE_PAIRS) ? 2 * RS_WAVES * RADIX : TILE_PAIRS;
+    __shared__ uint32_t wave_hist[RS_WAVES][RADIX];
+    __shared__ uint32_t digit_base[RADIX];
+    __shared__ uint32_t gbase[RADIX];
+    __shared__ uint32_t sbuf[SBUF];
+    __shared__ uint32_t wsum[RS_WAVES];
+    __shared__ uint32_t s_tile;
+
+    static_assert(TOK == 0 || (DB == 8 && !PAYLOAD && !BALLOT && !VIDX), "token passes: the plain 8-bit kernel");
+    const int t = threadIdx.x, lane = t & 63, wv = t >> 6;
+    const bool wide = a.wide ? a.wide[0] != 0u : false;
+    if (a.cond == 2 && !wide) return;
+    RS_STAMP(0);
+    const bool final_pass = a.cond == 0 ? a.last != 0 : (a.cond == 1 ? !wide : true);
+    if (!SCANNED) {
+        uint32_t failed = 0;
+        for (int q = 0; q < a.pass; ++q) failed |= a.error[q];
+        if (failed) return;
+    }
+    const uint32_t n_live = a.n_dev ? min(a.n, a.n_dev[0]) : a.n;
+    if (t == 0) {
+        uint32_t id = blockIdx.x;
+        if (a.xcd_band) {
+            const uint32_t live = (n_live + (uint32_t)TILE_PAIRS - 1) / (uint32_t)TILE_PAIRS;
+            const uint32_t q = live >> 3, r = live & 7u, x = id & 7u, j = id >> 3;
+            id = j < q + (x < r ? 1u : 0u) ? x * q + min(x, r) + j : 0xFFFFFFFFu;
+        }
+        s_tile = (!SCANNED && a.ticket) ? atomicAdd(a.ticket, 1u) : id;
+    }
+#pragma unroll
+    for (int w = 0; w < RS_WAVES; ++w)
+#pragma unroll
+        for (int j = 0; j < DPT; ++j) wave_hist[w][t * DPT + j] = 0;
+    if constexpr (TOK == 2) gbase[t] = rs_token_starts(a.error)[t];
+    __syncthreads();
+    const uint32_t tile = s_tile;
+    if (tile == 0xFFFFFFFFu) return;
+    const uint32_t tile_start = tile * (uint32_t)TILE_PAIRS;
+    if (tile_start >= n_live) return;
+    const uint32_t tile_n = min((uint32_t)TILE_PAIRS, n_live - tile_start);
+
+    uint32_t hcount[DPT], before[DPT];
+#pragma unroll
+    for (int j = 0; j < DPT; ++j) hcount[j] = before[j] = 0;
+    constexpr int R4 = RADIX / 4;
+    uint4 lv[RS_MAX_LEVELS - 1][DPT], tv[RS_TOP_BATCH / RS_WAVES][DPT];
+    uint32_t lw[RS_MAX_LEVELS - 1], tw[RS_TOP_BATCH / RS_WAVES], tb[RS_TOP_BATCH / RS_WAVES];
+    const int levels = a.tree.levels;
+    const uint32_t top_node = tile >> (RS_FAN_LOG * (levels - 1));
+    const uint4* __restrict__ c4 = reinterpret_cast<const uint4*>(a.counts);
+    const uint4* __restrict__ top4 = levels == 1 ? c4 : reinterpret_cast<const uint4*>(a.sums) + (size_t)a.tree.off[levels - 1] * R4;
+    if (SCANNED) {
+#pragma unroll
+        for (int l = 0; l < RS_MAX_LEVELS - 1; ++l) {
+            const bool have = l < levels - 1;
+            const uint32_t node = tile >> (RS_FAN_LOG * l), first = node & ~3u, nb = node & 3u;
+            const uint4* base = (l == 0 || !have) ? c4 : reinterpret_cast<const uint4*>(a.sums) + (size_t)a.tree.off[l] * R4;
+            lw[l] = (have && (uint32_t)wv < nb) ? 1u : 0u;
+#pragma unroll
+            for (int j = 0; j < DPT; ++j) lv[l][j] = base[(size_t)(lw[l] ? first + (uint32_t)wv : 0u) * R4 + j * WAVE + lane];
+        }
+#pragma unroll
+        for (int q = 0; q < RS_TOP_BATCH / RS_WAVES; ++q) {
+            const uint32_t r = (uint32_t)wv + 4u * q;
+            tw[q] = r < a.tree.top_rows ? 1u : 0u;
+            tb[q] = r < top_node ? 1u : 0u;
+#pragma unroll
+            for (int j = 0; j < DPT; ++j) tv[q][j] = top4[(size_t)(tw[q] ? r : 0u) * R4 + j * WAVE + lane];
+        }
+    } else {
+#pragma unroll
+        for (int j = 0; j < DPT; ++j) hcount[j] = a.hist[t * DPT + j];
+    }
+
+    uint32_t key[ITEMS], val[ITEMS], rank[ITEMS], pay[PAYLOAD ? ITEMS : 1];
+#pragma unroll
+    for (int i = 0; i < ITEMS; ++i) {
+        const uint32_t e = (uint32_t)wv * (ITEMS * WAVE) + (uint32_t)i * WAVE + lane;
+        const bool valid = e < tile_n;
+        key[i] = valid ? a.kin[tile_start + e] : 0xFFFFFFFFu;
+        if constexpr (TOK == 2) val[i] = 0u;
+        else if constexpr (VIDX) val[i] = tile_start + e;
+        else val[i] = valid ? a.vin[tile_start + e] : 0u;
+        if constexpr (PAYLOAD) pay[i] = valid ? a.pin[tile_start + e] : 0u;
+    }
+    if constexpr (TOK == 2) {
+        const uint32_t wfirst = (uint32_t)wv * (ITEMS * WAVE);
+        if (wfirst < tile_n) {
+            const uint32_t pos_a = tile_start + wfirst, pos_b = tile_start + min(wfirst + (uint32_t)(ITEMS * WAVE), tile_n) - 1u;
+            uint32_t ca = 0, cb = 0;
+#pragma unroll
+            for (int q = 0; q < 4; ++q) {
+                const uint32_t st = gbase[lane * 4 + q];
+                ca += st <= pos_a ? 1u : 0u; cb += st <= pos_b ? 1u : 0u;
+            }
+            const uint32_t da = (uint32_t)__builtin_amdgcn_readlane((int)wave_incl_scan_dpp(ca), 63) - 1u;
+            const uint32_t db = (uint32_t)__builtin_amdgcn_readlane((int)wave_incl_scan_dpp(cb), 63) - 1u;
+#pragma unroll
+            for (int i = 0; i < ITEMS; ++i) {
+                uint32_t lo = da, hi = db;
+                const uint32_t pos = min(pos_a + (uint32_t)i * WAVE + lane, pos_b);
+                while (lo < hi) {
+                    const uint32_t mid = (lo + hi + 1u) >> 1;
+                    if (gbase[mid] <= pos) lo = mid; else hi = mid - 1u;
+                }
+                val[i] = lo;
+            }
+        }
+    }
+    if (SCANNED) {
+        uint4* part = reinterpret_cast<uint4*>(sbuf);
+#pragma unroll
+        for (int j = 0; j < DPT; ++j) {
+            uint4 ab = make_uint4(0u, 0u, 0u, 0u), at = make_uint4(0u, 0u, 0u, 0u);
+#pragma unroll
+            for (int l = 0; l < RS_MAX_LEVELS - 1; ++l) {
+                ab.x += lw[l] ? lv[l][j].x : 0u; ab.y += lw[l] ? lv[l][j].y : 0u; ab.z += lw[l] ? lv[l][j].z : 0u; ab.w += lw[l] ? lv[l][j].w : 0u;
+            }
+#pragma unroll
+            for (int q = 0; q < RS_TOP_BATCH / RS_WAVES; ++q) {
+                at.x += tw[q] ? tv[q][j].x : 0u; at.y += tw[q] ? tv[q][j].y : 0u; at.z += tw[q] ? tv[q][j].z : 0u; at.w += tw[q] ? tv[q][j].w : 0u;
+                ab.x += tb[q] ? tv[q][j].x : 0u; ab.y += tb[q] ? tv[q][j].y : 0u; ab.z += tb[q] ? tv[q][j].z : 0u; ab.w += tb[q] ? tv[q][j].w : 0u;
+            }
+            for (uint32_t r0 = RS_TOP_BATCH; r0 < a.tree.top_rows; r0 += RS_TOP_BATCH)
+#pragma unroll
+                for (int q = 0; q < RS_TOP_BATCH / RS_WAVES; ++q) {
+                    const uint32_t r = r0 + (uint32_t)wv + 4u * q;
+                    if (r < a.tree.top_rows) {
+                        const uint4 v = top4[(size_t)r * R4 + j * WAVE + lane];
+                        at.x += v.x; at.y += v.y; at.z += v.z; at.w += v.w;
+                        if (r < top_node) { ab.x += v.x; ab.y += v.y; ab.z += v.z; ab.w += v.w; }
+                    }
+                }
+            part[(wv * 2 + 0) * R4 + j * WAVE + lane] = ab;
+            part[(wv * 2 + 1) * R4 + j * WAVE + lane] = at;
+        }
+    }
+    RS_DRAIN();
+    RS_STAMP(1);
+    if (!BALLOT) {
+#pragma unroll
+        for (int i = 0; i < ITEMS; ++i) {
+            const uint32_t e = (uint32_t)wv * (ITEMS * WAVE) + (uint32_t)i * WAVE + lane;
+            const uint32_t d = (rs_xf(key[i], a.sub) >> a.shift) & (RADIX - 1);
+            rank[i] = 0;
+            if (e < tile_n) rank[i] = __hip_atomic_fetch_add(&wave_hist[wv][d], 1u, __ATOMIC_RELAXED, __HIP_MEMORY_SCOPE_WORKGROUP);
+        }
+    } else {
+        const unsigned long long lt_mask = (1ull << lane) - 1ull;
+#pragma unroll
+        for (int i = 0; i < ITEMS; ++i) {
+            const uint32_t e = (uint32_t)wv * (ITEMS * WAVE) + (uint32_t)i * WAVE + lane;
+            const bool valid = e < tile_n;
+            const uint32_t d = (rs_xf(key[i], a.sub) >> a.shift) & (RADIX - 1);
+            unsigned long long peers = __builtin_amdgcn_ballot_w64(valid);
+#pragma unroll
+            for (int b = 0; b < DB; ++b) {
+                const bool bit = (d >> b) & 1u;
+                const unsigned long long bm = __builtin_amdgcn_ballot_w64(valid && bit);
+                peers &= bit ? bm : ~bm;
+            }
+            rank[i] = 0;
+            if (valid) {
+                const uint32_t prev = wave_hist[wv][d];
+                rank[i] = prev + (uint32_t)__popcll(peers & lt_mask);
+                if ((peers & lt_mask) == 0ull) wave_hist[wv][d] = prev + (uint32_t)__popcll(peers);
+            }
+        }
+    }
+    __syncthreads();
+    if (SCANNED) {
+#pragma unroll
+        for (int j = 0; j < DPT; ++j)
+#pragma unroll
+            for (int w = 0; w < RS_WAVES; ++w) {
+                before[j] += sbuf[(w * 2 + 0) * RADIX + t * DPT + j];
+                hcount[j] += sbuf[(w * 2 + 1) * RADIX + t * DPT + j];
+            }
+    }
+    RS_STAMP(2);
+
+    uint32_t total[DPT], tsum = 0;
+#pragma unroll
+    for (int j = 0; j < DPT; ++j) {
+        uint32_t run = 0;
+#pragma unroll
+        for (int w = 0; w < RS_WAVES; ++w) {
+            const uint32_t c = wave_hist[w][t * DPT + j];
+            wave_hist[w][t * DPT + j] = run;
+            run += c;
+        }
+        total[j] = run;
+        tsum += run;
+    }
+    const uint32_t incl = wave_incl_scan_dpp(tsum);
+    if (lane == 63) wsum[wv] = incl;
+    __syncthreads();
+    uint32_t wadd = 0;
+    for (int w = 0; w < wv; ++w) wadd += wsum[w];
+    uint32_t dbase[DPT];
+    {
+        uint32_t run = wadd + incl - tsum;
+#pragma unroll
+        for (int j = 0; j < DPT; ++j) { dbase[j] = run; digit_base[t * DPT + j] = run; run += total[j]; }
+    }
+    uint32_t gdigit_base[DPT];
+    if constexpr (SCANNED) {
+        rs_digit_bases<DPT>(hcount, gdigit_base, wsum, lane, wv);
+#pragma unroll
+        for (int j = 0; j < DPT; ++j) gbase[t * DPT + j] = gdigit_base[j] + before[j] - dbase[j];
+        __syncthreads();
+    } else {
+        static_assert(DPT == 1, "the one-sweep path ranks 256 digits");
+        constexpr uint32_t G = RS_GROUP;
+        const uint32_t live_tiles = (n_live + (uint32_t)TILE_PAIRS - 1) / (uint32_t)TILE_PAIRS;
+        const uint32_t grp = tile / G, jin = tile % G;
+        const uint32_t members = min(G, live_tiles - grp * G);
+        uint64_t* gstat = a.status + (size_t)a.tiles * RADIX;
+        rs_digit_bases<DPT>(hcount, gdigit_base, wsum, lane, wv);
+        __hip_atomic_store(a.status + (size_t)tile * RADIX + t, RS_FLAG_LOCAL | (uint64_t)total[0], __ATOMIC_RELAXED,
+                           __HIP_MEMORY_SCOPE_AGENT);
+        uint32_t spins = 0, pre = 0, gpre = 0;
+        bool ok = rs_gather(a.status + (size_t)grp * G * RADIX + t, RADIX, jin, pre, spins, a.error + a.pass);
+        if (jin == members - 1)
+            __hip_atomic_store(gstat + (size_t)grp * RADIX + t, RS_FLAG_GLOBAL | (uint64_t)(pre + total[0]), __ATOMIC_RELAXED,
+                               __HIP_MEMORY_SCOPE_AGENT);
+        if (ok) ok = rs_gather(gstat + t, RADIX, grp, gpre, spins, a.error + a.pass);
+        gbase[t] = gdigit_base[0] + gpre + pre - dbase[0];
+        __syncthreads();
+    }
+
+    RS_STAMP(3);
+#pragma unroll
+    for (int i = 0; i < ITEMS; ++i) {
+        const uint32_t e = (uint32_t)wv * (ITEMS * WAVE) + (uint32_t)i * WAVE + lane;
+        const uint32_t d = (rs_xf(key[i], a.sub) >> a.shift) & (RADIX - 1);
+        rank[i] = e < tile_n ? digit_base[d] + wave_hist[wv][d] + rank[i] : 0xFFFFFFFFu;
+    }
+    rs_exchange<ITEMS>(sbuf, rank, key, t);
+    __syncthreads();
+    rs_exchange<ITEMS>(sbuf, rank, val, t);
+    if constexpr (PAYLOAD) {
+        __syncthreads();
+        rs_exchange<ITEMS>(sbuf, rank, pay, t);
+    }
+    RS_STAMP(4);
+    uint32_t g[ITEMS];
+    bool live[ITEMS];
+#pragma unroll
+    for (int i = 0; i < ITEMS; ++i) {
+        const uint32_t p = (uint32_t)i * RS_THREADS + t;
+        live[i] = p < tile_n;
+        g[i] = gbase[(rs_xf(key[i], a.sub) >> a.shift) & (RADIX - 1)] + p;
+    }
+    if (!final_pass) {
+        if constexpr (TOK == 1) {
+            if (tile == 0u) rs_token_starts(a.error)[t] = gdigit_base[0];
+            const int hs = a.shift + 8;
+#pragma unroll
+            for (int i = 0; i < ITEMS; ++i)
+                if (live[i]) a.vout[g[i]] = ((key[i] >> hs) << hs) | val[i];
+            return;
+        }
+#pragma unroll
+        for (int i = 0; i < ITEMS; ++i)
+            if (live[i]) {
+                a.kout[g[i]] = key[i];
+                a.vout[g[i]] = val[i];
+                if constexpr (PAYLOAD) a.pout[g[i]] = pay[i];
+            }
+        RS_STAMP(5); RS_DRAIN(); RS_STAMP(6); RS_STAMP(7);
+        return;
+    }
+    if constexpr (TOK == 2) {
+        const uint32_t imask = (1u << a.shift) - 1u;
+#pragma unroll
+        for (int i = 0; i < ITEMS; ++i) {
+            if (live[i]) a.vfinal[g[i]] = key[i] & imask;
+            key[i] = ((key[i] >> a.shift) << 8) | val[i];
+        }
+    } else {
+#pragma unroll
+        for (int i = 0; i < ITEMS; ++i)
+            if (live[i]) {
+                if (a.kfinal) a.kfinal[g[i]] = key[i];
+                a.vfinal[g[i]] = val[i];
+            }
+    }
+    if (a.ranges) {
+        __shared__ uint32_t s_edge[RS_WAVES * ITEMS];
+        if (lane == 63) {
+#pragma unroll
+            for (int i = 0; i < ITEMS; ++i) s_edge[wv * ITEMS + i] = key[i];
+        }
+        __syncthreads();
+#pragma unroll
+        for (int i = 0; i < ITEMS; ++i) {
+            const uint32_t p = (uint32_t)i * RS_THREADS + t;
+            uint32_t l = (uint32_t)__shfl_up((int)key[i], 1, 64);
+            if (lane == 0) l = wv > 0 ? s_edge[(wv - 1) * ITEMS + i] : (i > 0 ? s_edge[(RS_WAVES - 1) * ITEMS + i - 1] : 0xFFFFFFFFu);
+            const uint32_t kr = TOK == 2 ? key[i] : key[i] >> a.range_shift, lr = TOK == 2 ? l : l >> a.range_shift;
+            if (p < tile_n && (p == 0 || lr != kr)) {
+                atomicMin(&a.ranges[kr].x, g[i]);
+                if (p > 0)
+                    atomicMax(&a.ranges[lr].y, gbase[TOK == 2 ? l >> 8 : (rs_xf(l, a.sub) >> a.shift) & (RADIX - 1)] + p);
+            }
+            if (p + 1 == tile_n) atomicMax(&a.ranges[kr].y, g[i] + 1u);
+        }
+    }
+    RS_STAMP(5);
+    RS_DRAIN();
+    RS_STAMP(6);
+    if (a.aux_out) {
+        uint2* __restrict__ aout = a.aux_out;
+        if constexpr (PAYLOAD) {
+#pragma unroll
+            for (int i = 0; i < ITEMS; ++i)
+                if (live[i]) {
+                    const uint32_t r = pay[i];
+                    aout[g[i]] = key[i] == 0xFFFFFFFFu ? make_uint2(0u, 0u)
+                                                       : make_uint2((r & 0xFFu) | ((r & 0xFF00u) << 8), ((r >> 16) & 0xFFu) | ((r >> 24) << 16));
+                }
+        } else {
+            const uint2* __restrict__ ain = a.aux_in;
+            uint2 r[ITEMS];
+#pragma unroll
+            for (int i = 0; i < ITEMS; ++i)
+                r[i] = (live[i] && !(a.aux_skip_ones && key[i] == 0xFFFFFFFFu)) ? ain[val[i]] : make_uint2(0u, 0u);
+#pragma unroll
+            for (int i = 0; i < ITEMS; ++i)
+                if (live[i]) aout[g[i]] = r[i];
+        }
+    }
+    RS_DRAIN();
+    RS_STAMP(7);
diff --git a/monogs_amd/csrc/tile_sort.h b/monogs_amd/csrc/tile_sort.h
--- a/monogs_amd/csrc/tile_sort.h
+++ b/monogs_amd/csrc/tile_sort.h
@@ -83,15 +83,10 @@
 }
 
 __device__ inline void tds_global_sort(uint32_t* __restrict__ kx, uint32_t* __restrict__ vx, uint32_t* __restrict__ ky,
-                                       uint32_t* __restrict__ vy, uint32_t n, const uint32_t* __restrict__ depth_key, int lo,
+                                       uint32_t* __restrict__ vy, uint32_t n, const uint32_t* __restrict__ depth_key,
                                        uint32_t (*s_cnt)[TDS_RADIX], uint32_t* s_run, uint32_t* s_wsum) {
     const int t = threadIdx.x, lane = t & 63, wv = t >> 6;
-    const uint32_t imask = lo ? (1u << (32 - lo)) - 1u : 0xFFFFFFFFu;
-    for (uint32_t e = t; e < n; e += TDS_THREADS) {
-        const uint32_t g = vx[e] & imask;
-        kx[e] = depth_key[g] - DEPTH_KEY_SUB;
-        vx[e] = g;
-    }
+    for (uint32_t e = t; e < n; e += TDS_THREADS) kx[e] = depth_key[vx[e]] - DEPTH_KEY_SUB;
     for (int sh = 0; sh < 32; sh += 8) {
         __threadfence();
         if (t < 256) s_run[t] = 0u;
@@ -142,17 +137,15 @@
 }
 
 __device__ __forceinline__ uint32_t tile_depth_sort(const TileSortArgs& ts, uint2 rg, bool skip, const TdsLds& lds) {
-    const int t = threadIdx.x, lane = t & 63, wv = t >> 6;
+    const int lane = threadIdx.x & 63, wv = threadIdx.x >> 6;
     const uint32_t n_live = ts.n_dev ? min(ts.n_cap, ts.n_dev[0]) : ts.n_cap;
     const uint32_t start = rg.x, end = min(rg.y, n_live);
     if (skip || start >= end) return 0u;
     const uint32_t n = end - start;
-    const int lo = tile_depth_lo_bits(ts.tb);
-    const uint32_t kmask = ts.tb < 32 ? (0xFFFFFFFFu >> ts.tb) : 0u, imask = lo ? (1u << (32 - lo)) - 1u : 0xFFFFFFFFu;
     if (n > (uint32_t)TDS_CAP) {
         uint32_t* const k = ts.keys + start;
         uint32_t* const v = ts.vals + start;
-        tds_global_sort(k, v, ts.keys_alt + start, ts.vals_alt + start, n, ts.depth_key, lo, lds.cnt, lds.k, lds.wsum);
+        tds_global_sort(k, v, ts.keys_alt + start, ts.vals_alt + start, n, ts.depth_key, lds.cnt, lds.k, lds.wsum);
         return 0u;
     }
     uint32_t d[TDS_ITEMS], g[TDS_ITEMS];
@@ -160,11 +153,14 @@
 #pragma unroll
     for (int i = 0; i < TDS_ITEMS; ++i) {
         const uint32_t e = (uint32_t)(wv * (TDS_ITEMS * WAVE) + i * WAVE + lane);
-        d[i] = 0u; g[i] = 0u;
+        g[i] = e < n ? ts.vals[start + e] : 0u;
+    }
+#pragma unroll
+    for (int i = 0; i < TDS_ITEMS; ++i) {
+        const uint32_t e = (uint32_t)(wv * (TDS_ITEMS * WAVE) + i * WAVE + lane);
+        d[i] = 0u;
         if (e < n) {
-            const uint32_t k = ts.keys[start + e], v = ts.vals[start + e];
-            d[i] = ((k & kmask) << lo) | (lo ? v >> (32 - lo) : 0u);
-            g[i] = v & imask;
+            d[i] = ts.depth_key[g[i]] - DEPTH_KEY_SUB;
             dmin = min(dmin, d[i]); dmax = max(dmax, d[i]);
         }
     }
@@ -177,35 +173,6 @@
     }
     const uint32_t span = mx - mn;
     tds_lds_sort(lds.k, lds.v, lds.cnt, lds.wsum, 0, (int)n, span ? 32 - __builtin_clz(span) : 0);
-    if (mx == DEPTH_KEY_NARROW) {
-        uint32_t c = 0;
-#pragma unroll
-        for (int i = 0; i < TDS_ITEMS; ++i) {
-            const uint32_t e = (uint32_t)(wv * (TDS_ITEMS * WAVE) + i * WAVE + lane);
-            c += (e < n && d[i] == DEPTH_KEY_NARROW) ? 1u : 0u;
-        }
-#pragma unroll
-        for (int o = 32; o > 0; o >>= 1) c += (uint32_t)__shfl_xor((int)c, o, 64);
-        if (lane == 0) lds.red[wv] = c;
-        __syncthreads();
-        uint32_t m = 0;
-#pragma unroll
-        for (int w = 0; w < TDS_WAVES; ++w) m += lds.red[w];
-        __syncthreads();
-        const uint32_t f = n - m;
-        uint32_t xmin = 0xFFFFFFFFu, xmax = 0u;
-        for (uint32_t e = f + t; e < n; e += TDS_THREADS) {
-            const uint32_t x = ts.depth_key[lds.v[e]] - DEPTH_KEY_SUB;
-            lds.k[e] = x;
-            xmin = min(xmin, x); xmax = max(xmax, x);
-        }
-        uint32_t rmn, rmx;
-        tds_minmax(xmin, xmax, lds.red, rmn, rmx);
-        for (uint32_t e = f + t; e < n; e += TDS_THREADS) lds.k[e] -= rmn;
-        __syncthreads();
-        const uint32_t rspan = rmx - rmn;
-        tds_lds_sort(lds.k, lds.v, lds.cnt, lds.wsum, (int)f, (int)m, rspan ? 32 - __builtin_clz(rspan) : 0);
-    }
 #pragma unroll
     for (int i = 0; i < TDS_ITEMS; ++i) {
         const int e = wv * (TDS_ITEMS * WAVE) + i * WAVE + lane;
```

Result: slower. 2930 Mpix/s (-1.3%).
